# megvii-research/basedet

Hardware: AMD Instinct MI355X
Metric: images/sec training RetinaNet-R50-FPN 1333x800 (higher is better)
Workload: dtype bf16; 1 GPU; retinanet_r50_800x1344 train step (fwd+bwd+allreduce+SGD), DummyLoader boxes, random-init weights, inputs resident in HBM; per_gpu_batch=16, global_batch=16, parallelism=dp1

## Files before the change

### basedet_amd/_lib.py

```python
import ctypes as C
import os

import torch

_HERE = os.path.dirname(os.path.abspath(__file__))
LIB_PATH = os.environ.get("BASEDET_HIP_LIB") or os.path.join(_HERE, "lib", "libbasedet_hip.so")

BD_MAX_SEGS = 8
EPI_RELU, EPI_ADD_BEFORE, EPI_ADD_AFTER, EPI_MASK, EPI_SPARSE = 1, 2, 4, 8, 16


class BasedetHipError(RuntimeError):
    pass


class ConvDesc(C.Structure):
    _fields_ = [
        ("N", C.c_int32), ("Cin", C.c_int32), ("Cout", C.c_int32), ("R", C.c_int32), ("S", C.c_int32),
        ("stride", C.c_int32), ("pad", C.c_int32), ("nseg", C.c_int32),
        ("Hi", C.c_int32 * BD_MAX_SEGS), ("Wi", C.c_int32 * BD_MAX_SEGS),
        ("Ho", C.c_int32 * BD_MAX_SEGS), ("Wo", C.c_int32 * BD_MAX_SEGS),
        ("in_off", C.c_int32 * BD_MAX_SEGS), ("out_off", C.c_int32 * BD_MAX_SEGS),
        ("in_pix_per_img", C.c_int32), ("out_pix_per_img", C.c_int32),
        ("route", C.c_int32 * 4), ("sr_seed", C.c_uint32),
    ]


class PackDesc(C.Structure):
    _fields_ = [("w", C.c_void_p), ("row_scale", C.c_void_p), ("w_fwd", C.c_void_p), ("w_dgrad", C.c_void_p),
                ("Cout", C.c_int32), ("RS", C.c_int32), ("Cin", C.c_int32), ("block_start", C.c_int32)]


_P, _I, _L, _F, _Z = C.c_void_p, C.c_int, C.c_int64, C.c_float, C.c_size_t
_D = C.POINTER(ConvDesc)

SIGNATURES = {
    "bd_last_error_string": (C.c_char_p, []),
    "bd_version": (_I, []),
    "bd_conv_last_kernel": (C.c_char_p, []),
    "bd_probe_mfma_rate": (_I, [C.c_double, C.POINTER(C.c_double), C.POINTER(C.c_double), _P]),
    "bd_probe_kernel_clock": (_I, [C.c_char_p, _I, C.POINTER(C.c_double), C.POINTER(C.c_double)]),
    "bd_conv2d_fwd": (_I, [_D, _P, _P, _P, _P, _P, _I, _P]),
    "bd_conv2d_dgrad": (_I, [_D, _P, _P, _P, _P, _P, _I, _P]),
    "bd_conv2d_fwd_bits": (_I, [_D, _P, _P, _P, _P, _P, _P, _I, _P]),
    "bd_conv2d_fwd_ex": (_I, [_D, _P, _P, _P, _P, _P, _P, _P, _F, _I, _P]),
    "bd_conv2d_dgrad_ex": (_I, [_D, _P, _P, _P, _P, _P, _P, _P, _F, _I, _P]),
    "bd_conv2d_dgrad_bits": (_I, [_D, _P, _P, _P, _P, _P, _I, _P]),
    "bd_conv2d_wgrad_workspace_bytes": (_Z, [_D]),
    "bd_conv2d_wgrad": (_I, [_D, _P, _P, _P, _P, _I, _P, _Z, _P]),
    "bd_conv2d_wgrad_bias_workspace_bytes": (_Z, [_D]),
    "bd_conv2d_wgrad_bias": (_I, [_D, _P, _P, _P, _P, _P, _I, _P, _Z, _P]),
    "bd_fpn_deconv_pack": (_I, [_P, _I, _P, _P, _P]),
    "bd_fpn_deconv_fwd": (_I, [_P, _P, _P, _P, _I, _I, _I, _I, _I, _I, _P]),
    "bd_fpn_deconv_dgrad": (_I, [_P, _P, _P, _P, _I, _I, _I, _I, _I, _I, _P]),
    "bd_fpn_deconv_wgrad_workspace_bytes": (_Z, [_I, _I, _I, _I]),
    "bd_fpn_deconv_wgrad": (_I, [_P, _P, _P, _I, _P, _Z, _I, _I, _I, _I, _I, _I, _P]),
    "bd_wgrad_queue_create": (_I, [_P]),
    "bd_wgrad_queue_destroy": (_I, [_P]),
    "bd_wgrad_queue_pending": (_I, [_P]),
    "bd_conv2d_wgrad_queued": (_I, [_P, _D, _P, _P, _P, _P, _P, _I, _P, _Z, _P]),
    "bd_wgrad_queue_flush": (_I, [_P, _P]),
    "bd_stem_conv7x7_fwd": (_I, [_I, _I, _I, _P, _P, _P, _P, _P]),
    "bd_stem_pool_fwd": (_I, [_I, _I, _I, _P, _P, _P, _P, _P]),
    "bd_stem_weight_pack": (_I, [_P, _P, _P, _P]),
    "bd_weight_pack": (_I, [_P, _P, _P, _P, _I, _I, _I, _P]),
    "bd_weight_pack_blocks": (_I, [_I, _I, _I]),
    "bd_weight_pack_multi": (_I, [_P, _I, _I, _P]),
    "bd_colsum_workspace_bytes": (_Z, [_I]),
    "bd_colsum_bf16": (_I, [_P, _I, _L, _L, _L, _I, _P, _I, _P, _Z, _P]),
    "bd_pad_normalize": (_I, [_P, _I, _I, _I, _I, _I, _P, _P, _P, _P]),
    "bd_bottleneck_fwd_supported": (_I, [_I, _I, _I, _I, _I, _I, _I]),
    "bd_bottleneck_fwd": (_I, [_I, _I, _I, _I, _I, _I, _P, _P, _P, _P, _P, _P, _P, _P, _P, _P, _P]),
    "bd_h2d_create": (_I, [C.POINTER(C.c_void_p), _I, _I]),
    "bd_h2d_threads": (_I, [_P]),
    "bd_h2d_submit": (_I, [_P, _P, _I, _L, _P, _L, _P]),
    "bd_h2d_destroy": (_I, [_P]),
    "bd_pad_normalize_nchw": (_I, [_P, _I, _I, _I, _I, _I, _P, _P, _P, _P]),
    "bd_maxpool3x3s2_fwd": (_I, [_P, _I, _I, _I, _I, _P, _P]),
    "bd_upsample2x_add_fwd": (_I, [_P, _L, _L, _P, _L, _L, _I, _I, _I, _I, _P]),
    "bd_upsample2x_add_bwd": (_I, [_P, _L, _L, _P, _L, _L, _I, _I, _I, _I, _I, _P]),
    "bd_relu_bf16": (_I, [_P, _P, _L, _P]),
    "bd_relu_bwd_bf16": (_I, [_P, _P, _P, _P, _L, _P]),
    "bd_add_bf16": (_I, [_P, _P, _P, _L, _P]),
    "bd_anchors_generate": (_I, [_I, _I, _I, _F, _P, _I, _P, _P]),
    "bd_points_generate": (_I, [_I, _I, _I, _F, _I, _P, _P]),
    "bd_box_pairwise": (_I, [_P, _I, _P, _I, _I, _P, _P]),
    "bd_box_encode": (_I, [_P, _P, _L, _P, _P, _P, _P]),
    "bd_box_decode": (_I, [_P, _P, _L, _P, _P, _P, _P]),
    "bd_retina_assign_encode": (_I, [_P, _I, _P, _P, _I, _I, _F, _F, _I, _P, _P, _P, _P, _P, _P, _P, _Z, _P]),
    "bd_fcos_assign": (_I, [_P, _I, _P, _P, _P, _I, _F, _P, _P, _I, _I, _P, _P, _P, _P, _P]),
    "bd_ota_assign_workspace_bytes": (_Z, [_I, _I]),
    "bd_ota_assign": (_I, [_P, _I, _P, _P, _I, _P, _I, _P, _P, _P, _I, _I, _F, _F, _F, _F, _I, _P, _P, _P, _P, _P, _Z, _P]),
    "bd_ota_sinkhorn_workspace_bytes": (_Z, [_I, _I, _I]),
    "bd_ota_assign_sinkhorn": (_I, [_P, _I, _P, _P, _I, _P, _I, _P, _P, _P, _I, _I, _F, _F, _F, _F, _I, _F, _I, _P, _P, _P, _P, _P, _Z, _P]),
    "bd_freeanchor_workspace_bytes": (_Z, [_I, _I, _I, _I]),
    "bd_freeanchor_loss_fwd_bwd": (_I, [_P, _P, _I, _I, _P, _I, _I, _P, _P, _I, _I, _P, _P, _F, _I, _F, _F, _F, _F, _P, _P, _P, _P, _Z, _P]),
    "bd_atss_assign_workspace_bytes": (_Z, [_I, _I]),
    "bd_atss_assign": (_I, [_P, _I, _P, _P, _I, _I, _F, _P, _P, _I, _I, _P, _P, _P, _P, _P, _Z, _P]),
    "bd_nms_workspace_bytes": (_Z, [_I]),
    "bd_batched_nms": (_I, [_P, _P, _P, _I, _F, _I, _P, _P, _P, _Z, _P]),
    "bd_focal_loss_fwd_bwd": (_I, [_P, _P, _L, _I, _F, _F, _P, _I, _F, _P, _P, _P]),
    "bd_focal_loss_fwd_bwd_general": (_I, [_P, _P, _L, _I, _F, _F, _P, _I, _F, _P, _P, _P]),
    "bd_smooth_l1_fwd_bwd": (_I, [_P, _P, _P, _L, _I, _I, _F, _P, _I, _F, _P, _P, _P]),
    "bd_giou_ltrb_fwd_bwd": (_I, [_P, _P, _P, _P, _L, _P, _F, _P, _P, _P]),
    "bd_bce_logits_fwd_bwd": (_I, [_P, _I, _I, _P, _P, _L, _P, _P, _P, _P]),
    "bd_groupnorm_workspace_bytes": (_Z, [_I, _I, _I, _L]),
    "bd_groupnorm_fwd": (_I, [_P, _P, _P, _I, _I, _P, _P, _L, _I, _F, _I, _P, _P, _P, _Z, _P]),
    "bd_conv2d_fwd_gnstats_bytes": (_Z, [_D]),
    "bd_conv2d_fwd_gnstats": (_I, [_D, _P, _P, _P, _P, _P, _Z, _P]),
    "bd_groupnorm_fwd_parts": (_I, [_D, _P, _P, _P, _P, _F, _I, _P, _P, _P]),
    "bd_groupnorm_bwd": (_I, [_P, _P, _P, _P, _P, _I, _I, _P, _P, _L, _I, _I, _P, _P, _P, _I, _P, _Z, _P]),
    "bd_fcos_offsets_fwd": (_I, [_P, _I, _P, _I, _I, _P, _P, _P, _L, _P, _P]),
    "bd_fcos_offsets_workspace_bytes": (_Z, []),
    "bd_fcos_offsets_bwd": (_I, [_P, _I, _P, _I, _I, _P, _P, _P, _L, _P, _P, _P, _P, _P, _Z, _P]),
    "bd_rpn_assign_encode": (_I, [_P, _I, _P, _P, _I, _I, _F, _F, _I, _P, _P, _P, _P, _P, _P, _P, _Z, _P]),
    "bd_sample_labels": (_I, [_P, _P, _P, _I, _I, _I, _I, _P, _P]),
    "bd_segment_topk": (_I, [_P, _I, _I, _L, _I, _I, _I, _I, _P, _P, _I, _F, _I, _P, _P, _P, _P]),
    "bd_nms_batched_workspace_bytes": (_Z, [_I, _I]),
    "bd_nms_batched": (_I, [_P, _P, _P, _I, _I, _F, _I, _I, _P, _P, _P, _Z, _P]),
    "bd_rpn_proposals_workspace_bytes": (_Z, [_I, _I, _P, _I, _I, _I]),
    "bd_rpn_proposals": (_I, [_P, _I, _I, _I, _I, _I, _L, _I, _P, _P, _P, _P, _I, _P, _P, _I, _F, _I, _P, _P, _P, _Z, _P]),
    "bd_rpn_proposals_joint": (_I, [_P, _I, _I, _I, _I, _I, _L, _I, _P, _P, _P, _P, _I, _P, _P, _I, _F, _I, _P, _P, _P, _Z, _P]),
    "bd_rcnn_sample_targets": (_I, [_P, _P, _I, _P, _P, _I, _I, _P, _P, _I, _I, _I, _F, _F, _F, _P, _P, _P, _P, _P, _P, _P, _P]),
    "bd_roi_align_fwd": (_I, [_P, _L, _I, _I, _P, _P, _P, _P, _P, _P, _I, _I, _I, _I, _I, _P, _P]),
    "bd_conv1x1_thin_bwd_workspace_bytes": (_Z, []),
    "bd_conv1x1_thin_fwd": (_I, [_P, _P, _P, _L, _I, _I, _P, _P]),
    "bd_conv1x1_thin_bwd": (_I, [_P, _P, _P, _L, _I, _I, _P, _P, _P, _I, _P, _Z, _P]),
    "bd_roi_align_bwd": (_I, [_P, _L, _I, _I, _P, _P, _P, _P, _P, _P, _I, _I, _I, _I, _I, _P, _P]),
    "bd_roi_align_bwd_bf16_workspace_bytes": (_Z, [_I, _I, _P, _P, _I]),
    "bd_roi_align_bwd_bf16": (_I, [_P, _L, _I, _I, _I, _P, _P, _P, _P, _P, _P, _I, _I, _I, _I, _I, _P, _I, _P, _Z, _P]),
    "bd_subsample2x_fwd": (_I, [_P, _L, _L, _I, _I, _P, _L, _L, _I, _I, _P]),
    "bd_subsample2x_bwd_add": (_I, [_P, _L, _L, _P, _L, _L, _I, _I, _I, _I, _P]),
    "bd_f32_to_bf16": (_I, [_P, _P, _L, _P]),
    "bd_f32_to_bf16_add": (_I, [_P, _P, _L, _P]),
    "bd_rpn_loss_fwd_bwd": (_I, [_P, _I, _I, _I, _I, _P, _P, _L, _F, _P, _P, _P, _P]),
    "bd_rcnn_loss_fwd_bwd": (_I, [_P, _I, _I, _I, _P, _P, _I, _F, _P, _P, _P, _P]),
    "bd_det_scores": (_I, [_P, _P, _I, _I, _L, _I, _P, _P]),
    "bd_rcnn_predict": (_I, [_P, _I, _I, _I, _P, _P, _I, _I, _P, _P, _P, _P, _P]),
    "bd_det_candidates": (_I, [_I, _P, _P, _P, _I, _I, _P, _I, _P, _P, _I, _I, _P, _P, _P, _P, _P, _P, _P]),
    "bd_det_finalize": (_I, [_P, _P, _P, _P, _P, _I, _P, _P, _P, _P, _P]),
    "bd_sgd_momentum_step": (_I, [_P, _P, _P, _L, _F, _F, _F, _F, _P]),
    "bd_clip_grad_value": (_I, [_P, _L, _F, _F, _F, _P]),
    "bd_clip_grad_norm_workspace_bytes": (_Z, []),
    "bd_clip_grad_norm": (_I, [_P, _L, _F, _F, _F, _P, _P, _Z, _P]),
    "bd_quantize_fp8": (_I, [_P, _L, _F, _P, _P]),
    "bd_weight_pack_fp8": (_I, [_P, _P, _I, _I, _I, _F, _P, _P, _P]),
    "bd_conv2d_fwd_fp8": (_I, [_D, _P, _P, _P, _P, _P, _P, _I, _P]),
    "bd_conv2d_fwd_fp8_ex": (_I, [_D, _P, _P, _P, _P, _P, _P, _P, _F, _I, _P]),
    "bd_quantize_bf8": (_I, [_P, _L, _F, _P, C.c_uint32, _P]),
    "bd_absmax_bf16": (_I, [_P, _L, _P, _P]),
    "bd_weight_pack_fp8_t": (_I, [_P, _P, _I, _I, _I, _F, _P, _P, _P]),
    "bd_conv2d_dgrad_fp8": (_I, [_D, _P, _P, _P, _P, _P, _P, _P, _F, _I, _P]),
    "bd_conv2d_wgrad_fp8_workspace_bytes": (_Z, [_D]),
    "bd_conv2d_wgrad_fp8": (_I, [_D, _P, _P, _F, _P, _P, _I, _P, _Z, _P]),
    "bd_conv1x1_fp8": (_I, [_D, _I, _P, _P, _P, _P, _P, _P, _P, _P, _P, _P, _F, _I, _P]),
    "bd_sigmoid_focal_loss_elem": (_I, [_P, _P, _L, _F, _F, _P, _P, _P, _P]),
    "bd_bce_elem": (_I, [_P, _P, _L, _I, _P, _P, _P, _P]),
    "bd_smooth_l1_elem": (_I, [_P, _P, _L, _F, _P, _P, _P, _P]),
    "bd_iou_loss_ltrb": (_I, [_P, _P, _L, _I, _F, _P, _P, _P, _P, _P]),
    "bd_iou_to_loss": (_I, [_P, _L, _I, _F, _P, _P]),
    "bd_matcher_matrix": (_I, [_P, _I, _L, _P, _P, _I, _I, _P, _P, _P, _P]),
    "bd_assign_roi_levels": (_I, [_P, _I, _I, _I, _I, _P, _P]),
    "bd_roi_pool_max_fwd": (_I, [_P, _I, _I, _I, _I, _P, _I, _F, _I, _I, _P, _P]),
    "bd_comm_unique_id": (_I, [_P]),
    "bd_comm_init": (_I, [C.POINTER(C.c_void_p), _P, _I, _I, _I]),
    "bd_comm_rank": (_I, [_P]),
    "bd_comm_world": (_I, [_P]),
    "bd_comm_stream": (_P, [_P]),
    "bd_comm_bcast": (_I, [_P, _P, _Z, _I, _I, _P]),
    "bd_comm_allreduce": (_I, [_P, _P, _Z, _I, _I, _P]),
    "bd_comm_allreduce_async": (_I, [_P, _P, _Z, _I, _I, C.POINTER(C.c_void_p), _I]),
    "bd_comm_allreduce_async_bf16": (_I, [_P, _P, _P, _Z, _I, C.POINTER(C.c_void_p), _I]),
    "bd_comm_wait": (_I, [_P, _P]),
    "bd_comm_destroy": (_I, [_P]),
}

_lib = None


def load():
    global _lib
    if _lib is not None:
        return _lib
    if not os.path.exists(LIB_PATH):
        raise BasedetHipError(
            f"{LIB_PATH} is missing: build it with `python -m basedet_amd.build` (hipcc, gfx950). "
            "There is no CPU fallback for the basedet_amd operator path.")
    lib = C.CDLL(LIB_PATH)
    for name, (res, args) in SIGNATURES.items():
        fn = getattr(lib, name)
        fn.restype = res
        fn.argtypes = args
    _lib = lib
    return lib


# ... 27 lines not shown
```

### basedet_amd/build.py

```python
import hashlib
import os
import subprocess
import sys

HERE = os.path.dirname(os.path.abspath(__file__))
CSRC = os.path.join(HERE, "csrc")
OUT_DIR = os.path.join(HERE, "lib")
LIB = os.path.join(OUT_DIR, os.environ.get("BD_LIB_NAME", "libbasedet_hip.so"))
HIPCC = os.environ.get("HIPCC", "/opt/rocm/bin/hipcc")
ARCH = "gfx950"

SOURCES = {
    "image_ops.hip": [],
    "h2d.hip": [],
    "conv_igemm.hip": [],
    "conv3x3.hip": [],
    "conv3x3_pp.hip": [],
    "conv3x3_pp128.hip": [],
    "conv1x1.hip": [],
    "conv1x1_ring.hip": [],
    "conv1x1_thin.hip": [],
    "bottleneck_fused.hip": [],
    "conv_fp8.hip": [],
    "conv3x3_pp8.hip": [],
    "conv_wgrad.hip": [],
    "conv_wgrad3x3.hip": [],
    "conv_wgrad3x3_ring.hip": [],
    "conv_wgrad3x3_fp8.hip": [],
    "conv_wgrad1x1.hip": [],
    "conv_wgrad1x1_ring.hip": [],
    "fpn_deconv.hip": [],
    "stem.hip": [],
    "boxops.hip": ["-ffp-contract=off"],
    "rcnn_ops.hip": ["-ffp-contract=off"],
    "postprocess.hip": ["-ffp-contract=off"],
    "freeanchor.hip": ["-ffp-contract=off"],
    "ota.hip": ["-ffp-contract=off"],
    "losses.hip": [],
    "norm.hip": [],
    "comm.hip": [],
    "layer_ops.hip": ["-ffp-contract=off"],
    "probe.hip": [],
}
COMMON = ["-O3", "-std=c++17", "-fPIC", f"--offload-arch={ARCH}", "-Wno-unused-result", "-I", os.path.join(HERE, "..", "include")]
COMMON += os.environ.get("BD_EXTRA_FLAGS", "").split()


def _digest():
    h = hashlib.sha256()
    for name in sorted(os.listdir(CSRC)) + ["../../include/basedet_hip.h"]:
        with open(os.path.join(CSRC, name), "rb") as f:
            h.update(name.encode())
            h.update(f.read())
    flags = [f for f in COMMON if not os.path.isabs(f)]
    h.update(repr(sorted(SOURCES.items())).encode() + repr(flags).encode())
    return h.hexdigest()


def build(force=False, verbose=True):
    os.makedirs(OUT_DIR, exist_ok=True)
    stamp = os.path.join(OUT_DIR, "build.stamp" if "BD_LIB_NAME" not in os.environ else os.environ["BD_LIB_NAME"] + ".stamp")
    dig = _digest()
    if not force and os.path.exists(LIB) and os.path.exists(stamp) and open(stamp).read().strip() == dig:
        return LIB
    objs = []
    procs = []
    for src, extra in SOURCES.items():
        obj = os.path.join(OUT_DIR, os.environ.get("BD_LIB_NAME", "") + src.replace(".hip", ".o"))
        cmd = [HIPCC, *COMMON, *extra, "-c", os.path.join(CSRC, src), "-o", obj]
        if verbose:
            print(" ".join(cmd), flush=True)
        procs.append((src, subprocess.Popen(cmd, stdout=subprocess.PIPE, stderr=subprocess.STDOUT, text=True)))
        objs.append(obj)
    failed = False
    for src, p in procs:
        out, _ = p.communicate()
        if p.returncode != 0:
            failed = True
            sys.stderr.write(f"--- {src} failed ---\n{out}\n")
        elif verbose and out.strip():
            print(out)
    if failed:
        raise RuntimeError("hipcc failed")
    cmd = [HIPCC, "-shared", "-fPIC", f"--offload-arch={ARCH}", "-o", LIB, *objs]
    if verbose:
        print(" ".join(cmd), flush=True)
    subprocess.check_call(cmd)
    with open(stamp, "w") as f:
        f.write(dig)
    return LIB


def build_driver(verbose=False):
    src = os.path.join(HERE, "..", "tools", "abi_driver.cpp")
    name = os.path.basename(LIB)
    out = os.path.join(OUT_DIR, "abi_driver" if name == "libbasedet_hip.so" else "abi_driver." + name)
    lib = build(force=False, verbose=verbose)
    if os.path.exists(out) and os.path.getmtime(out) >= max(os.path.getmtime(src), os.path.getmtime(lib)):
        return out
    cmd = [HIPCC, "-O2", "-std=c++17", "-x", "hip", f"--offload-arch={ARCH}", "-I", os.path.join(HERE, "..", "include"), src,
           "-o", out, "-L", OUT_DIR, "-l:" + os.path.basename(LIB), "-Wl,-rpath,$ORIGIN", "-Wno-unused-result", "-Wno-unused-value"]
    if verbose:
        print(" ".join(cmd), flush=True)
    subprocess.check_call(cmd)
    return out


if __name__ == "__main__":
    print(build(force="--force" in sys.argv))
    print(build_driver(verbose=True))
```

### basedet_amd/csrc/conv3x3_pp.hip

```cpp
#include "conv3x3_pp128_body.h"

namespace {

constexpr int PH = 4, PW = 16, IH = PH + 2, IW = PW + 2;
constexpr int NPATCH = 4;
constexpr int XROWS = NPATCH * IH * IW;
constexpr int X_PITCH = 144;
constexpr int X_BYTES = XROWS * X_PITCH;
constexpr int XPASSES = 7;
constexpr int TILE_CO = 256;
constexpr int W_SLOT = TILE_CO * 128;
constexpr int NSLOT = 3;
constexpr int W_BYTES = NSLOT * W_SLOT;
constexpr int GTAB_TILES = 16;
constexpr int GTAB_BYTES = GTAB_TILES * NPATCH * 32;
constexpr int LDS_BYTES = W_BYTES + X_BYTES + TILE_CO * 4 + GTAB_BYTES;
constexpr int MAX_SEG = BD_MAX_SEGS;
constexpr int TAIL_CO = 64;

struct PSeg { int patch_start, H, W, pw, src_off, dst_off; float inv_pw; };

struct PParams {
    const bf16_raw* src;
    const bf16_raw* w;
    const float* bias;
    const bf16_raw* add;
    const bf16_raw* mask;
    bf16_raw* dst;
    int CK, CO, flags, nseg;
    int src_ppi, dst_ppi;
    unsigned src_bytes;
    int patches_per_img, total_patches, n_tiles;
    int main_grid;
    int px_tiles;
    int tail_end;
    float inv_ppi;
    PSeg seg[MAX_SEG];
    float* gn_part;
};

typedef __attribute__((address_space(3))) void lds_void_t;
typedef __attribute__((address_space(1))) const void glb_void_t;

__device__ __forceinline__ int pp_div(int n, int d, float inv) {
    int q = (int)((float)n * inv);
    const int r = n - q * d;
    q += (r >= d) - (r < 0);
    return q;
}

__device__ __forceinline__ int swz(int row, int chunk) { return row * 128 + ((chunk ^ (row & 7)) << 4); }
__device__ __forceinline__ int colperm(int f) { return f < 4 ? 2 * f : (f < 12 ? 2 * (f - 4) + 1 : 2 * (f - 8)); }
__device__ __forceinline__ int xpos(int chunk) { return (chunk >> 2) * 64 + ((((chunk & 1) << 1) | ((chunk >> 1) & 1)) << 4); }

#ifdef BD_PP_STAMP
__device__ unsigned long long g_pp_stamp[64];
__device__ unsigned long long g_pp_span[2048];
#endif
#ifndef BD_PP_ABLATE
#define BD_PP_ABLATE 0
#endif
__device__ unsigned long long g_pp_clk[2];
#define PP_FENCE() __builtin_amdgcn_sched_barrier(0)
#define PP_BARRIER() do { asm volatile("" ::: "memory"); __builtin_amdgcn_s_barrier(); asm volatile("" ::: "memory"); } while (0)

template <int MODE, bool GNS = false>
__global__ __launch_bounds__(512, 1) void conv3x3_pp_kernel(const PParams p) {
    extern __shared__ __attribute__((aligned(16))) unsigned char smem[];
    if ((int)blockIdx.x >= p.main_grid) {
        pp128::body<MODE, TAIL_CO>(p, smem, (int)blockIdx.x - p.main_grid, (int)gridDim.x - p.main_grid, p.total_patches, p.tail_end,
                                   (p.CO + TAIL_CO - 1) / TAIL_CO);
        return;
    }
    if (blockIdx.x == 0 && threadIdx.x == 0) bd_clk_mark(g_pp_clk, false);
    unsigned char* wbuf = smem;
    unsigned char* xbuf = smem + W_BYTES;
    float* sbias = reinterpret_cast<float*>(smem + W_BYTES + X_BYTES);

#ifdef BD_PP_STAMP
    int st_n = 0;
    const bool st_on = blockIdx.x == 100 % gridDim.x && threadIdx.x == 0;
#define PP_STAMP() do { if (st_on && st_n < 62) g_pp_stamp[st_n] = __builtin_amdgcn_s_memtime(); ++st_n; } while (0)
    PP_STAMP();
    if (st_on) g_pp_stamp[62] = __builtin_amdgcn_s_memrealtime();
    if (threadIdx.x == 0 && blockIdx.x < 1024) g_pp_span[2 * blockIdx.x] = __builtin_amdgcn_s_memrealtime();
#else
#define PP_STAMP() do { } while (0)
#endif
    const int tid = threadIdx.x, lane = tid & 63, wave = __builtin_amdgcn_readfirstlane(tid >> 6);
    const int wm = wave >> 2, wp = wave & 3;
    int bid = blockIdx.x;
    {
        const int nwg = p.main_grid;
        const int q = nwg >> 3, r = nwg & 7, xcd = bid & 7;
        bid = (xcd < r ? xcd * (q + 1) : r * (q + 1) + (xcd - r) * q) + (bid >> 3);
    }
    const int ct = bid % p.n_tiles;
    int pt = bid / p.n_tiles;
    const int pt_step = p.main_grid / p.n_tiles;
    const int co0 = ct * TILE_CO;

    constexpr unsigned X_NONE = 0x80000000u;
    const int x_lds0 = (tid >> 3) * X_PITCH + xpos(tid & 7);
    unsigned x_off[XPASSES];

    int* gtab = reinterpret_cast<int*>(smem + W_BYTES + X_BYTES + TILE_CO * 4);
    const int pt_first = pt;
    auto build_table = [&](int k0) {
        const int k = k0 + (lane >> 2);
        const int ptile = pt_first + k * pt_step;
        const int pid = ptile * NPATCH + (lane & (NPATCH - 1));
        int vH = 0, vW = 0, vy = 0, vx = 0, vs = 0, vd = 0;
        if (ptile < p.px_tiles && pid < p.total_patches) {
            const int n = pp_div(pid, p.patches_per_img, p.inv_ppi);
            const int rem = pid - n * p.patches_per_img;
            int g_start = p.seg[0].patch_start, g_H = p.seg[0].H, g_W = p.seg[0].W, g_pw = p.seg[0].pw;
            int g_src = p.seg[0].src_off, g_dst = p.seg[0].dst_off;
            float g_inv = p.seg[0].inv_pw;
#pragma unroll
            for (int q = 1; q < MAX_SEG; ++q) {
                const bool in = q < p.nseg && rem >= p.seg[q].patch_start;
                g_start = in ? p.seg[q].patch_start : g_start; g_H = in ? p.seg[q].H : g_H; g_W = in ? p.seg[q].W : g_W;
                g_pw = in ? p.seg[q].pw : g_pw; g_src = in ? p.seg[q].src_off : g_src; g_dst = in ? p.seg[q].dst_off : g_dst;
                g_inv = in ? p.seg[q].inv_pw : g_inv;
            }
            const int local = rem - g_start;
            const int by = pp_div(local, g_pw, g_inv), bx = local - by * g_pw;
            vy = by * PH; vx = bx * PW; vH = g_H; vW = g_W;
            vs = n * p.src_ppi + g_src;
            vd = n * p.dst_ppi + g_dst;
        }
        typedef __attribute__((ext_vector_type(4))) int i32x4_t;
        i32x4_t* e = reinterpret_cast<i32x4_t*>(gtab + ((k & (GTAB_TILES - 1)) * NPATCH + (lane & (NPATCH - 1))) * 8);
        e[0] = (i32x4_t){vy, vx, vH, vW};
        e[1] = (i32x4_t){vs, vd, 0, 0};
    };
    auto decode = [&](int k, int& e_oy0, int& e_px0, int& e_H, int& e_W, int& e_dst) {
        int py0[NPATCH], px0[NPATCH], pH[NPATCH], pWd[NPATCH];
        int psrc[NPATCH], pdst[NPATCH];
        int tq = tid;
        asm volatile("" : "+v"(tq));
        {
            typedef __attribute__((ext_vector_type(4))) int i32x4_t;
            const i32x4_t* e = reinterpret_cast<const i32x4_t*>(gtab + ((k & (GTAB_TILES - 1)) * NPATCH + (tq & (NPATCH - 1))) * 8);
            const i32x4_t e0 = e[0], e1 = e[1];
#pragma unroll
            for (int q = 0; q < NPATCH; ++q) {
                py0[q] = __builtin_amdgcn_readlane(e0[0], q); px0[q] = __builtin_amdgcn_readlane(e0[1], q);
                pH[q] = __builtin_amdgcn_readlane(e0[2], q); pWd[q] = __builtin_amdgcn_readlane(e0[3], q);
                psrc[q] = __builtin_amdgcn_readlane(e1[0], q); pdst[q] = __builtin_amdgcn_readlane(e1[1], q);
            }
        }
#pragma unroll
        for (int k = 0; k < XPASSES; ++k) {
            const int row = (tq >> 3) + 64 * k;
            unsigned off = X_NONE;
            if (row < XROWS) {
                const int lo = (64 * k) / (IH * IW), hi = (64 * k + 63) / (IH * IW) < NPATCH ? (64 * k + 63) / (IH * IW) : NPATCH - 1;
                const bool up = row >= hi * (IH * IW);
                const int pk = up ? hi : lo;
                const int rr = row - pk * (IH * IW);
                const int iy = rr / IW, ix = rr - iy * IW;
                const int qy = up ? py0[hi] : py0[lo], qx = up ? px0[hi] : px0[lo], H = up ? pH[hi] : pH[lo];
                const int W = up ? pWd[hi] : pWd[lo], qs = up ? psrc[hi] : psrc[lo];
                const int y = qy - 1 + iy, x = qx - 1 + ix;
                if (y >= 0 && x >= 0 && y < H && x < W) off = (unsigned)((qs + y * W + x) * p.CK + (tq & 7) * 8) * 2u;
            }
            x_off[k] = off;
        }
        e_oy0 = py0[0]; e_px0 = px0[0]; e_H = pH[0]; e_W = pWd[0]; e_dst = pdst[0];
#pragma unroll
        for (int q = 1; q < NPATCH; ++q)
            if (wp == q) { e_oy0 = py0[q]; e_px0 = px0[q]; e_H = pH[q]; e_W = pWd[q]; e_dst = pdst[q]; }
    };
    int c_oy0, c_px0, c_H, c_W, c_dst;
    int kt = 0;
    if (wave == 0) build_table(0);
    asm volatile("s_waitcnt lgkmcnt(0)" ::: "memory");
    PP_BARRIER();
    decode(0, c_oy0, c_px0, c_H, c_W, c_dst);
    const __amdgpu_buffer_rsrc_t x_rsrc =
        __builtin_amdgcn_make_buffer_rsrc(const_cast<bf16_raw*>(p.src), 0, p.src_bytes, 0x00020000);
    u32x4_t rx[XPASSES];
    auto load_x = [&](int cb) {
        int so = cb * 128;
        asm volatile("" : "+s"(so));
        const bool dead = cb * 64 + (tid & 7) * 8 >= p.CK;
#pragma unroll
        for (int k = 0; k < XPASSES; ++k) rx[k] = __builtin_amdgcn_raw_buffer_load_b128(x_rsrc, dead ? X_NONE : x_off[k], so, 0);
    };
    auto write_x = [&]() {
#pragma unroll
        for (int k = 0; k < XPASSES; ++k)
            if (k < XPASSES - 1 || (tid >> 3) + 64 * k < XROWS)
                *reinterpret_cast<u32x4_t*>(xbuf + x_lds0 + k * (64 * X_PITCH)) = rx[k];
    };

    unsigned dma_src[4];
#pragma unroll
    for (int k = 0; k < 4; ++k) {
        const int pc = wave + 8 * k;
        const int lrow = 8 * pc + (lane >> 3);
        const int chunk = (lane & 7) ^ (lane >> 3);
        const int rho = lrow & 15;
        int co = co0 + (lrow & 192) + 32 * ((lrow >> 5) & 1) + 8 * (rho >> 2) + 4 * ((lrow >> 4) & 1) + (rho & 3);
        if (co >= p.CO) co = p.CO - 1;
        dma_src[k] = (unsigned)(co * 9 * p.CK + chunk * 8) * 2u;
    }
    const __amdgpu_buffer_rsrc_t w_rsrc =
        __builtin_amdgcn_make_buffer_rsrc(const_cast<bf16_raw*>(p.w), 0, (unsigned)(p.CO * 9 * p.CK) * 2u, 0x00020000);
    bool dma_on = true;
    auto dma_piece = [&](int tap, int cb, int slot, int k) {
        if ((BD_PP_ABLATE & 2) && !dma_on) return;
        unsigned char* l = wbuf + slot * W_SLOT + (wave + 8 * k) * 1024;
        int so = (tap * p.CK + cb * 64) * 2;
        asm volatile("" : "+s"(so));
        __builtin_amdgcn_raw_ptr_buffer_load_lds(w_rsrc, (lds_void_t*)l, 16, dma_src[k], so, 0, 0);
    };

    f32x4_t acc[8][4];

    const int frow = lane & 15, fchunk = lane >> 4;
    const unsigned char* a_base[2];
#pragma unroll
    for (int kk = 0; kk < 2; ++kk) a_base[kk] = wbuf + swz(wm * 128 + frow, kk * 4 + fchunk);
    typedef __attribute__((address_space(3))) const unsigned char lds_u8_t;
    typedef __attribute__((address_space(3))) const bf16x8_t lds_bf16x8_t;
    unsigned a_hi[2];
#pragma unroll
    for (int kk = 0; kk < 2; ++kk) {
        a_hi[kk] = (unsigned)(size_t)(lds_u8_t*)(a_base[kk]) + 2 * W_SLOT;
        asm volatile("" : "+v"(a_hi[kk]));
    }
    const unsigned char* b_base = xbuf + (wp * (IH * IW) + colperm(frow)) * X_PITCH + xpos(fchunk);

    bf16x8_t fa[8], fb[4];
    auto load_a = [&](int kk, int slot) {
#pragma unroll
        for (int i = 0; i < 8; ++i) {
            if (slot == 2) fa[i] = *(lds_bf16x8_t*)(size_t)(a_hi[kk] + i * 2048);
            else fa[i] = *reinterpret_cast<const bf16x8_t*>(a_base[kk] + slot * W_SLOT + i * 2048);
        }
    };
    auto load_b = [&](int kk, int t) {
        int dy = t / 3, dx = t - 3 * (t / 3);
        if (MODE == 1) { dy = 2 - dy; dx = 2 - dx; }
#pragma unroll
        for (int j = 0; j < 4; ++j)
            fb[j] = *reinterpret_cast<const bf16x8_t*>(b_base + ((j + dy) * IW + dx) * X_PITCH + kk * 64);
    };
    auto mfma_rows = [&](int i0, int i1) {
#pragma unroll
        for (int i = i0; i < i1; ++i)
#pragma unroll
            for (int j = 0; j < 4; ++j)
                asm volatile("v_mfma_f32_16x16x32_bf16 %0, %1, %2, %0" : "+v"(acc[i][j]) : "v"(fa[i]), "v"(fb[j]));
    };

    const int kblocks = (p.CK + 63) >> 6;

    PP_STAMP();
    if (tid < TILE_CO) sbias[tid] = (p.bias && co0 + tid < p.CO) ? p.bias[co0 + tid] : 0.f;
    load_x(0);
#pragma unroll
    for (int k = 0; k < 4; ++k) dma_piece(0, 0, 0, k);
#pragma unroll
    for (int k = 0; k < 4; ++k) dma_piece(1, 0, 1, k);
#pragma unroll
    for (int k = 0; k < 4; ++k) dma_piece(2, 0, 2, k);
    write_x();
    asm volatile("s_waitcnt vmcnt(0) lgkmcnt(0)" ::: "memory");
    PP_BARRIER();
    PP_FENCE();
    if (BD_PP_ABLATE & 2) dma_on = false;

    PP_STAMP();
#if defined(BD_PP_PRIO) && BD_PP_PRIO == 1
    if (wm == 1) __builtin_amdgcn_s_setprio(1);
#endif
    for (;;) {
    const int pt_next = pt + pt_step;
    const bool more = pt_next < p.px_tiles;
    int n_oy0 = 0, n_px0 = 0, n_H = 0, n_W = 0, n_dst = 0;
#pragma unroll
    for (int i = 0; i < 8; ++i)
#pragma unroll
        for (int j = 0; j < 4; ++j) acc[i][j] = (f32x4_t){0.f, 0.f, 0.f, 0.f};
    for (int cb = 0; cb < kblocks; ++cb) {
        const bool last_kb = cb + 1 == kblocks;
        const bool cont = !last_kb || more;
        const int nb = last_kb ? 0 : cb + 1;
        if (last_kb) PP_STAMP();
        if (last_kb && more) decode(kt + 1, n_oy0, n_px0, n_H, n_W, n_dst);
        if (wm == 1) PP_BARRIER();
        PP_FENCE();
#pragma unroll
        for (int t = 0; t < 9; ++t) {
#pragma unroll
            for (int kk = 0; kk < 2; ++kk) {
                const int slot = t % 3;
                if (!((BD_PP_ABLATE & 1) && kk == 1)) {
                load_b(kk, t);
                PP_FENCE();
                load_a(kk, slot);
                PP_FENCE();
                }
                if (kk == 1) {
                    if (BD_PP_ABLATE & 2) { }
                    else if (!cont && t >= 7) asm volatile("s_waitcnt vmcnt(0)" ::: "memory");
                    else if (t >= 1 || cb > 0) asm volatile("s_waitcnt vmcnt(1)" ::: "memory");
                    if (t == 6) {
                        if (cont) load_x(nb);
                        else {
#pragma unroll
                            for (int k = 0; k < XPASSES; ++k) asm volatile("" : "=v"(rx[k]));
                        }
                    }
                    PP_FENCE();
                }
                if (kk == 0) {
                    if (t + 1 < 9) { if (t > 1 || cb > 0) dma_piece(t + 1, cb, (t + 1) % 3, 3); }
                    else if (cont) dma_piece(0, nb, 0, 3);
                    if (t + 2 < 9) { if (t > 0 || cb > 0) dma_piece(t + 2, cb, (t + 2) % 3, 0); }
                    else if (cont) dma_piece(t - 7, nb, (t + 2) % 3, 0);
                } else {
#pragma unroll
                    for (int pc = 1; pc < 3; ++pc) {
                        if (t + 2 < 9) { if (t > 0 || cb > 0) dma_piece(t + 2, cb, (t + 2) % 3, pc); }
                        else if (cont) dma_piece(t - 7, nb, (t + 2) % 3, pc);
                    }
                    if (t == 8 && last_kb && more) dma_piece(1, 0, 1, 3);
                }
                PP_FENCE();
                PP_BARRIER();
                asm volatile("s_waitcnt lgkmcnt(0)" ::: "memory");
                PP_FENCE();
#if defined(BD_PP_PRIO) && BD_PP_PRIO == 0
                __builtin_amdgcn_s_setprio(1);
#endif
                mfma_rows(0, 8);
#if defined(BD_PP_PRIO) && BD_PP_PRIO == 0
                __builtin_amdgcn_s_setprio(0);
#endif
                PP_FENCE();
                PP_BARRIER();
                PP_FENCE();
            }
        }
        if (wm == 0) PP_BARRIER();
        PP_FENCE();
        if (cont) {
            write_x();
            asm volatile("s_waitcnt lgkmcnt(0)" ::: "memory");
            PP_BARRIER();
            PP_FENCE();
        }
    }

    PP_STAMP();
    asm volatile("s_nop 15\n\ts_nop 15" ::: "memory");
    int lq = lane;
    asm volatile("" : "+v"(lq));
    const int cg = lq >> 4, erow = lq & 15;
    const bool do_relu = !GNS && (p.flags & BD_EPI_RELU);
    const bool add_before = !GNS && (p.flags & BD_EPI_ADD_BEFORE) && p.add;
    const bool add_after = !GNS && (p.flags & BD_EPI_ADD_AFTER) && p.add;
    const bool do_mask = !GNS && (p.flags & BD_EPI_MASK) && p.mask;
    const int cbase = co0 + wm * 128 + 8 * cg;
    const int oy0 = c_oy0, ox = c_px0 + colperm(erow), H = c_H, W = c_W, dbase = c_dst;
    if (!add_before && !add_after) {
        typedef __attribute__((ext_vector_type(2))) float f32x2_e;
        typedef __attribute__((ext_vector_type(2))) __bf16 bf16x2_e;
        typedef __attribute__((ext_vector_type(2))) short i16x2_e;
        const i16x2_e relu_floor = do_relu ? (i16x2_e){0, 0} : (i16x2_e){-32768, -32768};
        bf16_raw* drow[4];
        const bf16_raw* mrow[4];
        bool okj[4];
#pragma unroll
        for (int j = 0; j < 4; ++j) {
            const int oy = oy0 + j;
            okj[j] = oy < H && ox < W;
            const long long e = (long long)(dbase + oy * W + ox) * p.CO + cbase;
            drow[j] = p.dst + e;
            mrow[j] = p.mask + e;
        }
        u32x4_t mv[4][4];
#pragma unroll
        for (int h = 0; h < 4; ++h) {
            const bool okh = cbase + 32 * h < p.CO;
#pragma unroll
            for (int j = 0; j < 4; ++j) {
                mv[h][j] = (u32x4_t){0u, 0u, 0u, 0u};
                if (do_mask && okh && okj[j]) mv[h][j] = *reinterpret_cast<const u32x4_t*>(mrow[j] + 32 * h);
            }
        }
        PP_FENCE();
        if (more) {
#pragma unroll
            for (int k = 0; k < 4; ++k) dma_piece(2, 0, 2, k);
        }
        PP_FENCE();
        float gsum[4] = {0.f, 0.f, 0.f, 0.f}, gsq[4] = {0.f, 0.f, 0.f, 0.f};
        auto unit = [&](int h, int j, const f32x4_t b0, const f32x4_t b1) {
            u32x4_t o;
#pragma unroll
            for (int k = 0; k < 4; ++k) {
                const f32x4_t a = acc[2 * h + (k >> 1)][j];
                const f32x4_t bb = (k >> 1) ? b1 : b0;
                f32x2_e v = {a[2 * (k & 1)], a[2 * (k & 1) + 1]};
                v += (f32x2_e){bb[2 * (k & 1)], bb[2 * (k & 1) + 1]};
                if constexpr (GNS) {
                    if (okj[j]) { gsum[h] += v[0] + v[1]; gsq[h] += v[0] * v[0] + v[1] * v[1]; }
                }
                i16x2_e w = __builtin_bit_cast(i16x2_e, __builtin_convertvector(v, bf16x2_e));
                if (do_mask) {
                    unsigned gate;
                    asm("v_pk_sub_i16 %0, 0, %1 clamp\n\tv_pk_ashrrev_i16 %0, 15, %0 op_sel_hi:[0,1]" : "=v"(gate) : "v"(mv[h][j][k]));
                    w &= __builtin_bit_cast(i16x2_e, gate);
                }
                w = __builtin_elementwise_max(w, relu_floor);
                o[k] = __builtin_bit_cast(unsigned, w);
            }
            return o;
        };
#pragma unroll
        for (int h = 0; h < 4; ++h) {
            const bool okh = cbase + 32 * h < p.CO;
            const f32x4_t b0 = *reinterpret_cast<const f32x4_t*>(sbias + wm * 128 + 8 * cg + 32 * h);
            const f32x4_t b1 = *reinterpret_cast<const f32x4_t*>(sbias + wm * 128 + 8 * cg + 32 * h + 4);
            if (h == 0) {
                u32x4_t o0[4];
#pragma unroll
                for (int j = 0; j < 4; ++j) o0[j] = unit(0, j, b0, b1);
                PP_FENCE();
                PP_STAMP();
                if (more) asm volatile("s_waitcnt vmcnt(4)" ::: "memory");
                else asm volatile("s_waitcnt vmcnt(0)" ::: "memory");
                PP_STAMP();
                PP_FENCE();
#pragma unroll
                for (int j = 0; j < 4; ++j) {
                    if (BD_PP_ABLATE & 4) asm volatile("" :: "v"(o0[j]));
                    else if (okh && okj[j]) *reinterpret_cast<u32x4_t*>(drow[j]) = o0[j];
                }
            } else {
#pragma unroll
                for (int j = 0; j < 4; ++j) {
                    const u32x4_t o = unit(h, j, b0, b1);
                    if (BD_PP_ABLATE & 4) asm volatile("" :: "v"(o));
                    else if (okh && okj[j]) *reinterpret_cast<u32x4_t*>(drow[j] + 32 * h) = o;
                }
            }
        }
        if constexpr (GNS) {
            const int pid = pt * NPATCH + wp;
#pragma unroll
            for (int h = 0; h < 4; ++h) {
                float a = gsum[h], b = gsq[h];
#pragma unroll
                for (int m = 8; m >= 1; m >>= 1) { a += __shfl_xor(a, m, 64); b += __shfl_xor(b, m, 64); }
                if (erow == 0 && pid < p.total_patches && cbase + 32 * h < p.CO) {
                    float* o = p.gn_part + ((long long)pid * 32 + ((cbase + 32 * h) >> 3)) * 2;
                    *reinterpret_cast<f32x2_t*>(o) = (f32x2_t){a, b};
                }
            }
        }
    } else {
    if (more) {
#pragma unroll
        for (int k = 0; k < 4; ++k) dma_piece(2, 0, 2, k);
    }
    long long erow_off[4];
#pragma unroll
    for (int j = 0; j < 4; ++j) erow_off[j] = (long long)(dbase + (oy0 + j) * W + ox) * p.CO + cbase;
#pragma unroll
    for (int hp = 0; hp < 2; ++hp) {
        u32x4_t av[2][4], mv[2][4];
#pragma unroll
        for (int hh = 0; hh < 2; ++hh) {
            const int h = 2 * hp + hh;
#pragma unroll
            for (int j = 0; j < 4; ++j) {
                const int oy = oy0 + j;
                const bool ok = cbase + 32 * h < p.CO && oy < H && ox < W;
                const long long idx = erow_off[j] + 32 * h;
                av[hh][j] = (u32x4_t){0u, 0u, 0u, 0u}; mv[hh][j] = (u32x4_t){0u, 0u, 0u, 0u};
                if (ok && (add_before || add_after)) av[hh][j] = *reinterpret_cast<const u32x4_t*>(p.add + idx);
                if (ok && do_mask) mv[hh][j] = *reinterpret_cast<const u32x4_t*>(p.mask + idx);
            }
        }
        if (hp == 0) asm volatile("s_waitcnt vmcnt(0)" ::: "memory");
#pragma unroll
        for (int hh = 0; hh < 2; ++hh) {
            const int h = 2 * hp + hh;
            if (cbase + 32 * h >= p.CO) continue;
            float bias[8];
            {
                const f32x4_t b0 = *reinterpret_cast<const f32x4_t*>(sbias + wm * 128 + 8 * cg + 32 * h);
                const f32x4_t b1 = *reinterpret_cast<const f32x4_t*>(sbias + wm * 128 + 8 * cg + 32 * h + 4);
#pragma unroll
                for (int k = 0; k < 4; ++k) { bias[k] = b0[k]; bias[4 + k] = b1[k]; }
            }
#pragma unroll
            for (int j = 0; j < 4; ++j) {
                const int oy = oy0 + j;
                if (oy >= H || ox >= W) continue;
                const long long idx = erow_off[j] + 32 * h;
                float v[8];
#pragma unroll
                for (int k = 0; k < 8; ++k) v[k] = acc[2 * h + (k >> 2)][j][k & 3] + bias[k];
                const u32x4_t a4 = av[hh][j], m4 = mv[hh][j];
                if (add_before) {
#pragma unroll
                    for (int k = 0; k < 4; ++k) { v[2 * k] += bf_lo(a4[k]); v[2 * k + 1] += bf_hi(a4[k]); }
                }
                if (do_relu) {
#pragma unroll
                    for (int k = 0; k < 8; ++k) v[k] = fmaxf(v[k], 0.f);
                }
                if (do_mask) {
#pragma unroll
                    for (int k = 0; k < 4; ++k) {
                        if (!(bf_lo(m4[k]) > 0.f)) v[2 * k] = 0.f;
                        if (!(bf_hi(m4[k]) > 0.f)) v[2 * k + 1] = 0.f;
                    }
                }
                if (add_after) {
#pragma unroll
                    for (int k = 0; k < 4; ++k) { v[2 * k] += bf_lo(a4[k]); v[2 * k + 1] += bf_hi(a4[k]); }
                }
                u32x4_t o;
#pragma unroll
                for (int k = 0; k < 4; ++k) o[k] = pack_bf2(v[2 * k], v[2 * k + 1]);
                *reinterpret_cast<u32x4_t*>(p.dst + idx) = o;
            }
        }
    }
    }
    PP_STAMP();
    if (!more) break;
    ++kt;
    pt = pt_next;
    c_oy0 = n_oy0; c_px0 = n_px0; c_H = n_H; c_W = n_W; c_dst = n_dst;
    PP_FENCE();
    PP_STAMP();
    }
    if (blockIdx.x == 0 && threadIdx.x == 0) bd_clk_mark(g_pp_clk, true);
#ifdef BD_PP_STAMP
    if (st_on) { g_pp_stamp[63] = __builtin_amdgcn_s_memrealtime(); g_pp_stamp[61] = __builtin_amdgcn_s_memtime(); }
    if (threadIdx.x == 0 && blockIdx.x < 1024) { asm volatile("s_waitcnt vmcnt(0)" ::: "memory"); g_pp_span[2 * blockIdx.x + 1] = __builtin_amdgcn_s_memrealtime(); }
#endif
}

}

BD_KNOB int g_pp_tail_split = 1;
BD_KNOB int g_pp_persistent = 1;
extern BD_KNOB int g_patch_pp;
static int pp_launch(const bd_conv_desc* d, int mode, const void* src, const void* w, const float* bias, const void* add,
                     const void* mask, void* dst, int flags, float* gn_part, hipStream_t stream) {
    PParams p{};
    p.gn_part = gn_part;
    p.CK = mode == 0 ? d->Cin : d->Cout;
    p.CO = mode == 0 ? d->Cout : d->Cin;
    p.src_ppi = mode == 0 ? d->in_pix_per_img : d->out_pix_per_img;
    p.dst_ppi = mode == 0 ? d->out_pix_per_img : d->in_pix_per_img;
    if (p.CK % 8 != 0 || p.CO <= 128 || p.CO % 8 != 0) return 1;
    if ((long long)d->N * p.src_ppi * p.CK * 2 >= 0x7fffffffll || (long long)d->N * p.dst_ppi >= 0x7fffffffll ||
        (long long)p.CO * 9 * p.CK >= 0x7fffffffll) return 1;
    p.src = (const bf16_raw*)src; p.w = (const bf16_raw*)w; p.bias = bias;
    p.add = (const bf16_raw*)add; p.mask = (const bf16_raw*)mask; p.dst = (bf16_raw*)dst;
    p.flags = flags; p.nseg = d->nseg;
    p.src_bytes = (unsigned)((long long)d->N * p.src_ppi * p.CK * 2);
    int ps = 0;
    for (int s = 0; s < d->nseg; ++s) {
        PSeg& sg = p.seg[s];
        sg.patch_start = ps; sg.H = d->Ho[s]; sg.W = d->Wo[s]; sg.pw = cdiv(d->Wo[s], PW); sg.inv_pw = 1.0f / (float)sg.pw;
        sg.src_off = mode == 0 ? d->in_off[s] : d->out_off[s];
        sg.dst_off = mode == 0 ? d->out_off[s] : d->in_off[s];
        ps += cdiv(d->Ho[s], PH) * sg.pw;
    }
    p.patches_per_img = ps;
    p.inv_ppi = 1.0f / (float)ps;
    p.total_patches = ps * d->N;
    if (p.total_patches >= (1 << 24)) return 1;
    p.n_tiles = cdiv(p.CO, TILE_CO);
    int grid = cdiv(p.total_patches, NPATCH) * p.n_tiles;
    int tail_wgs = 0;
    int px_tiles = cdiv(p.total_patches, NPATCH);
    p.tail_end = p.total_patches;
    const int num_cus = bd_num_cus();
    if (g_pp_tail_split && !gn_part && p.n_tiles == 1 && px_tiles > num_cus) {
        const int r = px_tiles % num_cus;
        if (r > 0 && r * (TILE_CO / TAIL_CO) <= num_cus) {
            px_tiles -= r;
            p.total_patches = px_tiles * NPATCH;
            tail_wgs = cdiv(p.tail_end - p.total_patches, NPATCH) * cdiv(p.CO, TAIL_CO);
        }
    }
    p.px_tiles = px_tiles;
    p.main_grid = px_tiles * p.n_tiles;
    if (g_pp_persistent) {
        const int g1 = (num_cus / p.n_tiles) * p.n_tiles;
        const int rounds = cdiv(px_tiles * p.n_tiles, g1 * GTAB_TILES);
        if (g1 * rounds < p.main_grid) p.main_grid = g1 * rounds;
    }
    {
        const int grid128 = cdiv(p.total_patches, NPATCH) * cdiv(p.CO, 128);
        if (!gn_part && g_patch_pp < 2 && 3 * cdiv(grid, 256) >= 2 * cdiv(grid128, 256)) return 1;
    }
    BD_ONCE_PER_DEVICE(
        (void)hipFuncSetAttribute(reinterpret_cast<const void*>(&conv3x3_pp_kernel<0>), hipFuncAttributeMaxDynamicSharedMemorySize, LDS_BYTES);
        (void)hipFuncSetAttribute(reinterpret_cast<const void*>(&conv3x3_pp_kernel<1>), hipFuncAttributeMaxDynamicSharedMemorySize, LDS_BYTES));
    bd_note_kernel("conv3x3_pp_kernel");
    if (gn_part) {
        BD_ONCE_PER_DEVICE((void)hipFuncSetAttribute(reinterpret_cast<const void*>(&conv3x3_pp_kernel<0, true>), hipFuncAttributeMaxDynamicSharedMemorySize, LDS_BYTES));
        hipLaunchKernelGGL((conv3x3_pp_kernel<0, true>), dim3(p.main_grid), dim3(512), LDS_BYTES, stream, p);
    } else if (mode == 0) hipLaunchKernelGGL((conv3x3_pp_kernel<0>), dim3(p.main_grid + tail_wgs), dim3(512), LDS_BYTES, stream, p);
    else hipLaunchKernelGGL((conv3x3_pp_kernel<1>), dim3(p.main_grid + tail_wgs), dim3(512), LDS_BYTES, stream, p);
    return 0;
}

int bd_pp_clk_read(unsigned long long* out2, int reset) {
    if (hipMemcpyFromSymbol(out2, HIP_SYMBOL(g_pp_clk), 16) != hipSuccess) return 1;
    if (reset) { const unsigned long long z[2] = {0, 0}; if (hipMemcpyToSymbol(HIP_SYMBOL(g_pp_clk), z, 16) != hipSuccess) return 1; }
    return 0;
}

#ifdef BD_PP_STAMP
extern "C" int bd_debug_pp_stamp(unsigned long long* out2) {
    return hipMemcpyFromSymbol(out2, HIP_SYMBOL(g_pp_stamp), 512) == hipSuccess ? 0 : 1;
}
extern "C" int bd_debug_pp_span(unsigned long long* out2048) {
    return hipMemcpyFromSymbol(out2048, HIP_SYMBOL(g_pp_span), 2048 * 8) == hipSuccess ? 0 : 1;
}
#endif

int bd_conv3x3_pp_launch(const bd_conv_desc* d, int mode, const void* src, const void* w, const float* bias, const void* add,
                         const void* mask, void* dst, int flags, hipStream_t stream) {
    return pp_launch(d, mode, src, w, bias, add, mask, dst, flags, nullptr, stream);
}

int bd_conv3x3_pp_patch_starts(const bd_conv_desc* d, int* starts) {
    int ps = 0;
    for (int s = 0; s < d->nseg; ++s) { starts[s] = ps; ps += cdiv(d->Ho[s], PH) * cdiv(d->Wo[s], PW); }
    starts[d->nseg] = ps;
    return ps;
}

extern "C" size_t bd_conv2d_fwd_gnstats_bytes(const bd_conv_desc* d) {
    if (!d || d->nseg < 1 || d->nseg > BD_MAX_SEGS) return 0;
    int starts[BD_MAX_SEGS + 1];
    return (size_t)d->N * bd_conv3x3_pp_patch_starts(d, starts) * 32 * 2 * sizeof(float);
}

extern "C" int bd_conv2d_fwd_gnstats(const bd_conv_desc* d, const void* x, const void* w_packed, const float* bias, void* y, float* part,
                                     size_t part_bytes, bd_stream_t stream) {
    BD_ROUTE(d);
    BD_REQUIRE(d && x && w_packed && y && part, "conv2d_fwd_gnstats: null pointer");
    BD_REQUIRE(d->R == 3 && d->S == 3 && d->stride == 1 && d->pad == 1 && d->Cout == 256 && d->Cin % 64 == 0,
               "conv2d_fwd_gnstats: 3x3 / stride 1 / pad 1 into 256 channels (GroupNorm(32, 256)) only; got %dx%d s%d p%d %d -> %d", d->R, d->S,
               d->stride, d->pad, d->Cin, d->Cout);
    for (int s = 0; s < d->nseg; ++s)
        BD_REQUIRE(d->Hi[s] == d->Ho[s] && d->Wi[s] == d->Wo[s], "conv2d_fwd_gnstats: level %d changes size", s);
    if (part_bytes < bd_conv2d_fwd_gnstats_bytes(d)) { bd_set_error("conv2d_fwd_gnstats: statistics buffer too small"); return BD_EWORKSPACE; }
    if (pp_launch(d, 0, x, w_packed, bias, nullptr, nullptr, y, 0, part, (hipStream_t)stream) != 0) {
        bd_set_error("conv2d_fwd_gnstats: shape not taken by conv3x3_pp_kernel (tensor too large for 32-bit offsets?)");
        return BD_EINVAL;
    }
    BD_CHECK_LAUNCH("bd_conv2d_fwd_gnstats");
    return BD_OK;
}
```

### basedet_amd/csrc/conv_igemm.hip

```cpp
#include "igemm_params.h"

using namespace igemm;

namespace {

template <int BK>
struct Cfg {
    static constexpr int CHUNKS = BK / 8;
    static constexpr int ROWS_PER_PASS = 256 / CHUNKS;
    static constexpr int PASSES = 128 / ROWS_PER_PASS;
    static constexpr int LDS_STRIDE = BK == 64 ? 160 : 64;
    static constexpr int TILE_BYTES = 128 * LDS_STRIDE;
    __device__ static __forceinline__ int off(int row, int chunk) {
        if constexpr (BK == 64) return row * LDS_STRIDE + chunk * 16;
        else return row * 64 + ((chunk ^ ((row >> 1) & 3)) << 4);
    }
};

template <int BK, bool PRE, bool BUF>
__global__ __launch_bounds__(256) void conv_igemm_kernel(const IgemmParams p) {
    using C = Cfg<BK>;
    extern __shared__ __attribute__((aligned(16))) unsigned char smem[];
    unsigned char* tiles = smem;
    unsigned int* s_tapmask = reinterpret_cast<unsigned int*>(smem);
// ... 380 lines not shown

}


int bd_conv3x3_patch_launch(const bd_conv_desc* d, int mode, const void* src, const void* w, const float* bias,
                            const void* add, const void* mask, void* dst, int flags, hipStream_t stream);

extern BD_KNOB int g_patch_dma;
extern BD_KNOB int g_patch_pp;
extern BD_KNOB int g_patch_pp128;
extern BD_KNOB int g_conv1x1_s2;
extern BD_KNOB int g_pp_tail_split;
extern BD_KNOB int g_pp_persistent;
static int bd_route_patch3x3(int enable) {
#ifdef BD_AB_SKIP
    g_skip_s2_3x3 = (enable >> 4) & 1;
#else
    if ((enable >> 4) & 1) {
        bd_set_error("bd_conv_desc.route[1]: bit 4 (skip the 3x3 / stride-2 launches: a timing A/B that leaves stale outputs) exists in "
                     "-DBD_AB_SKIP diagnostic builds only");
        return BD_EINVAL;
    }
#endif
    g_use_patch3x3 = enable & 1; g_bk32_for_1x1 = (enable >> 1) & 1;
    g_patch_dma = ((enable >> 3) & 1) ^ 1;
    g_patch_pp = ((enable >> 6) & 1) ? 0 : (((enable >> 7) & 1) ? 1 : 2);
    g_patch_pp128 = ((enable >> 9) & 1) ? -1 : ((enable >> 8) & 1);
    g_bk32_s2 = ((enable >> 10) & 1) ^ 1;
    g_igemm_prefetch_epi = ((enable >> 5) & 1) ^ 1;
    g_igemm_buf = ((enable >> 11) & 1) ^ 1;
    g_conv1x1_s2 = ((enable >> 12) & 1) ^ 1;
    g_pp_tail_split = ((enable >> 13) & 1) ^ 1;
    g_pp_persistent = ((enable >> 14) & 1) ^ 1;
    if ((enable >> 16) & 1) {
        bd_set_error("bd_conv_desc.route[1]: bit 16 (conv_igemm_wide.hip) is gone since round 6");
        return BD_EINVAL;
    }
    return BD_OK;
}

int bd_route_dense1x1(int depth);
int bd_route_wgrad(int use_tr);
extern BD_KNOB int g_fp8_patch;

BdRouteScope::BdRouteScope(const bd_conv_desc* d) : rc(BD_OK) {
    const int r0 = d ? d->route[0] : 0, r1 = d ? d->route[1] : 0, r2 = d ? d->route[2] : 0, r3 = d ? d->route[3] : 0;
    if (r0 < 0 || r1 < 0 || r2 < 0 || r3 < 0) {
        bd_set_error("bd_conv_desc.route: negative word (0 = the library's choice, otherwise the route + 1)");
        rc = BD_EINVAL;
        return;
    }
    if ((rc = bd_route_dense1x1(r0 ? r0 - 1 : 1)) != BD_OK) return;
    if ((rc = bd_route_patch3x3(r1 ? r1 - 1 : 3)) != BD_OK) return;
    if ((rc = bd_route_wgrad(r2 ? r2 - 1 : 1)) != BD_OK) return;
    g_fp8_patch = r3 ? (r3 - 1 != 0) : 1;
    g_fp8_sr_seed = d ? d->sr_seed : 0u;
}

int bd_conv1x1_dense_launch(const void* x, const void* w, const float* bias, const void* add, const void* mask, const unsigned* maskbits,
                            void* y, unsigned* ybits, void* y8, float q_scale, int y8_bf8, long long M, int CK, int CO, int flags,
                            hipStream_t stream);

int bd_conv1x1_s2_launch(const bd_conv_desc* d, int mode, const void* src, const void* w, const float* bias, const void* add, const void* mask,
                         const unsigned* maskbits, void* dst, int flags, hipStream_t stream);
namespace {
bool is_dense_1x1(const bd_conv_desc* d) {
    return d->R == 1 && d->S == 1 && d->stride == 1 && d->pad == 0 && d->nseg == 1 && d->in_off[0] == 0 && d->out_off[0] == 0 &&
           d->in_pix_per_img == d->Hi[0] * d->Wi[0] && d->out_pix_per_img == d->Ho[0] * d->Wo[0];
}
}

static int conv2d_fwd_impl(const bd_conv_desc* d, const void* x, const void* w_packed, const float* bias, const void* add, void* y,
                           unsigned* ybits, void* y8, float q_scale, int flags, bd_stream_t stream) {
    if (int e = check_desc(d)) return e;
    BD_REQUIRE(x && w_packed && y, "conv2d_fwd: null pointer");
    BD_REQUIRE(d->Cin % 8 == 0, "conv2d_fwd: Cin=%d must be a multiple of 8", d->Cin);
    BD_REQUIRE(d->Cout % 8 == 0, "conv2d_fwd: Cout=%d must be a multiple of 8", d->Cout);
    BD_REQUIRE(!(flags & BD_EPI_MASK), "conv2d_fwd: BD_EPI_MASK is a dgrad-only flag");
    if (is_dense_1x1(d) &&
        bd_conv1x1_dense_launch(x, w_packed, bias, add, nullptr, nullptr, y, ybits, y8, q_scale, 0, (long long)d->N * d->out_pix_per_img,
                                d->Cin, d->Cout, flags, (hipStream_t)stream) == 0) {
        BD_CHECK_LAUNCH("bd_conv2d_fwd(dense 1x1)");
        return BD_OK;
    }
    if (!ybits && !y8 && d->stride == 2 && d->R == 1 &&
        bd_conv1x1_s2_launch(d, 0, x, w_packed, bias, add, nullptr, nullptr, y, flags, (hipStream_t)stream) == 0) {
        BD_CHECK_LAUNCH("bd_conv2d_fwd(1x1 stride 2)");
        return BD_OK;
    }
    BD_REQUIRE(ybits == nullptr && y8 == nullptr, "conv2d_fwd_bits / _ex: the bit-packed ReLU mask and the e4m3 twin are written by the dense "
               "1x1 kernel only (1x1 / stride 1 over one dense level, Cout %% 32 == 0, tensors < 2 GB)");
#ifdef BD_AB_SKIP
    if (g_skip_s2_3x3 && d->R == 3 && d->S == 3 && d->stride == 2) return BD_OK;
#endif
    if (g_use_patch3x3 && is_3x3s1(d)) {
        bd_conv3x3_patch_launch(d, 0, x, w_packed, bias, add, nullptr, y, flags, (hipStream_t)stream);
        BD_CHECK_LAUNCH("bd_conv2d_fwd(3x3 patch)");
        return BD_OK;
    }
    IgemmParams p{};
    p.src = (const bf16_raw*)x; p.w = (const bf16_raw*)w_packed; p.bias = bias;
    p.add = (const bf16_raw*)add; p.mask = nullptr; p.dst = (bf16_raw*)y;
    p.CK = d->Cin; p.CO = d->Cout; p.R = d->R; p.S = d->S; p.stride = d->stride; p.pad = d->pad;
    p.mode = 0; p.flags = flags;
    p.nsub = d->nseg;
    long long m = 0;
    for (int s = 0; s < d->nseg; ++s) {
        SubSeg& ss = p.sub[s];
        ss.m_start = (int)m;
        ss.Hs = d->Ho[s]; ss.Ws = d->Wo[s]; ss.y0 = 0; ss.x0 = 0; ss.step = 1;
        ss.Wd = d->Wo[s]; ss.dst_off = d->out_off[s];
        ss.Hsrc = d->Hi[s]; ss.Wsrc = d->Wi[s]; ss.src_off = d->in_off[s];
        ss.inv_per_img = 1.0f / (float)(ss.Hs * ss.Ws); ss.inv_ws = 1.0f / (float)ss.Ws;
        m += (long long)d->N * d->Ho[s] * d->Wo[s];
    }
    BD_REQUIRE(m < (1ll << 24), "conv2d_fwd: too many pixels (2^24 limit of the fast index decode)");
    p.linear_dst = (d->nseg == 1 && d->out_off[0] == 0 && d->out_pix_per_img == d->Ho[0] * d->Wo[0]) ? 1 : 0;
    p.linear_src = (p.linear_dst && d->R == 1 && d->S == 1 && d->stride == 1 && d->pad == 0 && d->in_off[0] == 0 &&
                    d->in_pix_per_img == d->Hi[0] * d->Wi[0]) ? 1 : 0;
    p.M = (int)m;
    p.src_pix_per_img = d->in_pix_per_img; p.dst_pix_per_img = d->out_pix_per_img;
    set_buffer_sizes(p, d->N);
    p.m_tiles = cdiv(p.M, TILE_P); p.n_tiles = cdiv(p.CO, TILE_C);
    if (p.CK > 32 && !(g_bk32_for_1x1 && p.R * p.S == 1) && !(g_bk32_s2 && p.stride == 2 && p.m_tiles * p.n_tiles >= 512))
        launch_igemm<64>(p, (hipStream_t)stream);
    else launch_igemm<32>(p, (hipStream_t)stream);
    BD_CHECK_LAUNCH("bd_conv2d_fwd");
    return BD_OK;
}

extern "C" int bd_conv2d_fwd(const bd_conv_desc* d, const void* x, const void* w_packed, const float* bias,
                             const void* add, void* y, int flags, bd_stream_t stream) {
    BD_ROUTE(d);
    return conv2d_fwd_impl(d, x, w_packed, bias, add, y, nullptr, nullptr, 1.f, flags, stream);
}

extern "C" int bd_conv2d_fwd_ex(const bd_conv_desc* d, const void* x, const void* w_packed, const float* bias, const void* add, void* y,
                                uint32_t* ybits, void* y8, float q_scale, int flags, bd_stream_t stream) {
    BD_ROUTE(d);
    return conv2d_fwd_impl(d, x, w_packed, bias, add, y, ybits, y8, q_scale, flags, stream);
}

extern "C" int bd_conv2d_fwd_bits(const bd_conv_desc* d, const void* x, const void* w_packed, const float* bias, const void* add, void* y,
                                  uint32_t* ybits, int flags, bd_stream_t stream) {
    BD_ROUTE(d);
    BD_REQUIRE(ybits != nullptr, "conv2d_fwd_bits: null ybits");
    return conv2d_fwd_impl(d, x, w_packed, bias, add, y, ybits, nullptr, 1.f, flags, stream);
}

static int conv2d_dgrad_impl(const bd_conv_desc* d, const void* g, const void* w_packed_t, const void* add, const void* mask,
                             const unsigned* maskbits, void* dx, void* dx8, float q_scale, int flags, bd_stream_t stream) {
    if (int e = check_desc(d)) return e;
    BD_REQUIRE(g && w_packed_t && dx, "conv2d_dgrad: null pointer");
    if (d->stride == 1) flags &= ~BD_EPI_SPARSE;
    BD_REQUIRE(d->Cout % 8 == 0, "conv2d_dgrad: Cout=%d must be a multiple of 8 (pad the gradient)", d->Cout);
    BD_REQUIRE(d->Cin % 8 == 0, "conv2d_dgrad: Cin=%d must be a multiple of 8", d->Cin);
    BD_REQUIRE(!(flags & BD_EPI_RELU), "conv2d_dgrad: BD_EPI_RELU is a forward-only flag");
    if (is_dense_1x1(d) &&
        bd_conv1x1_dense_launch(g, w_packed_t, nullptr, add, mask, maskbits, dx, nullptr, dx8, q_scale, 1, (long long)d->N * d->in_pix_per_img,
                                d->Cout, d->Cin, flags, (hipStream_t)stream) == 0) {
        BD_CHECK_LAUNCH("bd_conv2d_dgrad(dense 1x1)");
        return BD_OK;
    }
    if (!dx8 && d->stride == 2 && d->R == 1 &&
        bd_conv1x1_s2_launch(d, 1, g, w_packed_t, nullptr, add, mask, maskbits, dx, flags, (hipStream_t)stream) == 0) {
        BD_CHECK_LAUNCH("bd_conv2d_dgrad(1x1 stride 2)");
        return BD_OK;
    }
    BD_REQUIRE(maskbits == nullptr && dx8 == nullptr, "conv2d_dgrad_bits / _ex: the bit-packed ReLU mask is read, and the e5m2 twin written, by "
               "the dense 1x1 kernel only (1x1 / stride 1 over one dense level, Cin %% 32 == 0, tensors < 2 GB)");
#ifdef BD_AB_SKIP
    if (g_skip_s2_3x3 && d->R == 3 && d->S == 3 && d->stride == 2) return BD_OK;
#endif
    if (g_use_patch3x3 && is_3x3s1(d)) {
        bd_conv3x3_patch_launch(d, 1, g, w_packed_t, nullptr, add, mask, dx, flags, (hipStream_t)stream);
        BD_CHECK_LAUNCH("bd_conv2d_dgrad(3x3 patch)");
        return BD_OK;
    }
    IgemmParams p{};
    p.src = (const bf16_raw*)g; p.w = (const bf16_raw*)w_packed_t; p.bias = nullptr;
    p.add = (const bf16_raw*)add; p.mask = (const bf16_raw*)mask; p.dst = (bf16_raw*)dx;
    p.CK = d->Cout; p.CO = d->Cin; p.R = d->R; p.S = d->S; p.stride = d->stride; p.pad = d->pad;
    p.mode = 1; p.flags = flags;
    long long m = 0;
    int ns = 0;
    const int st = d->stride;
    const bool sparse = (flags & BD_EPI_SPARSE) && st > 1;
    BD_REQUIRE(!(flags & BD_EPI_SPARSE) || ((flags & BD_EPI_ADD_BEFORE) && add == dx),
               "conv2d_dgrad: BD_EPI_SPARSE needs an in-place accumulate (BD_EPI_ADD_BEFORE with add == dx)");
    p.flags = flags & ~BD_EPI_SPARSE;
    for (int s = 0; s < d->nseg; ++s) {
        for (int qy = 0; qy < st; ++qy)
            for (int qx = 0; qx < st; ++qx) {
                const int Hs = (d->Hi[s] - qy + st - 1) / st, Ws = (d->Wi[s] - qx + st - 1) / st;
                if (Hs <= 0 || Ws <= 0) continue;
                if (sparse) {
                    bool ry = false, rx = false;
                    for (int r = 0; r < d->R; ++r) ry = ry || ((qy + d->pad - r) % st + st) % st == 0;
                    for (int c = 0; c < d->S; ++c) rx = rx || ((qx + d->pad - c) % st + st) % st == 0;
                    if (!(ry && rx)) continue;
                }
                BD_REQUIRE(ns < MAX_SUB, "conv2d_dgrad: too many sub-segments (levels x stride^2 > %d)", MAX_SUB);
                SubSeg& ss = p.sub[ns++];
                ss.m_start = (int)m;
                ss.Hs = Hs; ss.Ws = Ws; ss.y0 = qy; ss.x0 = qx; ss.step = st;
                ss.Wd = d->Wi[s]; ss.dst_off = d->in_off[s];
                ss.Hsrc = d->Ho[s]; ss.Wsrc = d->Wo[s]; ss.src_off = d->out_off[s];
                ss.inv_per_img = 1.0f / (float)(Hs * Ws); ss.inv_ws = 1.0f / (float)Ws;
                m += (long long)d->N * Hs * Ws;
            }
    }
    p.nsub = ns;
    BD_REQUIRE(m < (1ll << 24), "conv2d_dgrad: too many pixels (2^24 limit of the fast index decode)");
    p.linear_dst = (d->nseg == 1 && st == 1 && d->in_off[0] == 0 && d->in_pix_per_img == d->Hi[0] * d->Wi[0]) ? 1 : 0;
    p.linear_src = (p.linear_dst && d->R == 1 && d->S == 1 && d->pad == 0 && d->out_off[0] == 0 &&
                    d->out_pix_per_img == d->Ho[0] * d->Wo[0]) ? 1 : 0;
    p.M = (int)m;
    p.src_pix_per_img = d->out_pix_per_img; p.dst_pix_per_img = d->in_pix_per_img;
    set_buffer_sizes(p, d->N);
    p.m_tiles = cdiv(p.M, TILE_P); p.n_tiles = cdiv(p.CO, TILE_C);
    if (p.CK > 32 && !(g_bk32_for_1x1 && p.R * p.S == 1) && !(g_bk32_s2 && p.stride == 2 && p.m_tiles * p.n_tiles >= 512))
        launch_igemm<64>(p, (hipStream_t)stream);
    else launch_igemm<32>(p, (hipStream_t)stream);
    BD_CHECK_LAUNCH("bd_conv2d_dgrad");
    return BD_OK;
}

extern "C" int bd_conv2d_dgrad(const bd_conv_desc* d, const void* g, const void* w_packed_t, const void* add,
                               const void* mask, void* dx, int flags, bd_stream_t stream) {
    BD_ROUTE(d);
    return conv2d_dgrad_impl(d, g, w_packed_t, add, mask, nullptr, dx, nullptr, 1.f, flags, stream);
}

extern "C" int bd_conv2d_dgrad_ex(const bd_conv_desc* d, const void* g, const void* w_packed_t, const void* add, const void* mask,
                                  const uint32_t* maskbits, void* dx, void* dx8, float q_scale, int flags, bd_stream_t stream) {
    BD_ROUTE(d);
    return conv2d_dgrad_impl(d, g, w_packed_t, add, maskbits ? nullptr : mask, maskbits, dx, dx8, q_scale,
                             maskbits ? (flags | BD_EPI_MASK) : flags, stream);
}

extern "C" int bd_conv2d_dgrad_bits(const bd_conv_desc* d, const void* g, const void* w_packed_t, const void* add, const uint32_t* maskbits,
                                    void* dx, int flags, bd_stream_t stream) {
    BD_ROUTE(d);
    BD_REQUIRE(maskbits != nullptr, "conv2d_dgrad_bits: null maskbits");
    return conv2d_dgrad_impl(d, g, w_packed_t, add, nullptr, maskbits, dx, nullptr, 1.f, flags | BD_EPI_MASK, stream);
}
```

### basedet_amd/csrc/conv_wgrad.hip

```cpp
#include <vector>
#include "common.h"

namespace {

constexpr int TILE = 128;
constexpr int ROW_PITCH = 288;
constexpr int MAX_SEG = BD_MAX_SEGS;

struct WSeg {
    int m_start;
    int Ho, Wo, per_img;
    float inv_per_img, inv_wo;
    int Hi, Wi, in_off, out_off;
};

struct WgradParams {
    const bf16_raw* x;
    const bf16_raw* g;
    float* slab;
    int Cin, Cout, R, S, stride, pad;
    int M, nseg;
    int in_pix_per_img, out_pix_per_img;
    int ci_tiles, co_tiles, splits, steps_per_split, total_steps;
    WSeg seg[MAX_SEG];
// ... 147 lines not shown
        if (more) stage_write(cur ^ 1);
        __syncthreads();
        cur ^= 1;
    }

    float* slab = p.slab + (long long)split * p.Cout * RS * p.Cin;
#pragma unroll
    for (int j = 0; j < 4; ++j) {
        const int co = co0 + wco * 64 + j * 16 + idx;
        if (co >= p.Cout) continue;
#pragma unroll
        for (int i = 0; i < 4; ++i) {
            const int ci = ci0 + wci * 64 + i * 16 + g4 * 4;
            if (ci >= p.Cin) continue;
            *reinterpret_cast<f32x4_t*>(slab + ((long long)co * RS + tap) * p.Cin + ci) = acc[i][j];
        }
    }
}

}
#include "wgrad_reduce.h"
namespace {

__global__ __launch_bounds__(256) void wgrad_batch_reduce_kernel(const BdRedBatch b) {
    __shared__ f32x4_t red[4][64];
    int ei = 0;
#pragma unroll 1
    for (int k = 1; k < b.count; ++k)
        if ((int)blockIdx.x >= b.e[k].block_begin) ei = k;
    const BdRedEntry& en = b.e[ei];
    const int tx = threadIdx.x & 63, ty = threadIdx.x >> 6;
    const long long e = (long long)((int)blockIdx.x - en.block_begin) * 64 + tx;
    const long long n4 = en.n4;
    f32x4_t s = {0.f, 0.f, 0.f, 0.f};
    if (e < n4) {
        const long long stride = n4 * 4;
        const float* src = en.slab + e * 4;
        const int splits = en.splits;
        int k = ty;
        for (; k + 12 < splits; k += 16) {
            const f32x4_t v0 = *reinterpret_cast<const f32x4_t*>(src + (long long)k * stride);
            const f32x4_t v1 = *reinterpret_cast<const f32x4_t*>(src + (long long)(k + 4) * stride);
            const f32x4_t v2 = *reinterpret_cast<const f32x4_t*>(src + (long long)(k + 8) * stride);
            const f32x4_t v3 = *reinterpret_cast<const f32x4_t*>(src + (long long)(k + 12) * stride);
            s += v0; s += v1; s += v2; s += v3;
        }
        for (; k < splits; k += 4) s += *reinterpret_cast<const f32x4_t*>(src + (long long)k * stride);
    }
    red[ty][tx] = s;
    __syncthreads();
    if (ty != 0 || e >= n4) return;
    f32x4_t t = red[0][tx];
    t += red[1][tx]; t += red[2][tx]; t += red[3][tx];
    long long idx;
    int row;
    if (en.kind == 0) {
        idx = e * 4;
        row = (int)(idx / en.row_len);
    } else {
        const int regs = en.regs;
        const long long per_tile = 8ll * regs * 64;
        const int tile = (int)(e / per_tile);
        int r = (int)(e - tile * per_tile);
        const int wave = r / (regs * 64);
        r -= wave * (regs * 64);
        const int reg = r >> 6, lane = r & 63;
        const int ci_tile = tile / en.co_tiles, co_tile = tile - ci_tile * en.co_tiles;
        int co, ci, tap = 0, taps = 1;
        if (en.kind == 1) {
            tap = reg >> 2; taps = 9;
            co = co_tile * en.tco + (wave >> 2) * 64 + (reg & 3) * 16 + (lane & 15);
            ci = ci_tile * en.tci + (wave & 3) * 16 + (lane >> 4) * 4;
        } else {
            const int i = reg / en.fj, j = reg - i * en.fj;
            const int wco_n = en.tco / (16 * en.fj);
            const int wci = wave / wco_n, wco = wave - wci * wco_n;
            co = co_tile * en.tco + (wco * en.fj + j) * 16 + (lane & 15);
            ci = ci_tile * en.tci + (wci * en.fi + i) * 16 + (lane >> 4) * 4;
        }
        if (co >= en.Cout || ci >= en.Cin) return;
        idx = ((long long)co * taps + tap) * en.Cin + ci;
        row = co;
    }
    float* d = en.dw + idx;
    if (en.row_scale) t *= en.row_scale[row];
    if (en.accumulate) t += *reinterpret_cast<const f32x4_t*>(d);
    *reinterpret_cast<f32x4_t*>(d) = t;
}

int launch_batch(const BdRedEntry* entries, int count, hipStream_t stream) {
    for (int base = 0; base < count; base += BD_RED_MAX) {
        BdRedBatch b{};
        b.count = count - base < BD_RED_MAX ? count - base : BD_RED_MAX;
        int blocks = 0;
        for (int k = 0; k < b.count; ++k) {
            b.e[k] = entries[base + k];
            b.e[k].block_begin = blocks;
            blocks += (int)cdiv64(b.e[k].n4, 64);
        }
        if (blocks > 0) hipLaunchKernelGGL(wgrad_batch_reduce_kernel, dim3(blocks), dim3(256), 0, stream, b);
    }
    return 0;
}

BdRedEntry plain_entry(const float* slab, int splits, long long n, int row_len, const float* row_scale, float* dw, int accumulate) {
    BdRedEntry e{};
    e.slab = slab; e.dw = dw; e.row_scale = row_scale; e.kind = 0; e.splits = splits; e.accumulate = accumulate;
    e.n4 = (int)(n / 4); e.row_len = row_len;
    return e;
}

struct Plan { int ci_tiles, co_tiles, splits, steps_per_split, total_steps; long long M; };

constexpr int BKP_DEFAULT = 64;
BD_KNOB int g_wgrad_use_tr = 1;
BD_KNOB int g_wgrad_use_3x3 = 1;
BD_KNOB int g_wgrad_use_ring = 1;

bool is_3x3s1(const bd_conv_desc* d) {
    if (!(d->R == 3 && d->S == 3 && (d->stride == 1 || d->stride == 2) && d->pad == 1)) return false;
    if ((long long)d->N * d->in_pix_per_img * d->Cin * 2 >= 0x7fffffffll || (long long)d->N * d->out_pix_per_img * d->Cout * 2 >= 0x7fffffffll)
        return false;
    for (int s = 0; s < d->nseg; ++s)
        if ((d->Hi[s] - 1) / d->stride + 1 != d->Ho[s] || (d->Wi[s] - 1) / d->stride + 1 != d->Wo[s]) return false;
    return true;
}

Plan make_plan(const bd_conv_desc* d) {
    Plan pl;
    long long M = 0;
    for (int s = 0; s < d->nseg; ++s) M += (long long)d->N * d->Ho[s] * d->Wo[s];
    pl.M = M;
    pl.ci_tiles = cdiv(d->Cin, TILE);
    pl.co_tiles = cdiv(d->Cout, TILE);
    pl.total_steps = (int)cdiv64(M, BKP_DEFAULT);
    const int tiles = d->R * d->S * pl.ci_tiles * pl.co_tiles;
    int splits = 1024 / tiles;
    if (splits < 1) splits = 1;
    const int max_splits = pl.total_steps / 4 > 0 ? pl.total_steps / 4 : 1;
    if (splits > max_splits) splits = max_splits;
    pl.steps_per_split = cdiv(pl.total_steps, splits);
    pl.splits = cdiv(pl.total_steps, pl.steps_per_split);
    return pl;
}

}

int bd_wgrad1x1_splits(const bd_conv_desc* d);
int bd_wgrad1x1_launch(const bd_conv_desc* d, const void* x, const void* g, float* slab, int* splits_out, hipStream_t stream);
int bd_wgrad3x3_splits(const bd_conv_desc* d, int* total_patches_out, int* patches_per_img_out);
int bd_wgrad3x3_launch(const bd_conv_desc* d, const void* x, const void* g, float* slab, float* csum, int* splits_out, hipStream_t stream);
bool bd_wgrad3x3r_eligible(const bd_conv_desc* d);
size_t bd_wgrad3x3r_slab_bytes(const bd_conv_desc* d, int* splits_out);
int bd_wgrad3x3r_launch(const bd_conv_desc* d, const void* x, const void* g, float* slab, float* csum, int* splits_out, hipStream_t stream);
void bd_wgrad3x3r_entry(const bd_conv_desc* d, BdRedEntry* e);
bool bd_wgrad1x1r_eligible(const bd_conv_desc* d);
size_t bd_wgrad1x1r_slab_bytes(const bd_conv_desc* d, int* splits_out);
int bd_wgrad1x1r_launch(const bd_conv_desc* d, const void* x, const void* g, float* slab, int* splits_out, hipStream_t stream);
void bd_wgrad1x1r_entry(const bd_conv_desc* d, BdRedEntry* e);

int bd_route_wgrad(int use_tr) {
    g_wgrad_use_tr = use_tr & 1;
    g_wgrad_use_3x3 = (use_tr & 2) ? 0 : 1;
    g_wgrad_use_ring = (use_tr & 4) ? 0 : 1;
    if (!(use_tr & 1)) g_wgrad_use_3x3 = 0;
    return BD_OK;
}

void bd_wgrad_reduce_launch(const float* slab, int splits, long long n, int row_len, const float* row_scale, float* dw, int accumulate,
                            hipStream_t stream) {
    const BdRedEntry e = plain_entry(slab, splits, n, row_len, row_scale, dw, accumulate);
    launch_batch(&e, 1, stream);
}

extern "C" size_t bd_conv2d_wgrad_workspace_bytes(const bd_conv_desc* d) {
    BdRouteScope rs__(d);
    if (rs__.rc != BD_OK) return 0;
    if (!d || d->nseg < 1 || d->nseg > BD_MAX_SEGS) return 0;
    const Plan pl = make_plan(d);
    size_t splits = (size_t)pl.splits;
    if (is_3x3s1(d)) {
        const size_t s3 = (size_t)bd_wgrad3x3_splits(d, nullptr, nullptr);
        if (s3 > splits) splits = s3;
    }
    if (d->R == 1 && d->S == 1 && d->pad == 0) {
        const size_t s1 = (size_t)bd_wgrad1x1_splits(d);
        if (s1 > splits) splits = s1;
    }
    size_t bytes = splits * d->Cout * d->R * d->S * d->Cin * sizeof(float);
    if (bd_wgrad3x3r_eligible(d)) {
        const size_t r = bd_wgrad3x3r_slab_bytes(d, nullptr);
        if (r > bytes) bytes = r;
    }
    if (bd_wgrad1x1r_eligible(d)) {
        const size_t r = bd_wgrad1x1r_slab_bytes(d, nullptr);
        if (r > bytes) bytes = r;
    }
    return bytes;
}

namespace {
size_t align256(size_t v) { return (v + 255) & ~size_t(255); }
}

extern "C" size_t bd_colsum_workspace_bytes(int C);
extern "C" int bd_colsum_bf16(const void* g, int N, int64_t pix_per_img, int64_t off, int64_t cnt, int C, float* out, int accumulate,
                              void* ws, size_t ws_bytes, bd_stream_t stream);
struct bd_wgrad_queue { std::vector<BdRedEntry> entries; };
static int wgrad_impl(const bd_conv_desc* d, const void* x, const void* g, const float* row_scale, float* dw, float* dbias,
                      int accumulate, void* ws, size_t ws_bytes, bd_stream_t stream, bd_wgrad_queue* q);

extern "C" size_t bd_conv2d_wgrad_bias_workspace_bytes(const bd_conv_desc* d) {
    BdRouteScope rs__(d);
    if (rs__.rc != BD_OK) return 0;
    const size_t w = bd_conv2d_wgrad_workspace_bytes(d);
    if (!w) return 0;
    size_t extra = bd_colsum_workspace_bytes(d->Cout);
    if (is_3x3s1(d)) {
        const size_t s3 = (size_t)bd_wgrad3x3_splits(d, nullptr, nullptr) * d->Cout * sizeof(float);
        if (s3 > extra) extra = s3;
    }
    if (bd_wgrad3x3r_eligible(d)) {
        int sr = 1;
        (void)bd_wgrad3x3r_slab_bytes(d, &sr);
        const size_t s3 = (size_t)sr * d->Cout * sizeof(float);
        if (s3 > extra) extra = s3;
    }
    return align256(w) + extra;
}

extern "C" int bd_conv2d_wgrad_bias(const bd_conv_desc* d, const void* x, const void* g, const float* row_scale, float* dw,
                                    float* dbias, int accumulate, void* ws, size_t ws_bytes, bd_stream_t stream) {
    BD_ROUTE(d);
    BD_REQUIRE(dbias, "conv2d_wgrad_bias: null bias gradient");
    BD_REQUIRE(d && d->Cout <= 2048, "conv2d_wgrad_bias: Cout must be <= 2048");
    const size_t need = bd_conv2d_wgrad_bias_workspace_bytes(d);
    if (ws_bytes < need) {
        bd_set_error("conv2d_wgrad_bias: workspace %zu < required %zu bytes", ws_bytes, need);
        return BD_EWORKSPACE;
    }
    return wgrad_impl(d, x, g, row_scale, dw, dbias, accumulate, ws, ws_bytes, stream, nullptr);
}

extern "C" int bd_conv2d_wgrad(const bd_conv_desc* d, const void* x, const void* g, const float* row_scale,
                               float* dw, int accumulate, void* ws, size_t ws_bytes, bd_stream_t stream) {
    BD_ROUTE(d);
    return wgrad_impl(d, x, g, row_scale, dw, nullptr, accumulate, ws, ws_bytes, stream, nullptr);
}

extern "C" int bd_wgrad_queue_create(bd_wgrad_queue_t* out) {
    BD_REQUIRE(out != nullptr, "bd_wgrad_queue_create: null argument");
    *out = new bd_wgrad_queue();
    return BD_OK;
}
extern "C" int bd_wgrad_queue_destroy(bd_wgrad_queue_t q) {
    delete q;
    return BD_OK;
}
extern "C" int bd_wgrad_queue_pending(bd_wgrad_queue_t q) { return q ? (int)q->entries.size() : 0; }
extern "C" int bd_conv2d_wgrad_queued(bd_wgrad_queue_t q, const bd_conv_desc* d, const void* x, const void* g, const float* row_scale, float* dw,
                                      float* dbias, int accumulate, void* ws, size_t ws_bytes, bd_stream_t stream) {
    BD_ROUTE(d);
    BD_REQUIRE(q != nullptr, "bd_conv2d_wgrad_queued: null queue");
    if (dbias) {
        BD_REQUIRE(d && d->Cout <= 2048, "conv2d_wgrad_queued: Cout must be <= 2048");
        const size_t need = bd_conv2d_wgrad_bias_workspace_bytes(d);
        if (ws_bytes < need) {
            bd_set_error("conv2d_wgrad_queued: workspace %zu < required %zu bytes", ws_bytes, need);
            return BD_EWORKSPACE;
        }
    }
    return wgrad_impl(d, x, g, row_scale, dw, dbias, accumulate, ws, ws_bytes, stream, q);
}
extern "C" int bd_wgrad_queue_flush(bd_wgrad_queue_t q, bd_stream_t stream) {
    BD_REQUIRE(q != nullptr, "bd_wgrad_queue_flush: null queue");
    if (q->entries.empty()) return BD_OK;
    launch_batch(q->entries.data(), (int)q->entries.size(), (hipStream_t)stream);
    q->entries.clear();
    BD_CHECK_LAUNCH("bd_wgrad_queue_flush");
    return BD_OK;
}

static int wgrad_impl(const bd_conv_desc* d, const void* x, const void* g, const float* row_scale, float* dw, float* dbias,
                      int accumulate, void* ws, size_t ws_bytes, bd_stream_t stream, bd_wgrad_queue* q) {
    BD_REQUIRE(d && x && g && dw && ws, "conv2d_wgrad: null pointer");
    BD_REQUIRE(d->nseg >= 1 && d->nseg <= BD_MAX_SEGS, "conv2d_wgrad: nseg out of range");
    BD_REQUIRE(d->Cin % 8 == 0 && d->Cout % 8 == 0, "conv2d_wgrad: Cin=%d / Cout=%d must be multiples of 8", d->Cin, d->Cout);
    const Plan pl = make_plan(d);
    BD_REQUIRE(pl.M < (1ll << 24), "conv2d_wgrad: %lld pixels exceed the 2^24 fast-division range", pl.M);
    const size_t need = bd_conv2d_wgrad_workspace_bytes(d);
    if (ws_bytes < need) {
        bd_set_error("conv2d_wgrad: workspace %zu < required %zu bytes", ws_bytes, need);
        return BD_EWORKSPACE;
    }
    unsigned char* extra = (unsigned char*)ws + align256(need);
    auto bias_fallback = [&]() -> int {
        long long dense = 0;
        bool packed = true;
        for (int s = 0; s < d->nseg; ++s) { packed = packed && d->out_off[s] == dense; dense += (long long)d->Ho[s] * d->Wo[s]; }
        if (packed && dense == d->out_pix_per_img)
            return bd_colsum_bf16(g, 1, 0, 0, (int64_t)d->N * dense, d->Cout, dbias, accumulate, extra, bd_colsum_workspace_bytes(d->Cout), stream);
        for (int s = 0; s < d->nseg; ++s) {
            const int e = bd_colsum_bf16(g, d->N, d->out_pix_per_img, d->out_off[s], (int64_t)d->Ho[s] * d->Wo[s], d->Cout, dbias,
                                         (s > 0 || accumulate) ? 1 : 0, extra, bd_colsum_workspace_bytes(d->Cout), stream);
            if (e != BD_OK) return e;
        }
        return BD_OK;
    };
    auto finish = [&](const BdRedEntry& we, int splits, bool fused_csum) -> int {
        BdRedEntry es[2] = {we, {}};
        int n = 1;
        if (dbias && fused_csum) es[n++] = plain_entry((const float*)extra, splits, d->Cout, 1, nullptr, dbias, accumulate);
        if (q) {
            for (int k = 0; k < n; ++k) q->entries.push_back(es[k]);
        } else {
            launch_batch(es, n, (hipStream_t)stream);
            BD_CHECK_LAUNCH("bd_conv2d_wgrad(reduce)");
        }
        return (dbias && !fused_csum) ? bias_fallback() : BD_OK;
    };
    if (g_wgrad_use_3x3 && g_wgrad_use_ring && bd_wgrad3x3r_eligible(d)) {
        int splitsr = 1;
        bd_note_kernel("conv_wgrad3x3_ring_kernel");
        bd_wgrad3x3r_launch(d, x, g, (float*)ws, dbias ? (float*)extra : nullptr, &splitsr, (hipStream_t)stream);
        BD_CHECK_LAUNCH("bd_conv2d_wgrad(3x3 ring)");
        BdRedEntry e{};
        bd_wgrad3x3r_entry(d, &e);
        e.slab = (const float*)ws; e.splits = splitsr; e.row_scale = row_scale; e.dw = dw; e.accumulate = accumulate;
        return finish(e, splitsr, true);
    }
    if (g_wgrad_use_3x3 && is_3x3s1(d)) {
        int splits3 = 1;
        bd_note_kernel("conv_wgrad3x3_kernel");
        bd_wgrad3x3_launch(d, x, g, (float*)ws, dbias ? (float*)extra : nullptr, &splits3, (hipStream_t)stream);
        BD_CHECK_LAUNCH("bd_conv2d_wgrad(3x3)");
        return finish(plain_entry((const float*)ws, splits3, (long long)d->Cout * 9 * d->Cin, 9 * d->Cin, row_scale, dw, accumulate), splits3, true);
    }
    if (g_wgrad_use_3x3 && g_wgrad_use_ring && bd_wgrad1x1r_eligible(d)) {
        int splitsr = 1;
        bd_note_kernel("conv_wgrad1x1_ring_kernel");
        bd_wgrad1x1r_launch(d, x, g, (float*)ws, &splitsr, (hipStream_t)stream);
        BD_CHECK_LAUNCH("bd_conv2d_wgrad(1x1 ring)");
        BdRedEntry e{};
        bd_wgrad1x1r_entry(d, &e);
        e.slab = (const float*)ws; e.splits = splitsr; e.row_scale = row_scale; e.dw = dw; e.accumulate = accumulate;
        return finish(e, splitsr, false);
    }
    if (g_wgrad_use_3x3 && d->R == 1 && d->S == 1 && d->pad == 0) {
        int splits1 = 1;
        bd_note_kernel("conv_wgrad1x1_kernel");
        bd_wgrad1x1_launch(d, x, g, (float*)ws, &splits1, (hipStream_t)stream);
        BD_CHECK_LAUNCH("bd_conv2d_wgrad(1x1)");
        return finish(plain_entry((const float*)ws, splits1, (long long)d->Cout * d->Cin, d->Cin, row_scale, dw, accumulate), splits1, false);
    }
    WgradParams p{};
    p.x = (const bf16_raw*)x; p.g = (const bf16_raw*)g; p.slab = (float*)ws;
    p.Cin = d->Cin; p.Cout = d->Cout; p.R = d->R; p.S = d->S; p.stride = d->stride; p.pad = d->pad;
    p.M = (int)pl.M; p.nseg = d->nseg;
    p.in_pix_per_img = d->in_pix_per_img; p.out_pix_per_img = d->out_pix_per_img;
    p.ci_tiles = pl.ci_tiles; p.co_tiles = pl.co_tiles; p.splits = pl.splits;
    p.steps_per_split = pl.steps_per_split; p.total_steps = pl.total_steps;
    long long m = 0;
    for (int s = 0; s < d->nseg; ++s) {
        WSeg& sg = p.seg[s];
        sg.m_start = (int)m;
        sg.Ho = d->Ho[s]; sg.Wo = d->Wo[s]; sg.per_img = d->Ho[s] * d->Wo[s];
        sg.inv_per_img = 1.0f / (float)sg.per_img; sg.inv_wo = 1.0f / (float)sg.Wo;
        sg.Hi = d->Hi[s]; sg.Wi = d->Wi[s]; sg.in_off = d->in_off[s]; sg.out_off = d->out_off[s];
        m += (long long)d->N * sg.per_img;
    }
    const int grid = pl.splits * d->R * d->S * pl.ci_tiles * pl.co_tiles;
    const size_t lds = 4 * BKP_DEFAULT * ROW_PITCH;
    BD_ONCE_PER_DEVICE(
        (void)hipFuncSetAttribute(reinterpret_cast<const void*>(&conv_wgrad_kernel<BKP_DEFAULT, true>),
                            hipFuncAttributeMaxDynamicSharedMemorySize, (int)lds);
        (void)hipFuncSetAttribute(reinterpret_cast<const void*>(&conv_wgrad_kernel<BKP_DEFAULT, false>),
                            hipFuncAttributeMaxDynamicSharedMemorySize, (int)lds));
    bd_note_kernel("conv_wgrad_kernel");
    if (g_wgrad_use_tr)
        hipLaunchKernelGGL((conv_wgrad_kernel<BKP_DEFAULT, true>), dim3(grid), dim3(256), lds, (hipStream_t)stream, p);
    else
        hipLaunchKernelGGL((conv_wgrad_kernel<BKP_DEFAULT, false>), dim3(grid), dim3(256), lds, (hipStream_t)stream, p);
    BD_CHECK_LAUNCH("bd_conv2d_wgrad");
    const long long n = (long long)d->Cout * d->R * d->S * d->Cin;
    return finish(plain_entry((const float*)ws, pl.splits, n, d->R * d->S * d->Cin, row_scale, dw, accumulate), pl.splits, false);
}
```

### basedet_amd/csrc/conv_wgrad3x3_ring.hip

```cpp
#include <stdlib.h>
#include "common.h"
#include "wgrad_reduce.h"

namespace {

constexpr int RK_CI = 64, RK_CO = 128;
constexpr int XW = 10;
constexpr int X_PIECES = 13;
constexpr int X_BYTES = X_PIECES * 1024;
constexpr int G_PIECES = 16;
constexpr int G_BYTES = G_PIECES * 1024;
constexpr int STAGE = X_BYTES + G_BYTES;
constexpr int DEPTH = 3;
constexpr int NSTAGE = 5;
constexpr int LDS_BYTES = NSTAGE * STAGE;
constexpr int REGS = 36;
constexpr unsigned X_NONE = 0x80000000u;

typedef __attribute__((address_space(3))) void lds_void_rk_t;

struct RSeg { int patch_start, H, W, pw, in_off, out_off, Hi, Wi; };

struct RParams {
    const bf16_raw* x;
    const bf16_raw* g;
    float* slab;
    float* csum;
    int Cin, Cout, N, nseg;
    int in_ppi, out_ppi;
    unsigned x_bytes, g_bytes;
    int patches_per_img, total_patches, patches_per_split;
    int ci_tiles, co_tiles;
    RSeg seg[BD_MAX_SEGS];
};

#ifdef BD_RK_STAMP
__device__ unsigned long long g_rk_stamp[8][8];
#endif

#ifndef BD_RK_ABLATE
#define BD_RK_ABLATE 0
#endif
__device__ unsigned long long g_rk_clk[2];

__device__ __forceinline__ void rk_dma16(__amdgpu_buffer_rsrc_t rsrc, unsigned lds_addr, unsigned voff, int soff = 0) {
    asm volatile("s_mov_b32 m0, %1\n\ts_nop 0\n\tbuffer_load_dwordx4 %0, %2, %3 offen lds" : : "v"(voff), "s"(lds_addr), "s"(rsrc), "s"(soff) : "memory");
}

__global__ __launch_bounds__(512) void conv_wgrad3x3_ring_kernel(const RParams p) {
    extern __shared__ __attribute__((aligned(16))) unsigned char smem[];
    const int tid = threadIdx.x, lane = tid & 63, wave = __builtin_amdgcn_readfirstlane(tid >> 6);
    const int wi = wave & 3, wo = wave >> 2;
    if (blockIdx.x == 0 && threadIdx.x == 0) bd_clk_mark(g_rk_clk, false);
    int bid = blockIdx.x;
    {
        const int nwg = gridDim.x;
        const int q = nwg >> 3, r = nwg & 7, xcd = bid & 7;
        bid = (xcd < r ? xcd * (q + 1) : r * (q + 1) + (xcd - r) * q) + (bid >> 3);
    }
    const int wg = bid;
    const int tiles = p.ci_tiles * p.co_tiles;
    const int split = bid / tiles;
    bid -= split * tiles;
    const int ci_tile = bid / p.co_tiles, co_tile = bid - ci_tile * p.co_tiles;
    const int ci0 = ci_tile * RK_CI, co0 = co_tile * RK_CO;
    const int pbeg = split * p.patches_per_split;
    int pend = pbeg + p.patches_per_split;
    if (pend > p.total_patches) pend = p.total_patches;
    const int nsteps = pend > pbeg ? pend - pbeg : 0;

    const bool two_x = wave + 8 < X_PIECES;
    int x_iy[2], x_ix[2], x_cb[2];
    bool x_ok[2], g_ok[2];
#pragma unroll
    for (int k = 0; k < 2; ++k) {
        const int R = 8 * (wave + 8 * k) + (lane >> 3);
        const int iy = R / XW, ix = R - iy * XW;
        const int c = (lane & 7) ^ (2 * ((ix >> 1) & 3));
        x_ok[k] = R < XW * XW && ci0 + c * 8 < p.Cin;
        x_iy[k] = x_ok[k] ? iy : 0;
        x_ix[k] = ix;
        x_cb[k] = c * 16;
    }
    int g_ry[2], g_rx[2], g_cb[2];
#pragma unroll
    for (int k = 0; k < 2; ++k) {
        const int R = 4 * (wave + 8 * k) + (lane >> 4);
        const int pos = lane & 15;
        const int c = 2 * ((pos >> 1) ^ (R & 7)) + (pos & 1);
        g_ok[k] = co0 + c * 8 < p.Cout;
        g_ry[k] = R >> 3;
        g_rx[k] = R & 7;
        g_cb[k] = c * 16;
    }
    const unsigned lds0 = __builtin_amdgcn_readfirstlane((unsigned)reinterpret_cast<uintptr_t>((lds_void_rk_t*)smem));
    const __amdgpu_buffer_rsrc_t x_rsrc = __builtin_amdgcn_make_buffer_rsrc(const_cast<bf16_raw*>(p.x), 0, p.x_bytes, 0x00020000);
    const __amdgpu_buffer_rsrc_t g_rsrc = __builtin_amdgcn_make_buffer_rsrc(const_cast<bf16_raw*>(p.g), 0, p.g_bytes, 0x00020000);

    int c_n = 0, c_s = 0, c_by = 0, c_bx = 0, c_rows = 1;
    RSeg sg = p.seg[0];
    int x_vec[2], g_vec[2];
    unsigned x_in[2], g_in[2];
    auto level_vectors = [&]() {
#pragma unroll
        for (int k = 0; k < 2; ++k) {
            x_vec[k] = ((x_iy[k] * sg.Wi + x_ix[k]) * p.Cin) * 2 + x_cb[k];
            g_vec[k] = ((g_ry[k] * sg.W + g_rx[k]) * p.Cout) * 2 + g_cb[k];
            x_in[k] = x_ok[k] ? (unsigned)x_vec[k] : X_NONE;
            g_in[k] = g_ok[k] ? (unsigned)g_vec[k] : X_NONE;
        }
    };
    auto seek = [&](int pid) {
        c_n = pid / p.patches_per_img;
        const int rem = pid - c_n * p.patches_per_img;
        c_s = 0;
#pragma unroll
        for (int k = 1; k < BD_MAX_SEGS; ++k)
            if (k < p.nseg && rem >= p.seg[k].patch_start) c_s = k;
        sg = p.seg[c_s];
        const int local = rem - sg.patch_start;
        c_by = local / sg.pw; c_bx = local - c_by * sg.pw;
        c_rows = (sg.H + 7) >> 3;
        level_vectors();
    };
    auto advance = [&]() {
        if (++c_bx < sg.pw) return;
        c_bx = 0;
        if (++c_by < c_rows) return;
        c_by = 0;
        if (p.nseg == 1) { ++c_n; return; }
        if (++c_s == p.nseg) { c_s = 0; ++c_n; }
        sg = p.seg[c_s];
        c_rows = (sg.H + 7) >> 3;
        level_vectors();
    };
    bool in_loop = false;
    auto issue_x = [&](int stage, bool dead) {
        if ((BD_RK_ABLATE & 2) && in_loop) return;
        const unsigned Xs = lds0 + stage * STAGE + wave * 1024;
        const int ys = c_by * 8 - 1, xs = c_bx * 8 - 1;
        const int xorg = ((c_n * p.in_ppi + sg.in_off + ys * sg.Wi + xs) * p.Cin + ci0) * 2;
        if (!dead && ys >= 0 && xs >= 0 && ys + XW <= sg.Hi && xs + XW <= sg.Wi) {
#pragma unroll
            for (int k = 0; k < 2; ++k) {
                if (k == 1 && (!two_x || (BD_RK_ABLATE & 4))) break;
                rk_dma16(x_rsrc, Xs + k * 8192, x_in[k], xorg);
            }
            return;
        }
#pragma unroll
        for (int k = 0; k < 2; ++k) {
            if (k == 1 && (!two_x || (BD_RK_ABLATE & 4))) break;
            const bool ok = !dead & x_ok[k] & ((unsigned)(ys + x_iy[k]) < (unsigned)sg.Hi) & ((unsigned)(xs + x_ix[k]) < (unsigned)sg.Wi);
            rk_dma16(x_rsrc, Xs + k * 8192, ok ? (unsigned)(xorg + x_vec[k]) : X_NONE);
        }
    };
    auto issue_g = [&](int stage, bool dead) {
        if ((BD_RK_ABLATE & 2) && in_loop) return;
        const unsigned Gs = lds0 + stage * STAGE + X_BYTES + wave * 1024;
        const int y0 = c_by * 8, x0 = c_bx * 8;
        const int gorg = ((c_n * p.out_ppi + sg.out_off + y0 * sg.W + x0) * p.Cout + co0) * 2;
        if (!dead && y0 + 8 <= sg.H && x0 + 8 <= sg.W) {
#pragma unroll
            for (int k = 0; k < 2; ++k) rk_dma16(g_rsrc, Gs + k * 8192, g_in[k], gorg);
            return;
        }
#pragma unroll
        for (int k = 0; k < 2; ++k) {
            const bool ok = !dead & g_ok[k] & (y0 + g_ry[k] < sg.H) & (x0 + g_rx[k] < sg.W);
            rk_dma16(g_rsrc, Gs + k * 8192, ok ? (unsigned)(gorg + g_vec[k]) : X_NONE);
        }
    };

    const int g4 = lane >> 4, idx = lane & 15;
    const int tr_q = idx >> 2, tr_p = idx & 3;
    const int prow_hi = 2 * (g4 >> 1);
    const int pcol = 4 * (g4 & 1) + tr_q;
    int xa[3], ga[4];
#pragma unroll
    for (int s = 0; s < 3; ++s)
        xa[s] = (prow_hi * XW + pcol + s) * 128 + ((wi ^ (((pcol + s) >> 1) & 3)) * 32) + tr_p * 8;
#pragma unroll
    for (int j = 0; j < 4; ++j)
        ga[j] = X_BYTES + (prow_hi * 8 + pcol) * 256 + (((4 * wo + j) ^ pcol) * 32) + tr_p * 8;

    typedef __attribute__((ext_vector_type(8))) short s16x8_t;
    auto tr_frag = [&](const unsigned char* a0, int hi_bytes) -> bf16x8_t {
        const s16x4_t lo = __builtin_amdgcn_ds_read_tr16_b64_v4i16((__attribute__((address_space(3))) s16x4_t*)(a0));
        const s16x4_t hi = __builtin_amdgcn_ds_read_tr16_b64_v4i16((__attribute__((address_space(3))) s16x4_t*)(a0 + hi_bytes));
        const s16x8_t v = {lo[0], lo[1], lo[2], lo[3], hi[0], hi[1], hi[2], hi[3]};
        return __builtin_bit_cast(bf16x8_t, v);
    };

    f32x4_t acc[9][4];
#pragma unroll
    for (int t = 0; t < 9; ++t)
#pragma unroll
        for (int j = 0; j < 4; ++j) acc[t][j] = (f32x4_t){0.f, 0.f, 0.f, 0.f};
    f32x4_t cacc = {0.f, 0.f, 0.f, 0.f};
    const bool do_cs = p.csum != nullptr && ci_tile == 0;
    bf16x8_t ones;
    {
        const s16x8_t o = {0x3f80, 0x3f80, 0x3f80, 0x3f80, 0x3f80, 0x3f80, 0x3f80, 0x3f80};
        ones = __builtin_bit_cast(bf16x8_t, o);
    }

    typedef __attribute__((ext_vector_type(8))) int i32x8_t;
    typedef __attribute__((ext_vector_type(4))) int i32x4_t;
    typedef __attribute__((ext_vector_type(2))) int i32x2_t;
    i32x8_t xr[3];
    bf16x8_t fb[4];
    auto tr64 = [&](const unsigned char* a0) -> i32x2_t {
        const s16x4_t v = __builtin_amdgcn_ds_read_tr16_b64_v4i16((__attribute__((address_space(3))) s16x4_t*)(a0));
        return __builtin_bit_cast(i32x2_t, v);
    };
    auto load_half = [&](int stage, int kk) {
        const unsigned char* base = smem + stage * STAGE;
#pragma unroll
        for (int j = 0; j < 4; ++j) fb[j] = tr_frag(base + ga[j] + (4 * kk * 8) * 256, 8 * 256);
#pragma unroll
        for (int sx = 0; sx < 3; ++sx) {
            const unsigned char* b0 = base + xa[sx] + (4 * kk * XW) * 128;
            const i32x2_t r0 = tr64(b0), r1 = tr64(b0 + XW * 128), r2 = tr64(b0 + 2 * XW * 128), r3 = tr64(b0 + 3 * XW * 128);
            xr[sx] = (i32x8_t){r0[0], r0[1], r1[0], r1[1], r2[0], r2[1], r3[0], r3[1]};
        }
    };
    auto mfma_taps = [&](int t0, int t1, bool with_bias) {
#pragma unroll
        for (int t = t0; t < t1; ++t) {
            const int r = t / 3, sx = t - 3 * (t / 3);
            const i32x4_t w = r == 0 ? __builtin_shufflevector(xr[sx], xr[sx], 0, 1, 2, 3)
                                     : (r == 1 ? __builtin_shufflevector(xr[sx], xr[sx], 2, 3, 4, 5) : __builtin_shufflevector(xr[sx], xr[sx], 4, 5, 6, 7));
            const bf16x8_t a = __builtin_bit_cast(bf16x8_t, w);
#pragma unroll
            for (int j = 0; j < 4; ++j)
                acc[t][j] = __builtin_amdgcn_mfma_f32_16x16x32_bf16(a, fb[j], acc[t][j], 0, 0, 0);
        }
        if (with_bias && do_cs) {
            if (wi == 0) cacc = __builtin_amdgcn_mfma_f32_16x16x32_bf16(ones, fb[0], cacc, 0, 0, 0);
            else if (wi == 1) cacc = __builtin_amdgcn_mfma_f32_16x16x32_bf16(ones, fb[1], cacc, 0, 0, 0);
            else if (wi == 2) cacc = __builtin_amdgcn_mfma_f32_16x16x32_bf16(ones, fb[2], cacc, 0, 0, 0);
            else cacc = __builtin_amdgcn_mfma_f32_16x16x32_bf16(ones, fb[3], cacc, 0, 0, 0);
        }
    };
#define RK_BARRIER() do { asm volatile("" ::: "memory"); __builtin_amdgcn_s_barrier(); asm volatile("" ::: "memory"); } while (0)
#define RK_FENCE() __builtin_amdgcn_sched_barrier(0)

#if defined(BD_PP_PRIO) && BD_PP_PRIO == 1
    if (wave >= 4) __builtin_amdgcn_s_setprio(1);
#endif
    if (nsteps > 0) {
        seek(pbeg);
#pragma unroll 1
        for (int d = 0; d < DEPTH; ++d) {
            issue_x(d, d >= nsteps);
            issue_g(d, d >= nsteps);
            advance();
        }
        if (two_x) asm volatile("s_waitcnt vmcnt(8)" ::: "memory");
        else asm volatile("s_waitcnt vmcnt(6)" ::: "memory");
        RK_BARRIER();
        if (wo == 1) RK_BARRIER();
        RK_FENCE();
        in_loop = true;
        int stage = 0, fill = DEPTH;
#ifdef BD_RK_STAMP
        unsigned long long st[4] = {0, 0, 0, 0};
        const unsigned long long st_begin = __builtin_amdgcn_s_memtime(), st_rbegin = __builtin_amdgcn_s_memrealtime();
        unsigned long long last__ = st_begin;
#define RK_T(i) do { const unsigned long long now__ = __builtin_amdgcn_s_memtime(); st[i] += now__ - last__; last__ = now__; } while (0)
#else
#define RK_T(i) do { } while (0)
#endif
#pragma unroll 1
        for (int t = 0; t < nsteps; ++t) {
            const bool dead = t + DEPTH >= nsteps;
#pragma unroll
            for (int kk = 0; kk < 2; ++kk) {
                if (!((BD_RK_ABLATE & 1) && kk == 1)) load_half(stage, kk);
                RK_FENCE();
                if (kk == 0) {
                    issue_x(fill, dead);
                } else {
                    if (BD_RK_ABLATE & 6) { }
                    else if (two_x) asm volatile("s_waitcnt vmcnt(6)" ::: "memory");
                    else asm volatile("s_waitcnt vmcnt(4)" ::: "memory");
                    issue_g(fill, dead);
                    advance();
                }
                RK_FENCE();
                RK_T(0);
                RK_BARRIER();
                RK_T(1);
                asm volatile("s_waitcnt lgkmcnt(0)" ::: "memory");
                RK_FENCE();
#if defined(BD_PP_PRIO) && BD_PP_PRIO == 0
                __builtin_amdgcn_s_setprio(1);
#endif
                mfma_taps(0, 9, true);
#if defined(BD_PP_PRIO) && BD_PP_PRIO == 0
                __builtin_amdgcn_s_setprio(0);
#endif
                RK_FENCE();
                RK_T(2);
                RK_BARRIER();
                RK_FENCE();
                RK_T(3);
            }
            stage = stage + 1 == NSTAGE ? 0 : stage + 1;
            fill = fill + 1 == NSTAGE ? 0 : fill + 1;
        }
        if (wo == 0) RK_BARRIER();
#ifdef BD_RK_STAMP
        if (blockIdx.x == 100 % gridDim.x && lane == 0) {
            for (int k = 0; k < 4; ++k) g_rk_stamp[wave][k] = st[k];
            g_rk_stamp[wave][4] = (unsigned long long)nsteps;
            g_rk_stamp[wave][5] = __builtin_amdgcn_s_memtime() - st_begin;
            g_rk_stamp[wave][6] = __builtin_amdgcn_s_memrealtime() - st_rbegin;
        }
#endif
    }

    float* out = p.slab + ((size_t)(wg * 8 + wave) * REGS) * 256 + lane * 4;
#pragma unroll
    for (int t = 0; t < 9; ++t)
#pragma unroll
        for (int j = 0; j < 4; ++j) *reinterpret_cast<f32x4_t*>(out + (t * 4 + j) * 256) = acc[t][j];
    if (do_cs && g4 == 0) {
        const int co = co0 + wo * 64 + wi * 16 + idx;
        if (co < p.Cout) p.csum[(size_t)split * p.Cout + co] = cacc[0];
    }
    if (blockIdx.x == 0 && threadIdx.x == 0) bd_clk_mark(g_rk_clk, true);
}

struct RPlan { int ci_tiles, co_tiles, tiles, splits, total, ppi, per; };

RPlan ring_plan(const bd_conv_desc* d) {
    RPlan pl;
    pl.ppi = 0;
    for (int s = 0; s < d->nseg; ++s) pl.ppi += cdiv(d->Ho[s], 8) * cdiv(d->Wo[s], 8);
    pl.total = pl.ppi * d->N;
    pl.ci_tiles = cdiv(d->Cin, RK_CI);
    pl.co_tiles = cdiv(d->Cout, RK_CO);
    pl.tiles = pl.ci_tiles * pl.co_tiles;
    static const int target_env = bd_tune_env("BD_WGRAD3R_TARGET", 0);
    const int target = target_env > 0 ? target_env : bd_num_cus();
    int splits = target / pl.tiles;
    if (splits < 1) splits = 1;
    const int max_splits = pl.total / 8 > 0 ? pl.total / 8 : 1;
    if (splits > max_splits) splits = max_splits;
    pl.per = cdiv(pl.total, splits);
    pl.splits = cdiv(pl.total, pl.per);
    return pl;
}

}

int bd_rk_clk_read(unsigned long long* out2, int reset) {
    if (hipMemcpyFromSymbol(out2, HIP_SYMBOL(g_rk_clk), 16) != hipSuccess) return 1;
    if (reset) { const unsigned long long z[2] = {0, 0}; if (hipMemcpyToSymbol(HIP_SYMBOL(g_rk_clk), z, 16) != hipSuccess) return 1; }
    return 0;
}

#ifdef BD_RK_STAMP
extern "C" int bd_debug_rk_stamp(unsigned long long* out64) {
    return hipMemcpyFromSymbol(out64, HIP_SYMBOL(g_rk_stamp), sizeof(g_rk_stamp)) == hipSuccess ? 0 : 1;
}
#endif

bool bd_wgrad3x3r_eligible(const bd_conv_desc* d) {
    if (!(d->R == 3 && d->S == 3 && d->stride == 1 && d->pad == 1)) return false;
    if (d->Cin < 64 || d->Cout < 96 || d->Cin % 8 || d->Cout % 8) return false;
    if ((long long)d->N * d->in_pix_per_img * d->Cin * 2 >= 0x7fffffffll || (long long)d->N * d->out_pix_per_img * d->Cout * 2 >= 0x7fffffffll)
        return false;
    for (int s = 0; s < d->nseg; ++s)
        if (d->Hi[s] != d->Ho[s] || d->Wi[s] != d->Wo[s]) return false;
    return true;
}

size_t bd_wgrad3x3r_slab_bytes(const bd_conv_desc* d, int* splits_out) {
    const RPlan pl = ring_plan(d);
    if (splits_out) *splits_out = pl.splits;
    return (size_t)pl.splits * pl.tiles * 8 * REGS * 1024;
}

int bd_wgrad3x3r_launch(const bd_conv_desc* d, const void* x, const void* g, float* slab, float* csum, int* splits_out, hipStream_t stream) {
    RParams p{};
    const RPlan pl = ring_plan(d);
    p.x = (const bf16_raw*)x; p.g = (const bf16_raw*)g; p.slab = slab; p.csum = csum;
    p.Cin = d->Cin; p.Cout = d->Cout; p.N = d->N; p.nseg = d->nseg;
    p.in_ppi = d->in_pix_per_img; p.out_ppi = d->out_pix_per_img;
    p.x_bytes = (unsigned)((long long)d->N * d->in_pix_per_img * d->Cin * 2);
    p.g_bytes = (unsigned)((long long)d->N * d->out_pix_per_img * d->Cout * 2);
    p.total_patches = pl.total; p.patches_per_img = pl.ppi; p.patches_per_split = pl.per;
    p.ci_tiles = pl.ci_tiles; p.co_tiles = pl.co_tiles;
    int ps = 0;
    for (int s = 0; s < d->nseg; ++s) {
        RSeg& sg = p.seg[s];
        sg.patch_start = ps; sg.H = d->Ho[s]; sg.W = d->Wo[s]; sg.pw = cdiv(d->Wo[s], 8);
        sg.in_off = d->in_off[s]; sg.out_off = d->out_off[s]; sg.Hi = d->Hi[s]; sg.Wi = d->Wi[s];
        ps += cdiv(d->Ho[s], 8) * sg.pw;
    }
    BD_ONCE_PER_DEVICE(
        (void)hipFuncSetAttribute(reinterpret_cast<const void*>(&conv_wgrad3x3_ring_kernel), hipFuncAttributeMaxDynamicSharedMemorySize, LDS_BYTES));
    hipLaunchKernelGGL(conv_wgrad3x3_ring_kernel, dim3(pl.splits * pl.tiles), dim3(512), LDS_BYTES, stream, p);
    *splits_out = pl.splits;
    return 0;
}

void bd_wgrad3x3r_entry(const bd_conv_desc* d, BdRedEntry* e) {
    const RPlan pl = ring_plan(d);
    e->kind = 1; e->regs = REGS; e->co_tiles = pl.co_tiles; e->tci = RK_CI; e->tco = RK_CO; e->fi = 0; e->fj = 0;
    e->Cin = d->Cin; e->Cout = d->Cout; e->n4 = 8 * REGS * 64 * pl.tiles; e->row_len = 0;
}
```

### basedet_amd/models/engine.py

```python
import numpy as np
import torch

from .. import ops
from ..ops import Geom

BN_EPS = 1e-5


class ParamArena:

    def __init__(self, device):
        self.device = device
        self.entries = []
        self.total = 0
        self.w = self.g = self.v = None

    def reserve(self, name, shape):
        n = int(np.prod(shape))
        off = self.total
        self.entries.append((name, tuple(shape), off, n))
        self.total += (n + 63) // 64 * 64
        return len(self.entries) - 1

    def allocate(self):
        self.w = torch.zeros(self.total, dtype=torch.float32, device=self.device)
        self.g = torch.zeros(self.total, dtype=torch.float32, device=self.device)
        self.v = torch.zeros(self.total, dtype=torch.float32, device=self.device)

    def view(self, which, idx):
        _, shape, off, n = self.entries[idx]
        return getattr(self, which)[off:off + n].view(shape)


class ConvLayer:

    def __init__(self, name, cin, cout, k, stride, pad, device, bn_prefix=None, has_bias=False, trainable=True,
                 cout_pad=None):
        self.name, self.cin, self.cout_real, self.k, self.stride, self.pad = name, cin, cout, k, stride, pad
        self.cout = cout_pad or cout
        self.bn_prefix, self.has_bias, self.trainable = bn_prefix, has_bias, trainable
        self.device = device
        self.w = self.b = self.gw = self.gb = None
        self.row_scale = None
        self.w_fwd = torch.empty((self.cout, k * k, cin), dtype=torch.bfloat16, device=device)
        self.w_dgrad = torch.empty((cin, k * k, self.cout), dtype=torch.bfloat16, device=device) if trainable else None
        self._desc_cache = {}
        self.fp8 = False
        self.fp8_dgrad = False
        self.fp8_wgrad = False
        self.fp8_1x1 = False
        self.fp8_1x1_dgrad = False
        self.w_q8 = self.w_scale8 = self.w_q8t = self.w_scale8t = None
        self.act_scale = 1.0
        self.grad_scale = 4096.0
        self.amax_slot = None
        self.probe_ctl = None
        self.q8_scratch = None

    def bind(self, arena, params):
        w = torch.from_numpy(params[self.name + ".weight"]).permute(0, 2, 3, 1).contiguous()
        if self.cout != self.cout_real:
            pad = torch.zeros((self.cout - self.cout_real,) + tuple(w.shape[1:]))
            w = torch.cat([w, pad], 0)
        if self.trainable:
            self.w = arena.view("w", self._wi); self.gw = arena.view("g", self._wi)
            self.w.copy_(w)
        else:
            self.w = w.to(self.device)
        if self.bn_prefix:
            g, b = params[self.bn_prefix + ".weight"], params[self.bn_prefix + ".bias"]
            m, v = params[self.bn_prefix + ".running_mean"], params[self.bn_prefix + ".running_var"]
            scale = g / np.sqrt(v + BN_EPS)
            self.row_scale = torch.from_numpy(scale.astype(np.float32)).to(self.device)
            self.b = torch.from_numpy((b - m * scale).astype(np.float32)).to(self.device)
        elif self.has_bias:
            b = torch.from_numpy(params[self.name + ".bias"])
            if self.cout != self.cout_real:
                b = torch.cat([b, torch.zeros(self.cout - self.cout_real)])
            if self.trainable:
                self.b = arena.view("w", self._bi); self.gb = arena.view("g", self._bi)
                self.b.copy_(b)
            else:
                self.b = b.to(self.device)

    def reserve(self, arena):
        if not self.trainable:
            return
        self._wi = arena.reserve(self.name + ".weight", (self.cout, self.k, self.k, self.cin))
        if self.has_bias:
            self._bi = arena.reserve(self.name + ".bias", (self.cout,))

    def export(self, out):
        out[self.name + ".weight"] = self.w[: self.cout_real].permute(0, 3, 1, 2).contiguous().cpu().numpy()
        if self.has_bias and not self.bn_prefix:
            out[self.name + ".bias"] = self.b[: self.cout_real].cpu().numpy().copy()

    def export_grad(self, out):
        out[self.name + ".weight"] = self.gw[: self.cout_real].permute(0, 3, 1, 2).contiguous().cpu()
        if self.gb is not None:
            out[self.name + ".bias"] = self.gb[: self.cout_real].cpu().clone()

    def enable_fp8(self, q8_scratch, act_scale=1.0, dgrad=False, grad_scale=4096.0, wgrad=False):
        assert self.cin % 16 == 0 and self.cout % 8 == 0
        self.fp8, self.q8_scratch, self.act_scale = True, q8_scratch, float(act_scale)
        self.w_q8 = torch.empty((self.cout, self.k * self.k, self.cin), dtype=torch.uint8, device=self.device)
        self.w_scale8 = torch.empty((self.cout,), dtype=torch.float32, device=self.device)
        if wgrad and self.trainable and self.k == 3 and self.stride == 1 and self.cin % 16 == 0 and self.cout % 16 == 0:
            self.fp8_wgrad, self.grad_scale = True, float(grad_scale)
        if dgrad and self.trainable and self.k == 3 and self.stride == 1 and self.cin > 128 and self.cout % 16 == 0:
            self.fp8_dgrad, self.grad_scale = True, float(grad_scale)
            self.w_q8t = torch.empty((self.cin, self.k * self.k, self.cout), dtype=torch.uint8, device=self.device)
            self.w_scale8t = torch.empty((self.cin,), dtype=torch.float32, device=self.device)

    def enable_fp8_1x1(self, act_scale=1.0, dgrad=False, grad_scale=4096.0, expanding=True):
        assert self.k == 1 and self.stride == 1 and self.cin % 32 == 0 and self.cout % 32 == 0
        self.act_scale, self.grad_scale = float(act_scale), float(grad_scale)
        if self.cin % 128 == 0 and (self.cin >= 2 * self.cout or expanding):
            self.fp8_1x1 = True
            self.w_q8 = torch.empty((self.cout, 1, self.cin), dtype=torch.uint8, device=self.device)
            self.w_scale8 = torch.empty((self.cout,), dtype=torch.float32, device=self.device)
        if dgrad and self.trainable and self.cout % 128 == 0 and (self.cout >= 2 * self.cin or expanding):
            self.fp8_1x1_dgrad = True
            self.w_q8t = torch.empty((self.cin, 1, self.cout), dtype=torch.uint8, device=self.device)
            self.w_scale8t = torch.empty((self.cin,), dtype=torch.float32, device=self.device)

    def pack_fp8(self):
        if self.k == 1 and (self.fp8_1x1 or self.fp8_1x1_dgrad):
            if self.fp8_1x1:
                ops.weight_pack_fp8(self.w, self.row_scale, self.cout, 1, self.cin, self.act_scale, self.w_q8, self.w_scale8)
            if self.fp8_1x1_dgrad:
                ops.weight_pack_fp8_t(self.w, self.row_scale, self.cout, 1, self.cin, self.grad_scale, self.w_q8t, self.w_scale8t)
            return
        ops.weight_pack_fp8(self.w, self.row_scale, self.cout, self.k * self.k, self.cin, self.act_scale, self.w_q8, self.w_scale8)
        if self.fp8_dgrad:
            ops.weight_pack_fp8_t(self.w, self.row_scale, self.cout, self.k * self.k, self.cin, self.grad_scale, self.w_q8t, self.w_scale8t)

    def pack(self):
        ops.weight_pack(self.w, self.row_scale, self.w_fwd, self.w_dgrad, self.cout, self.k * self.k, self.cin)
        if self.fp8 or self.fp8_1x1 or self.fp8_1x1_dgrad:
            self.pack_fp8()

    def desc(self, gin: Geom, gout: Geom):
        key = (gin.N, tuple(gin.H), tuple(gin.W), tuple(gin.off), gin.pix_per_img,
               tuple(gout.H), tuple(gout.W), tuple(gout.off), gout.pix_per_img)
        d = self._desc_cache.get(key)
        if d is None:
            d = ops.conv_desc(gin, gout, self.cin, self.cout, self.k, self.k, self.stride, self.pad)
            self._desc_cache[key] = d
        return d

    def forward(self, x, gin, gout, y, add=None, relu=False, bits=None, x8=None, y8=None, q_scale=1.0):
        flags = (ops.EPI_RELU if relu else 0) | (ops.EPI_ADD_BEFORE if add is not None else 0)
        if self.fp8_1x1 and x8 is not None and ops.conv1x1_fp8_ok(self.desc(gin, gout), 0):
            return ops.conv1x1_fp8(self.desc(gin, gout), 0, x8, self.w_q8, self.w_scale8, self.b, y, add=add, bits=bits, y8=y8,
                                   q_scale=q_scale, flags=flags)
        if self.fp8 and bits is None:
            xq = x8 if x8 is not None else ops.quantize_fp8(x, self.act_scale, self.q8_scratch(x.numel())[: x.numel()])
            return ops.conv2d_fwd_fp8(self.desc(gin, gout), xq, self.w_q8, self.w_scale8, self.b, y, add=add, flags=flags, y8=y8,
                                      q_scale=self.act_scale)
        return ops.conv2d_fwd(self.desc(gin, gout), x, self.w_fwd, self.b, y, add=add, flags=flags, bits=bits,
                              y8=y8 if (y8 is not None and ops.dense_1x1_bits_ok(self.desc(gin, gout))) else None, q_scale=q_scale)

    def gnstats_ok(self):
        return (not self.fp8) and self.k == 3 and self.stride == 1 and self.pad == 1 and self.cout == 256 and self.cin % 64 == 0

    def forward_gnstats(self, x, gin, gout, y, part):
        return ops.conv2d_fwd_gnstats(self.desc(gin, gout), x, self.w_fwd, self.b, y, part)

    def dgrad(self, g, gin, gout, dx, first=True, mask=None, add_after=None, maskbits=None, g8=None, dx8=None, q_scale=1.0,
              add_before=None, sparse=False):
        flags, add = 0, None
        if add_after is not None:
            flags |= ops.EPI_ADD_AFTER
            add = add_after
        elif add_before is not None:
            flags |= ops.EPI_ADD_BEFORE
            add = add_before
        elif not first:
            flags |= ops.EPI_ADD_BEFORE
            add = dx
            if sparse and self.stride > 1:
                flags |= ops.EPI_SPARSE
        if mask is not None or maskbits is not None:
            flags |= ops.EPI_MASK
        if maskbits is not None:
            mask = None
        d = self.desc(gin, gout)
        if self.amax_slot is not None and self.probe_ctl[0] and (self.fp8_1x1_dgrad or self.fp8_dgrad):
            ops.absmax_bf16(g, self.amax_slot)
        if self.fp8_1x1_dgrad and g8 is not None and ops.conv1x1_fp8_ok(d, 1):
            ops.conv1x1_fp8(d, 1, g8, self.w_q8t, self.w_scale8t, None, dx, add=add, mask=mask, maskbits=maskbits, y8=dx8,
                            q_scale=q_scale, flags=flags)
            return dx8 is not None
        if self.fp8_dgrad and maskbits is None:
            gq = g8 if g8 is not None else ops.quantize_bf8(g, self.grad_scale, self.q8_scratch(g.numel())[: g.numel()])
            ops.conv2d_dgrad_fp8(d, gq, self.w_q8t, self.w_scale8t, dx, add=add, mask=mask, flags=flags, dx8=dx8, q_scale=q_scale)
            return dx8 is not None
        if dx8 is not None and not ops.dense_1x1_bits_ok(d):
            dx8 = None
        ops.conv2d_dgrad(d, g, self.w_dgrad, dx, add=add, mask=mask, flags=flags, maskbits=maskbits, dx8=dx8, q_scale=q_scale)
        return dx8 is not None

    def dgrad_writes_twin(self, gin, gout):
        return self.fp8_dgrad or ops.dense_1x1_bits_ok(self.desc(gin, gout))

    def wgrad(self, x, g, gin, gout, ws, colsum_ws=None, x8=None, g8=None, queue=None):
        d = self.desc(gin, gout)
        if self.fp8_wgrad and x8 is not None and g8 is not None:
            ops.conv2d_wgrad_fp8(d, x8, g8, 1.0 / (self.act_scale * self.grad_scale), self.gw, ws, row_scale=self.row_scale)
            if self.gb is not None:
                ops.colsum_bf16(g, g.shape[0], self.cout, self.gb, colsum_ws)
            return
        if queue is not None:
            queue.wgrad(d, x, g, self.gw, self.gb, ws, row_scale=self.row_scale)
        elif self.gb is not None:
            ops.conv2d_wgrad_bias(d, x, g, self.gw, self.gb, ws, row_scale=self.row_scale)
        else:
            ops.conv2d_wgrad(d, x, g, self.gw, ws, row_scale=self.row_scale)

    def thin_backward_ok(self, gin: Geom):
        return (self.k == 1 and self.stride == 1 and self.pad == 0 and self.cin == 256 and self.cout == 16 and self.trainable
                and self.row_scale is None and self.gb is not None and not (self.fp8 or self.fp8_1x1)
                and sum(h * w for h, w in zip(gin.H, gin.W)) == gin.pix_per_img)

    def thin_forward(self, x, gin: Geom, y):
        ops.conv1x1_thin_fwd(x, self.w, self.b, gin.pixels, self.cin, self.cout, y)

    def thin_backward(self, x, g, gin: Geom, dx, ws):
        ops.conv1x1_thin_bwd(x, g, self.w, gin.pixels, self.cin, self.cout, dx, self.gw, self.gb, self.cout_real, ws)

    def wgrad_ws_bytes(self, gin, gout):
        d = self.desc(gin, gout)
        n = ops.conv2d_wgrad_bias_workspace_bytes(d) if self.gb is not None else ops.conv2d_wgrad_workspace_bytes(d)
        return max(n, ops.conv2d_wgrad_fp8_workspace_bytes(d)) if self.fp8_wgrad else n


class FusedPredConv(ConvLayer):

    def __init__(self, name, parts, cin, k, stride, pad, device, cout_pad):
        self.parts = parts
        super().__init__(name, cin, sum(c for _, c in parts), k, stride, pad, device, has_bias=True, trainable=True, cout_pad=cout_pad)

    def bind(self, arena, params):
        merged = dict(params)
        merged[self.name + ".weight"] = np.concatenate([params[n + ".weight"] for n, _ in self.parts], 0)
        merged[self.name + ".bias"] = np.concatenate([params[n + ".bias"] for n, _ in self.parts], 0)
        super().bind(arena, merged)

    def export(self, out):
        o = 0
        for n, c in self.parts:
            out[n + ".weight"] = self.w[o:o + c].permute(0, 3, 1, 2).contiguous().cpu().numpy()
            out[n + ".bias"] = self.b[o:o + c].cpu().numpy().copy()
            o += c

    def export_grad(self, out):
        o = 0
        for n, c in self.parts:
            out[n + ".weight"] = self.gw[o:o + c].permute(0, 3, 1, 2).contiguous().cpu()
            out[n + ".bias"] = self.gb[o:o + c].cpu().clone()
            o += c


class FCLayer(ConvLayer):

    def __init__(self, name, cin, cout, device, in_chw=None, parts=None, cout_pad=None):
        self.in_chw = in_chw
        self.parts = parts
        super().__init__(name, cin, cout, 1, 1, 0, device, has_bias=True, trainable=True, cout_pad=cout_pad)

    def _names(self):
        return [n for n, _ in self.parts] if self.parts else [self.name]

    def _to_ours(self, w):
        if self.in_chw:
            c, h, wd = self.in_chw
            w = w.reshape(-1, c, h, wd).permute(0, 2, 3, 1).reshape(-1, c * h * wd)
        return w.contiguous()

    def _to_ref(self, w):
        if self.in_chw:
            c, h, wd = self.in_chw
            w = w.reshape(-1, h, wd, c).permute(0, 3, 1, 2).reshape(-1, c * h * wd)
        return w.contiguous()

    def bind(self, arena, params):
        w = np.concatenate([np.asarray(params[n + ".weight"], np.float32) for n in self._names()], 0)
        b = np.concatenate([np.asarray(params[n + ".bias"], np.float32) for n in self._names()], 0)
        w = self._to_ours(torch.from_numpy(w)).numpy().reshape(self.cout_real, self.cin, 1, 1)
        super().bind(arena, {self.name + ".weight": w, self.name + ".bias": b})

    def _split(self, w, b, out, to_numpy):
        w = self._to_ref(w[: self.cout_real].reshape(self.cout_real, self.cin))
        b = b[: self.cout_real]
        o = 0
        for n, c in (self.parts or [(self.name, self.cout_real)]):
            wn, bn = w[o:o + c].cpu(), b[o:o + c].cpu()
            out[n + ".weight"] = wn.numpy().copy() if to_numpy else wn.clone()
            out[n + ".bias"] = bn.numpy().copy() if to_numpy else bn.clone()
            o += c

    def export(self, out):
        self._split(self.w, self.b, out, True)

    def export_grad(self, out):
        self._split(self.gw, self.gb, out, False)


class DeconvLayer(ConvLayer):

    def __init__(self, name, ch, device):
        super().__init__(name, ch, ch, 4, 2, 1, device)
        self.ch = ch
        self.w_fwd = torch.empty((4, ch, 4, ch), dtype=torch.bfloat16, device=device)
        self.w_dgrad = torch.empty((ch, 16, ch), dtype=torch.bfloat16, device=device)

    def pack(self):
        ops.fpn_deconv_pack(self.w, self.ch, self.w_fwd, self.w_dgrad)

    def forward(self, x, gc: Geom, y, add=None):
        return ops.fpn_deconv_fwd(x, self.w_fwd, y, gc.N, gc.H[0], gc.W[0], self.ch, add=add)

    def dgrad(self, dy, gc: Geom, dx, add=None):
        return ops.fpn_deconv_dgrad(dy, self.w_dgrad, dx, gc.N, gc.H[0], gc.W[0], self.ch, add=add)

    def wgrad(self, x, g, gin, gout, ws, colsum_ws=None, x8=None, g8=None, queue=None):
        ops.fpn_deconv_wgrad(x, g, self.gw, ws, gout.N, gout.H[0], gout.W[0], self.ch)

    def wgrad_ws_bytes(self, gin, gout):
        return ops.fpn_deconv_wgrad_workspace_bytes(gout.N, gout.H[0], gout.W[0], self.ch)
```

### basedet_amd/models/retinanet.py

```python
import math

import numpy as np
import torch
from contextlib import nullcontext as _nullcontext

from .. import ops
from ..utils.registry import registers
from . import params as P
from .fpn_base import FPNDetector, _round_up


@registers.models.register()
class RetinaNet(FPNDetector):
    @staticmethod
    def init_params(cfg, seed=0):
        return P.init_retinanet_params(cfg, seed)

    @classmethod
    def check_config(cls, cfg):
        super().check_config(cfg)
        if not cfg.MODEL.HEAD.get("WITH_NORM", True):
            raise ValueError("MODEL.HEAD.WITH_NORM = False is not supported for the RetinaNet family: only True (the default) is implemented")

    def _build_head(self, add, params):
        m = self.cfg.MODEL
        dev = self.device
        ch = self.fpn_ch
        self.num_anchors = len(m.ANCHOR.SCALES[0]) * len(m.ANCHOR.RATIOS[0])
        nc = m.HEAD.NUM_CONVS
        self.cls_tower = [add(f"head.cls_subnet.{2 * i}", ch, ch, 3, 1, 1, bias=True) for i in range(nc)]
        self.box_tower = [add(f"head.bbox_subnet.{2 * i}", ch, ch, 3, 1, 1, bias=True) for i in range(nc)]
        A, K = self.num_anchors, self.num_classes
        self.cls_score = add("head.cls_score", ch, A * K, 3, 1, 1, bias=True)
        self.box_ld = _round_up(A * 4, 8)
        self.bbox_pred = add("head.bbox_pred", ch, A * 4, 3, 1, 1, bias=True, cout_pad=self.box_ld)
        scales = np.asarray(m.ANCHOR.SCALES, np.float32).tolist()
        ratios = np.asarray(m.ANCHOR.RATIOS, np.float32).tolist()
        if len(ratios) == 1:
            ratios = ratios * len(self.strides)
        if len(scales) == 1:
            scales = scales * len(self.strides)
        self.base_anchors = []
        for sc_, ra_ in zip(scales, ratios):
            base = []
            for s_ in sc_:
                area = float(s_) ** 2.0
                for r_ in ra_:
                    w = math.sqrt(area / float(r_)); h = float(r_) * w
                    base.append([-w / 2.0, -h / 2.0, w / 2.0, h / 2.0])
            self.base_anchors.append(torch.tensor(base, dtype=torch.float32, device=dev))

    def _head_convs(self):
        return self.cls_tower + self.box_tower + [self.cls_score, self.bbox_pred]

    def _plan_head(self, pl):
        dev = self.device
        ch = self.fpn_ch
        N = pl.N
        sizes = pl.sizes
        bf = dict(dtype=torch.bfloat16, device=dev)

        def act(g, c):
            return torch.empty((g.pixels, c), **bf)

        nc = len(self.cls_tower)
        pl.cls_act = [act(pl.pyr, ch) for _ in range(nc)]
        pl.box_act = [act(pl.pyr, ch) for _ in range(nc)]
        A, K = self.num_anchors, self.num_classes
        pl.logits = act(pl.pyr, A * K)
        pl.offsets = act(pl.pyr, self.box_ld)
        pl.d_logits = torch.empty_like(pl.logits)
        pl.d_offsets = torch.empty_like(pl.offsets)
        pl.g_tower = [[act(pl.pyr, ch) for _ in range(nc)] for _ in range(2)]
        tw = lambda: torch.empty((pl.pyr.pixels, ch), dtype=torch.uint8, device=dev)
        pl.cls_act8 = [tw() if c.fp8 else None for c in self.cls_tower]
        pl.box_act8 = [tw() if c.fp8 else None for c in self.box_tower]
        tg = self.fp8_grad_twins
        pl.g_tower8 = [[tw() if (c.fp8_dgrad and tg) else None for c in tower] for tower in (self.cls_tower, self.box_tower)]
        pl.g_P8 = tw() if (tg and all(t[0].fp8_dgrad for t in (self.cls_tower, self.box_tower))) else None
        tot = pl.pyr.pix_per_img * A
        pl.anchors = torch.empty((tot, 4), dtype=torch.float32, device=dev)
        o = 0
        for (h, w), s, base in zip(sizes, self.strides, self.base_anchors):
            n = h * w * A
            ops.anchors_generate(h, w, s, self.cfg.MODEL.ANCHOR.OFFSET, base, pl.anchors[o:o + n])
            o += n
        pl.A_total = tot
        pl.labels = torch.empty((N, tot), dtype=torch.int32, device=dev)
        pl.match_idx = torch.empty((N, tot), dtype=torch.int32, device=dev)
        pl.gt_offsets = torch.empty((N, tot, 4), dtype=torch.float32, device=dev)
        pl.num_fg = torch.zeros((1,), dtype=torch.int32, device=dev)
        pl.loss_buf = torch.zeros((2,), dtype=torch.float32, device=dev)

    def head_forward(self, pl):
        side = None
        if (bool(self.cfg.MODEL.get("HEAD_TOWERS_CONCURRENT", True)) and self.device.type == "cuda" and self.async_wgrad
                and self._tstream is not None and self.weight_dtype != "fp8_e4m3"):
            side = self._tstream
            side.wait_stream(torch.cuda.current_stream())
        with torch.cuda.stream(side) if side is not None else _nullcontext():
            t, t8 = pl.P, getattr(pl, "P8", None)
            for c, a, a8 in zip(self.box_tower, pl.box_act, pl.box_act8):
                c.forward(t, pl.pyr, pl.pyr, a, relu=True, x8=t8, y8=a8); t, t8 = a, a8
            self.bbox_pred.forward(t, pl.pyr, pl.pyr, pl.offsets, x8=t8)
        t, t8 = pl.P, getattr(pl, "P8", None)
        for c, a, a8 in zip(self.cls_tower, pl.cls_act, pl.cls_act8):
            c.forward(t, pl.pyr, pl.pyr, a, relu=True, x8=t8, y8=a8); t, t8 = a, a8
        self.cls_score.forward(t, pl.pyr, pl.pyr, pl.logits, x8=t8)
        if side is not None:
            torch.cuda.current_stream().wait_stream(side)

    def get_losses(self, inputs):
        assert self.training
        pre = self.pre_process(inputs)
        pl = pre["plan"]
        self._cur = pl
        m = self.cfg.MODEL
        gt = pre["gt_boxes"]
        num_gt = pre["img_info"][:, 4].to(torch.int32).contiguous()
        N, Gmax = gt.shape[0], gt.shape[1]
        ws = pl.wgrad_ws[: N * Gmax]
        thr = m.MATCHER.THRESHOLDS
        side = self._tstream if (self.async_wgrad and self._tstream is not None and m.get("ASSIGN_ON_SIDE_STREAM", True)) else None
        if side is not None:
            side.wait_stream(torch.cuda.current_stream())
        with torch.cuda.stream(side) if side is not None else _nullcontext():
            ops.retina_assign_encode(pl.anchors, gt, num_gt, thr[0], thr[1], m.MATCHER.ALLOW_LOW_QUALITY, m.BOX_REG.MEAN,
                                     m.BOX_REG.STD, pl.labels, pl.match_idx, pl.gt_offsets, pl.num_fg, ws)
        self.network_forward(pl)
        if side is not None:
            torch.cuda.current_stream().wait_stream(side)
        pl.loss_buf.zero_()
        rows = N * pl.A_total
        ops.focal_loss_fwd_bwd(pl.logits, pl.labels, rows, self.num_classes, m.LOSSES.FOCAL_LOSS_ALPHA,
                               m.LOSSES.FOCAL_LOSS_GAMMA, pl.num_fg, 1.0, pl.loss_buf[0:1], pl.d_logits)
        ops.smooth_l1_fwd_bwd(pl.offsets, pl.gt_offsets, pl.labels, pl.pyr.pixels, self.num_anchors, self.box_ld,
                              m.LOSSES.SMOOTH_L1_BETA, pl.num_fg, m.LOSSES.REG_LOSS_WEIGHT, pl.loss_buf[1:2], pl.d_offsets)
        cls_loss, reg_loss = pl.loss_buf[0], pl.loss_buf[1]
        return {"total_loss": cls_loss + reg_loss, "cls_loss": cls_loss, "reg_loss": reg_loss}

    def head_backward(self, pl, ws, cws):
        pyr = pl.pyr
        for ti, (tower, acts, pred, dpred) in enumerate(((self.cls_tower, pl.cls_act, self.cls_score, pl.d_logits),
                                                         (self.box_tower, pl.box_act, self.bbox_pred, pl.d_offsets))):
            gbuf, g8 = pl.g_tower[ti], pl.g_tower8[ti]
            n = len(tower)
            gs = tower[n - 1].grad_scale
            self._wgrad(pred, acts[-1], dpred, pyr, pyr, ws, cws)
            tw = g8[n - 1] if pred.dgrad_writes_twin(pyr, pyr) else None
            if not pred.dgrad(dpred, pyr, pyr, gbuf[n - 1], mask=acts[-1], dx8=tw, q_scale=gs):
                tw = None
            act8 = pl.cls_act8 if ti == 0 else pl.box_act8
            for i in range(n - 1, -1, -1):
                x = acts[i - 1] if i > 0 else pl.P
                x8 = (act8[i - 1] if i > 0 else pl.P8) if tw is not None else None
                self._wgrad(tower[i], x, gbuf[i], pyr, pyr, ws, cws, x8=x8, g8=tw)
                if i > 0:
                    nxt = g8[i - 1] if tower[i].dgrad_writes_twin(pyr, pyr) else None
                    wrote = tower[i].dgrad(gbuf[i], pyr, pyr, gbuf[i - 1], mask=acts[i - 1], g8=tw, dx8=nxt, q_scale=tower[i - 1].grad_scale)
                    tw = nxt if wrote else None
                else:
                    wrote_p = tower[i].dgrad(gbuf[i], pyr, pyr, pl.g_P, first=(ti == 0), g8=tw,
                                             dx8=pl.g_P8 if tower[i].dgrad_writes_twin(pyr, pyr) else None,
                                             q_scale=self.output[self.fpn_stages[0]].grad_scale)
        pl.g_P8_ready = pl.g_P8 is not None and bool(wrote_p)

    def _debug_head(self, pl, out, lvl):
        for i in range(pl.pyr.nlev):
            for k in range(len(self.cls_tower)):
                out[f"cls{k}_{i}"] = lvl(pl.cls_act[k], i)
                out[f"box{k}_{i}"] = lvl(pl.box_act[k], i)
            out[f"logits_{i}"] = lvl(pl.logits, i)
            out[f"offs_{i}"] = lvl(pl.offsets, i, self.num_anchors * 4)

    def inference(self, inputs):
        assert not self.training
        pre = self.pre_process(inputs)
        pl = pre["plan"]
        assert pl.N == 1, "inference supports batch size 1 (retinanet.py:174)"
        self.network_forward(pl)
        K, A = self.num_classes, self.num_anchors
        m = self.cfg.MODEL
        rows = pl.pyr.pix_per_img * A
        scores = torch.empty((rows * K,), dtype=torch.float32, device=self.device)
        ops.det_scores(pl.logits, rows, K, scores)
        return self._detect(scores, [h * w * A for h, w in pl.sizes], K, 0, pre["img_info"], anchors=pl.anchors, offsets=pl.offsets,
                            off_ld=self.box_ld, A=A, mean=m.BOX_REG.MEAN, std=m.BOX_REG.STD)
```

### basedet_amd/ops.py

```python
import ctypes as C
from dataclasses import dataclass, field
from typing import List, Optional

import torch

from . import _lib
from ._lib import ConvDesc, EPI_ADD_AFTER, EPI_ADD_BEFORE, EPI_MASK, EPI_RELU, EPI_SPARSE, check, f32arr, i32arr, ptr, stream_ptr


@dataclass
class Geom:
    N: int
    H: List[int]
    W: List[int]
    off: List[int] = field(default_factory=list)
    pix_per_img: int = 0

    def __post_init__(self):
        if not self.off:
            o = 0
            self.off = []
            for h, w in zip(self.H, self.W):
                self.off.append(o)
                o += h * w
            if not self.pix_per_img:
                self.pix_per_img = o
        if not self.pix_per_img:
            self.pix_per_img = sum(h * w for h, w in zip(self.H, self.W))

    @property
    def nlev(self):
        return len(self.H)

    @property
    def pixels(self):
        return self.N * self.pix_per_img

    def level(self, i):
        return Geom(self.N, [self.H[i]], [self.W[i]], [self.off[i]], self.pix_per_img)

    def conv_out(self, R, stride, pad):
        H = [(h + 2 * pad - R) // stride + 1 for h in self.H]
        W = [(w + 2 * pad - R) // stride + 1 for w in self.W]
        return Geom(self.N, H, W)


def single(N, H, W):
    return Geom(N, [H], [W])


def conv_desc(gin: Geom, gout: Geom, Cin, Cout, R, S, stride, pad) -> ConvDesc:
    d = ConvDesc()
    d.N, d.Cin, d.Cout, d.R, d.S, d.stride, d.pad, d.nseg = gin.N, Cin, Cout, R, S, stride, pad, gin.nlev
    assert gin.nlev == gout.nlev <= _lib.BD_MAX_SEGS
    for i in range(gin.nlev):
        d.Hi[i], d.Wi[i], d.Ho[i], d.Wo[i] = gin.H[i], gin.W[i], gout.H[i], gout.W[i]
        d.in_off[i], d.out_off[i] = gin.off[i], gout.off[i]
    d.in_pix_per_img, d.out_pix_per_img = gin.pix_per_img, gout.pix_per_img
    return d


def L():
    return _lib.load()


_ROUTE = [0, 0, 0, 0]
_SR_SEED = [0]
_ROUTE_NAMES = {"dense1x1": 0, "patch3x3": 1, "wgrad": 2, "fp8_patch": 3}


def set_route(**kw):
    for k, v in kw.items():
        _ROUTE[_ROUTE_NAMES[k]] = 0 if v is None else int(v) + 1


def reset_route():
    _ROUTE[:] = [0, 0, 0, 0]
    _SR_SEED[0] = 0


def _stamp(d):
    d.route[0], d.route[1], d.route[2], d.route[3] = _ROUTE
    d.sr_seed = _SR_SEED[0]
    return d


def conv2d_fwd(d, x, w_packed, bias, y, add=None, flags=0, bits=None, y8=None, q_scale=1.0):
    if y8 is not None:
        check(L().bd_conv2d_fwd_ex(C.byref(_stamp(d)), ptr(x), ptr(w_packed), ptr(bias), ptr(add), ptr(y), ptr(bits), ptr(y8), float(q_scale), flags,
                                   stream_ptr()), "bd_conv2d_fwd_ex")
        return y
    if bits is not None:
        check(L().bd_conv2d_fwd_bits(C.byref(_stamp(d)), ptr(x), ptr(w_packed), ptr(bias), ptr(add), ptr(y), ptr(bits), flags, stream_ptr()),
              "bd_conv2d_fwd_bits")
        return y
    check(L().bd_conv2d_fwd(C.byref(_stamp(d)), ptr(x), ptr(w_packed), ptr(bias), ptr(add), ptr(y), flags, stream_ptr()), "bd_conv2d_fwd")
    return y


def conv2d_dgrad(d, g, w_packed_t, dx, add=None, mask=None, flags=0, maskbits=None, dx8=None, q_scale=1.0):
    if dx8 is not None:
        check(L().bd_conv2d_dgrad_ex(C.byref(_stamp(d)), ptr(g), ptr(w_packed_t), ptr(add), ptr(mask), ptr(maskbits), ptr(dx), ptr(dx8),
                                     float(q_scale), flags, stream_ptr()), "bd_conv2d_dgrad_ex")
        return dx
    if maskbits is not None:
        check(L().bd_conv2d_dgrad_bits(C.byref(_stamp(d)), ptr(g), ptr(w_packed_t), ptr(add), ptr(maskbits), ptr(dx), flags, stream_ptr()),
              "bd_conv2d_dgrad_bits")
        return dx
    check(L().bd_conv2d_dgrad(C.byref(_stamp(d)), ptr(g), ptr(w_packed_t), ptr(add), ptr(mask), ptr(dx), flags, stream_ptr()), "bd_conv2d_dgrad")
    return dx


def quantize_fp8(x, scale, q):
    check(L().bd_quantize_fp8(ptr(x), x.numel(), float(scale), ptr(q), stream_ptr()), "bd_quantize_fp8")
    return q


def weight_pack_fp8(w, row_scale, Cout, RS, Cin, act_scale, wq, wscale):
    check(L().bd_weight_pack_fp8(ptr(w), ptr(row_scale), Cout, RS, Cin, float(act_scale), ptr(wq), ptr(wscale), stream_ptr()),
          "bd_weight_pack_fp8")


def conv2d_fwd_fp8(d, xq, wq, wscale, bias, y, add=None, flags=0, y8=None, q_scale=1.0):
    check(L().bd_conv2d_fwd_fp8_ex(C.byref(_stamp(d)), ptr(xq), ptr(wq), ptr(wscale), ptr(bias), ptr(add), ptr(y), ptr(y8), float(q_scale), flags,
                                   stream_ptr()), "bd_conv2d_fwd_fp8")
    return y


def quantize_bf8(x, scale, q):
    check(L().bd_quantize_bf8(ptr(x), x.numel(), float(scale), ptr(q), _SR_SEED[0], stream_ptr()), "bd_quantize_bf8")
    return q


def fp8_set_stochastic_rounding(seed):
    _SR_SEED[0] = int(seed) & 0xFFFFFFFF


def absmax_bf16(x, out):
    check(L().bd_absmax_bf16(ptr(x), x.numel(), ptr(out), stream_ptr()), "bd_absmax_bf16")


def weight_pack_fp8_t(w, row_scale, Cout, RS, Cin, grad_scale, wq_t, wscale_t):
    check(L().bd_weight_pack_fp8_t(ptr(w), ptr(row_scale), Cout, RS, Cin, float(grad_scale), ptr(wq_t), ptr(wscale_t), stream_ptr()),
          "bd_weight_pack_fp8_t")


def conv2d_dgrad_fp8(d, g8, wq_t, wscale_t, dx, add=None, mask=None, flags=0, dx8=None, q_scale=1.0):
    check(L().bd_conv2d_dgrad_fp8(C.byref(_stamp(d)), ptr(g8), ptr(wq_t), ptr(wscale_t), ptr(add), ptr(mask), ptr(dx), ptr(dx8), float(q_scale),
                                  flags, stream_ptr()), "bd_conv2d_dgrad_fp8")
    return dx


def conv1x1_fp8(d, mode, xq, wq, wscale, bias, y, add=None, mask=None, maskbits=None, bits=None, y8=None, q_scale=1.0, flags=0):
    check(L().bd_conv1x1_fp8(C.byref(_stamp(d)), mode, ptr(xq), ptr(wq), ptr(wscale), ptr(bias), ptr(add), ptr(mask), ptr(maskbits), ptr(y),
                             ptr(bits), ptr(y8), float(q_scale), flags, stream_ptr()), "bd_conv1x1_fp8")
    return y


def conv2d_wgrad_fp8_workspace_bytes(d):
    return int(L().bd_conv2d_wgrad_fp8_workspace_bytes(C.byref(_stamp(d))))


def conv2d_wgrad_fp8(d, x8, g8, inv_scale, dw, ws, row_scale=None, accumulate=False):
    check(L().bd_conv2d_wgrad_fp8(C.byref(_stamp(d)), ptr(x8), ptr(g8), float(inv_scale), ptr(row_scale), ptr(dw), int(accumulate), ptr(ws),
                                  ws.numel() * ws.element_size(), stream_ptr()), "bd_conv2d_wgrad_fp8")
    return dw


def conv1x1_fp8_ok(d, mode):
    K, CO = (d.Cin, d.Cout) if mode == 0 else (d.Cout, d.Cin)
    return dense_1x1_bits_ok(d) and K % 128 == 0 and CO % 32 == 0


def fp8_dgrad_ok(d):
    same = all(d.Hi[i] == d.Ho[i] and d.Wi[i] == d.Wo[i] for i in range(d.nseg))
    return d.R == 3 and d.S == 3 and d.stride == 1 and d.pad == 1 and same and d.Cin > 128 and d.Cin % 8 == 0 and d.Cout % 16 == 0


def dense_1x1_bits_ok(d):
    return (d.R == 1 and d.S == 1 and d.stride == 1 and d.pad == 0 and d.nseg == 1 and d.in_off[0] == 0 and d.out_off[0] == 0
            and d.in_pix_per_img == d.Hi[0] * d.Wi[0] and d.out_pix_per_img == d.Ho[0] * d.Wo[0]
            and d.Cin % 32 == 0 and d.Cout % 32 == 0 and d.N * d.in_pix_per_img * max(d.Cin, d.Cout) * 2 < 0x7fffffff)


def conv2d_wgrad_workspace_bytes(d):
    return int(L().bd_conv2d_wgrad_workspace_bytes(C.byref(_stamp(d))))


def conv2d_wgrad(d, x, g, dw, ws, row_scale=None, accumulate=False):
    check(L().bd_conv2d_wgrad(C.byref(_stamp(d)), ptr(x), ptr(g), ptr(row_scale), ptr(dw), int(accumulate), ptr(ws),
                              ws.numel() * ws.element_size(), stream_ptr()), "bd_conv2d_wgrad")
    return dw


def conv2d_wgrad_bias_workspace_bytes(d):
    return int(L().bd_conv2d_wgrad_bias_workspace_bytes(C.byref(_stamp(d))))


def conv2d_wgrad_bias(d, x, g, dw, dbias, ws, row_scale=None, accumulate=False):
    check(L().bd_conv2d_wgrad_bias(C.byref(_stamp(d)), ptr(x), ptr(g), ptr(row_scale), ptr(dw), ptr(dbias), int(accumulate), ptr(ws),
                                   ws.numel() * ws.element_size(), stream_ptr()), "bd_conv2d_wgrad_bias")
    return dw


def fpn_deconv_pack(w, C, w_fwd, w_dgrad):
    check(L().bd_fpn_deconv_pack(ptr(w), C, ptr(w_fwd), ptr(w_dgrad), stream_ptr()), "bd_fpn_deconv_pack")


def fpn_deconv_fwd(x, w_fwd, y, N, Hc, Wc, C, add=None):
    check(L().bd_fpn_deconv_fwd(ptr(x), ptr(w_fwd), ptr(add), ptr(y), N, Hc, Wc, 2 * Hc, 2 * Wc, C, stream_ptr()), "bd_fpn_deconv_fwd")
    return y


def fpn_deconv_dgrad(dy, w_dgrad, dx, N, Hc, Wc, C, add=None):
    check(L().bd_fpn_deconv_dgrad(ptr(dy), ptr(w_dgrad), ptr(add), ptr(dx), N, Hc, Wc, 2 * Hc, 2 * Wc, C, stream_ptr()), "bd_fpn_deconv_dgrad")
    return dx


def fpn_deconv_wgrad_workspace_bytes(N, Hc, Wc, C):
    return int(L().bd_fpn_deconv_wgrad_workspace_bytes(N, Hc, Wc, C))


def fpn_deconv_wgrad(x, dy, dw, ws, N, Hc, Wc, C, accumulate=False):
    check(L().bd_fpn_deconv_wgrad(ptr(x), ptr(dy), ptr(dw), int(accumulate), ptr(ws), ws.numel() * ws.element_size(), N, Hc, Wc,
                                  2 * Hc, 2 * Wc, C, stream_ptr()), "bd_fpn_deconv_wgrad")
    return dw


def stem_conv7x7_fwd(N, H, W, x_halo, w_stem, bias, y):
    check(L().bd_stem_conv7x7_fwd(N, H, W, ptr(x_halo), ptr(w_stem), ptr(bias), ptr(y), stream_ptr()), "bd_stem_conv7x7_fwd")
    return y


def stem_weight_pack(w, row_scale, w_stem):
    check(L().bd_stem_weight_pack(ptr(w), ptr(row_scale), ptr(w_stem), stream_ptr()), "bd_stem_weight_pack")


def weight_pack(w, row_scale, w_fwd, w_dgrad, Cout, RS, Cin):
    check(L().bd_weight_pack(ptr(w), ptr(row_scale), ptr(w_fwd), ptr(w_dgrad), Cout, RS, Cin, stream_ptr()), "bd_weight_pack")


def build_pack_table(entries, device):
    import ctypes as C
    import numpy as np
    from ._lib import PackDesc
    arr = (PackDesc * len(entries))()
    start = 0
    for i, (w, rs, wf, wd, co, r, ci) in enumerate(entries):
        arr[i].w = w.data_ptr()
        arr[i].row_scale = rs.data_ptr() if rs is not None else None
        arr[i].w_fwd = wf.data_ptr() if wf is not None else None
        arr[i].w_dgrad = wd.data_ptr() if wd is not None else None
        arr[i].Cout, arr[i].RS, arr[i].Cin, arr[i].block_start = co, r, ci, start
        start += int(L().bd_weight_pack_blocks(co, r, ci))
    raw = np.frombuffer(bytes(arr), dtype=np.uint8).copy()
    return torch.from_numpy(raw).to(device), len(entries), start


def weight_pack_multi(table):
    t, n, blocks = table
    check(L().bd_weight_pack_multi(ptr(t), n, blocks, stream_ptr()), "bd_weight_pack_multi")


# ... 491 lines not shown
```

### include/basedet_hip.h

```cpp
#ifndef BASEDET_HIP_H
#define BASEDET_HIP_H

#include <stddef.h>
#include <stdint.h>

#ifdef __cplusplus
extern "C" {
#endif

#define BD_OK 0
#define BD_EINVAL (-1)
#define BD_ELAUNCH (-2)
#define BD_EWORKSPACE (-3)

#define BD_MAX_SEGS 8

#define BD_EPI_RELU 1
#define BD_EPI_ADD_BEFORE 2
#define BD_EPI_ADD_AFTER 4
#define BD_EPI_MASK 8
#define BD_EPI_SPARSE 16

typedef void* bd_stream_t;

typedef struct bd_conv_desc {
    int32_t N;
    int32_t Cin, Cout;
    int32_t R, S;
    int32_t stride, pad;
    int32_t nseg;
    int32_t Hi[BD_MAX_SEGS], Wi[BD_MAX_SEGS];
    int32_t Ho[BD_MAX_SEGS], Wo[BD_MAX_SEGS];
    int32_t in_off[BD_MAX_SEGS], out_off[BD_MAX_SEGS];
    int32_t in_pix_per_img, out_pix_per_img;
    int32_t route[4];
    uint32_t sr_seed;
} bd_conv_desc;

const char* bd_last_error_string(void);
int bd_version(void);
const char* bd_conv_last_kernel(void);
int bd_probe_mfma_rate(double seconds, double* tflops_out, double* clock_mhz_out, bd_stream_t stream);

int bd_probe_kernel_clock(const char* kernel, int reset, double* clock_mhz_out, double* busy_ms_out);


int bd_conv2d_fwd(const bd_conv_desc* d, const void* x, const void* w_packed, const float* bias,
                  const void* add, void* y, int flags, bd_stream_t stream);

int bd_conv2d_dgrad(const bd_conv_desc* d, const void* g, const void* w_packed_t, const void* add,
                    const void* mask, void* dx, int flags, bd_stream_t stream);

int bd_conv2d_fwd_bits(const bd_conv_desc* d, const void* x, const void* w_packed, const float* bias, const void* add, void* y,
                       uint32_t* ybits, int flags, bd_stream_t stream);
int bd_conv2d_dgrad_bits(const bd_conv_desc* d, const void* g, const void* w_packed_t, const void* add, const uint32_t* maskbits,
                         void* dx, int flags, bd_stream_t stream);
int bd_conv2d_fwd_ex(const bd_conv_desc* d, const void* x, const void* w_packed, const float* bias, const void* add, void* y,
                     uint32_t* ybits, void* y8, float q_scale, int flags, bd_stream_t stream);
int bd_conv2d_dgrad_ex(const bd_conv_desc* d, const void* g, const void* w_packed_t, const void* add, const void* mask,
                       const uint32_t* maskbits, void* dx, void* dx8, float q_scale, int flags, bd_stream_t stream);

size_t bd_conv2d_wgrad_workspace_bytes(const bd_conv_desc* d);
int bd_conv2d_wgrad(const bd_conv_desc* d, const void* x, const void* g, const float* row_scale, float* dw,
                    int accumulate, void* ws, size_t ws_bytes, bd_stream_t stream);

size_t bd_conv2d_wgrad_bias_workspace_bytes(const bd_conv_desc* d);
int bd_conv2d_wgrad_bias(const bd_conv_desc* d, const void* x, const void* g, const float* row_scale, float* dw, float* dbias,
                         int accumulate, void* ws, size_t ws_bytes, bd_stream_t stream);

typedef struct bd_wgrad_queue* bd_wgrad_queue_t;
int bd_wgrad_queue_create(bd_wgrad_queue_t* out);
int bd_wgrad_queue_destroy(bd_wgrad_queue_t q);
int bd_wgrad_queue_pending(bd_wgrad_queue_t q);
int bd_conv2d_wgrad_queued(bd_wgrad_queue_t q, const bd_conv_desc* d, const void* x, const void* g, const float* row_scale, float* dw,
                           float* dbias, int accumulate, void* ws, size_t ws_bytes, bd_stream_t stream);
int bd_wgrad_queue_flush(bd_wgrad_queue_t q, bd_stream_t stream);



int bd_stem_conv7x7_fwd(int N, int H, int W, const void* x_halo, const void* w_stem, const float* bias,
                        void* y, bd_stream_t stream);
int bd_stem_pool_fwd(int N, int H, int W, const void* x_halo, const void* w_stem, const float* bias, void* y_pool,
                     bd_stream_t stream);
int bd_stem_weight_pack(const float* w , const float* row_scale, void* w_stem,
                        bd_stream_t stream);

int bd_weight_pack(const float* w, const float* row_scale, void* w_fwd, void* w_dgrad, int Cout, int RS,
                   int Cin, bd_stream_t stream);

typedef struct bd_pack_desc {
    const float* w;
    const float* row_scale;
    void* w_fwd;
    void* w_dgrad;
    int32_t Cout, RS, Cin, block_start;
} bd_pack_desc;
int bd_weight_pack_blocks(int Cout, int RS, int Cin);
int bd_weight_pack_multi(const bd_pack_desc* descs_dev, int n, int total_blocks, bd_stream_t stream);

size_t bd_colsum_workspace_bytes(int C);
int bd_colsum_bf16(const void* g, int N, int64_t pix_per_img, int64_t off, int64_t cnt, int C, float* out,
                   int accumulate, void* ws, size_t ws_bytes, bd_stream_t stream);

int bd_bottleneck_fwd_supported(int N, int H, int W, int Cin, int Cmid, int Cout, int has_downsample);
int bd_bottleneck_fwd(int N, int H, int W, int Cin, int Cmid, int Cout, const void* x, const void* w1, const float* b1, const void* w2,
                      const float* b2, const void* w3, const float* b3, const void* wd, const float* bd, void* y, bd_stream_t stream);


int bd_pad_normalize(const float* in, int N, int H, int W, int Hp, int Wp, const float* mean3,
                     const float* std3, void* out, bd_stream_t stream);
typedef struct bd_h2d* bd_h2d_t;
#define BD_HOST_F64 0
#define BD_HOST_F32 1
#define BD_HOST_U8 2
int bd_h2d_create(bd_h2d_t* out, int device, int threads);
int bd_h2d_threads(bd_h2d_t h);
int bd_h2d_submit(bd_h2d_t h, const void* src_host, int src_dtype, int64_t n, float* dst_dev, int64_t chunk_elems, bd_stream_t stream);
int bd_h2d_destroy(bd_h2d_t h);

int bd_pad_normalize_nchw(const float* in, int N, int H, int W, int Hp, int Wp, const float* mean3,
                          const float* std3, float* out, bd_stream_t stream);

int bd_maxpool3x3s2_fwd(const void* x, int N, int H, int W, int C, void* y, bd_stream_t stream);

int bd_upsample2x_add_fwd(const void* top, int64_t top_pix_per_img, int64_t top_off, void* lateral,
                          int64_t lat_pix_per_img, int64_t lat_off, int N, int H, int W, int C,
                          bd_stream_t stream);
int bd_upsample2x_add_bwd(const void* dlat, int64_t lat_pix_per_img, int64_t lat_off, void* dtop,
                          int64_t top_pix_per_img, int64_t top_off, int N, int H, int W, int C,
                          int accumulate, bd_stream_t stream);

int bd_fpn_deconv_pack(const float* w, int C, void* w_fwd, void* w_dgrad, bd_stream_t stream);
int bd_fpn_deconv_fwd(const void* x, const void* w_fwd, const void* add, void* y, int N, int Hc, int Wc, int Hf, int Wf, int C,
                      bd_stream_t stream);
int bd_fpn_deconv_dgrad(const void* dy, const void* w_dgrad, const void* add, void* dx, int N, int Hc, int Wc, int Hf, int Wf, int C,
                        bd_stream_t stream);
size_t bd_fpn_deconv_wgrad_workspace_bytes(int N, int Hc, int Wc, int C);
int bd_fpn_deconv_wgrad(const void* x, const void* dy, float* dw, int accumulate, void* ws, size_t ws_bytes, int N, int Hc, int Wc,
                        int Hf, int Wf, int C, bd_stream_t stream);

int bd_relu_bf16(const void* x, void* y, int64_t n, bd_stream_t stream);
int bd_relu_bwd_bf16(const void* g, const void* mask, const void* add, void* y, int64_t n, bd_stream_t stream);
int bd_add_bf16(const void* a, const void* b, void* y, int64_t n, bd_stream_t stream);


int bd_anchors_generate(int H, int W, int stride, float offset, const float* base, int A, float* out,
                        bd_stream_t stream);
int bd_points_generate(int H, int W, int stride, float offset, int A, float* out, bd_stream_t stream);

int bd_box_pairwise(const float* b1, int m, const float* b2, int n, int mode, float* out, bd_stream_t stream);

int bd_box_encode(const float* anchors, const float* gt, int64_t n, const float* mean4_host,
                  const float* std4_host, float* out, bd_stream_t stream);
int bd_box_decode(const float* anchors, const float* deltas, int64_t n, const float* mean4_host,
                  const float* std4_host, float* out, bd_stream_t stream);

int bd_retina_assign_encode(const float* anchors, int A, const float* gt_boxes, const int32_t* num_gt, int N,
                            int Gmax, float thr_lo, float thr_hi, int allow_low_quality,
                            const float* mean4_host, const float* std4_host, int32_t* labels,
                            int32_t* match_idx, float* offsets, int32_t* num_fg, void* ws, size_t ws_bytes,
                            bd_stream_t stream);

int bd_fcos_assign(const float* points, int P, const int32_t* lvl_start_host, const float* soi_host,
                   const int32_t* strides_host, int L, float radius, const float* gt_boxes,
                   const int32_t* num_gt, int N, int Gmax, int32_t* labels, float* offsets, float* ctrness,
                   float* stats, bd_stream_t stream);

size_t bd_atss_assign_workspace_bytes(int N, int P);
int bd_atss_assign(const float* points, int P, const int32_t* lvl_start_host, const int32_t* strides_host, int L, int topk,
                   float anchor_scale, const float* gt_boxes, const int32_t* num_gt, int N, int Gmax, int32_t* labels,
                   float* offsets, float* ctrness, float* stats, void* ws, size_t ws_bytes, bd_stream_t stream);

size_t bd_ota_assign_workspace_bytes(int N, int P);
int bd_ota_assign(const float* points, int P, const int32_t* lvl_start_host, const int32_t* strides_host, int L, const void* logits,
                  int K, const void* pred_ltrb, const float* gt_boxes, const int32_t* num_gt, int N, int Gmax, float alpha,
                  float gamma, float reg_weight, float center_radius, int candidate_k, int32_t* labels, float* targets,
                  float* gt_ious, float* stats, void* ws, size_t ws_bytes, bd_stream_t stream);

size_t bd_ota_sinkhorn_workspace_bytes(int N, int P, int Gmax);
int bd_ota_assign_sinkhorn(const float* points, int P, const int32_t* lvl_start_host, const int32_t* strides_host, int L,
                           const void* logits, int K, const void* pred_ltrb, const float* gt_boxes, const int32_t* num_gt, int N,
                           int Gmax, float alpha, float gamma, float reg_weight, float center_radius, int topq, float eps, int iters,
                           int32_t* labels, float* targets, float* gt_ious, float* stats, void* ws, size_t ws_bytes,
                           bd_stream_t stream);

size_t bd_freeanchor_workspace_bytes(int N, int Gmax, int bucket, int A);
int bd_freeanchor_loss_fwd_bwd(const void* logits, const void* offsets, int box_ld, int anchors_per_pix, const float* anchors,
                               int A, int K, const float* gt_boxes, const int32_t* num_gt, int N, int Gmax, const float* mean4,
                               const float* std4, float iou_thresh, int bucket, float beta, float reg_weight, float alpha,
                               float gamma, float* loss_out, void* d_logits, void* d_offsets, void* ws, size_t ws_bytes,
                               bd_stream_t stream);

size_t bd_nms_workspace_bytes(int n);
int bd_batched_nms(const float* boxes, const float* scores, const int32_t* idxs, int n, float iou_thresh,
                   int max_output, int32_t* keep, int32_t* num_keep, void* ws, size_t ws_bytes,
                   bd_stream_t stream);


int bd_focal_loss_fwd_bwd(const void* logits, const int32_t* labels, int64_t rows, int K, float alpha,
                          float gamma, const void* norm, int norm_is_float, float grad_scale,
                          float* loss_sum, void* dlogits, bd_stream_t stream);
int bd_focal_loss_fwd_bwd_general(const void* logits, const int32_t* labels, int64_t rows, int K, float alpha,
                                  float gamma, const void* norm, int norm_is_float, float grad_scale,
                                  float* loss_sum, void* dlogits, bd_stream_t stream);
// ... 191 lines not shown
```

Before: 639.4 images/sec.

## Skip zero-gradient patches in RetinaNet box-branch 3x3 dgrad and wgrad

Adds a gradient-sparsity scan that marks spatial patches whose output gradient is all zero, compacts the live patches into a list, and runs sparse variants of the 3x3 dgrad and ring wgrad kernels that only visit live patches (and their halo neighbours). Dead dgrad outputs are zeroed explicitly unless the result accumulates in place. It is enabled by default for the box tower and bbox_pred, whose regression-loss gradients are zero away from positive anchors. The cost is extra scan and compaction launches, a single-block compaction kernel, and per-descriptor scratch buffers; the tail-split scheduling is disabled on the sparse path.

Result: faster. 679.4 images/sec (median of 6 runs) (+6.3%).

```diff
diff --git a/basedet_amd/_lib.py b/basedet_amd/_lib.py
--- a/basedet_amd/_lib.py
+++ b/basedet_amd/_lib.py
@@ -23,6 +23,7 @@
         ("in_off", C.c_int32 * BD_MAX_SEGS), ("out_off", C.c_int32 * BD_MAX_SEGS),
         ("in_pix_per_img", C.c_int32), ("out_pix_per_img", C.c_int32),
         ("route", C.c_int32 * 4), ("sr_seed", C.c_uint32),
+        ("gskip", C.c_int32), ("gskip_ws", C.c_void_p), ("gskip_ws_bytes", C.c_size_t),
     ]
 
 
@@ -42,6 +43,7 @@
     "bd_probe_kernel_clock": (_I, [C.c_char_p, _I, C.POINTER(C.c_double), C.POINTER(C.c_double)]),
     "bd_conv2d_fwd": (_I, [_D, _P, _P, _P, _P, _P, _I, _P]),
     "bd_conv2d_dgrad": (_I, [_D, _P, _P, _P, _P, _P, _I, _P]),
+    "bd_conv2d_dgrad_gskip_bytes": (_Z, [_D]),
     "bd_conv2d_fwd_bits": (_I, [_D, _P, _P, _P, _P, _P, _P, _I, _P]),
     "bd_conv2d_fwd_ex": (_I, [_D, _P, _P, _P, _P, _P, _P, _P, _F, _I, _P]),
     "bd_conv2d_dgrad_ex": (_I, [_D, _P, _P, _P, _P, _P, _P, _P, _F, _I, _P]),
diff --git a/basedet_amd/build.py b/basedet_amd/build.py
--- a/basedet_amd/build.py
+++ b/basedet_amd/build.py
@@ -16,6 +16,7 @@
     "conv_igemm.hip": [],
     "conv3x3.hip": [],
     "conv3x3_pp.hip": [],
+    "gskip.hip": [],
     "conv3x3_pp128.hip": [],
     "conv1x1.hip": [],
     "conv1x1_ring.hip": [],
diff --git a/basedet_amd/csrc/conv3x3_pp.hip b/basedet_amd/csrc/conv3x3_pp.hip
--- a/basedet_amd/csrc/conv3x3_pp.hip
+++ b/basedet_amd/csrc/conv3x3_pp.hip
@@ -37,6 +37,10 @@
     float inv_ppi;
     PSeg seg[MAX_SEG];
     float* gn_part;
+    const int* sp_live;
+    const int* sp_list;
+    const int* sp_count;
+    int sp_keep_dead;
 };
 
 typedef __attribute__((address_space(3))) void lds_void_t;
@@ -64,15 +68,15 @@
 #define PP_FENCE() __builtin_amdgcn_sched_barrier(0)
 #define PP_BARRIER() do { asm volatile("" ::: "memory"); __builtin_amdgcn_s_barrier(); asm volatile("" ::: "memory"); } while (0)
 
-template <int MODE, bool GNS = false>
+template <int MODE, bool GNS = false, bool SPARSE = false>
 __global__ __launch_bounds__(512, 1) void conv3x3_pp_kernel(const PParams p) {
     extern __shared__ __attribute__((aligned(16))) unsigned char smem[];
-    if ((int)blockIdx.x >= p.main_grid) {
+    if (!SPARSE && (int)blockIdx.x >= p.main_grid) {
         pp128::body<MODE, TAIL_CO>(p, smem, (int)blockIdx.x - p.main_grid, (int)gridDim.x - p.main_grid, p.total_patches, p.tail_end,
                                    (p.CO + TAIL_CO - 1) / TAIL_CO);
         return;
     }
-    if (blockIdx.x == 0 && threadIdx.x == 0) bd_clk_mark(g_pp_clk, false);
+    if (!SPARSE && blockIdx.x == 0 && threadIdx.x == 0) bd_clk_mark(g_pp_clk, false);
     unsigned char* wbuf = smem;
     unsigned char* xbuf = smem + W_BYTES;
     float* sbias = reinterpret_cast<float*>(smem + W_BYTES + X_BYTES);
@@ -100,6 +104,48 @@
     const int pt_step = p.main_grid / p.n_tiles;
     const int co0 = ct * TILE_CO;
 
+    auto zero_dead = [&](int z0, int zn) {
+        if (p.sp_keep_dead) return;
+        const int cpp = p.CO >> 3;
+        const int items = PH * PW * cpp;
+        for (int k0 = 0; z0 + k0 * zn < p.total_patches; k0 += 512) {
+            const int k = k0 + wave * 64 + lane;
+            const int q = z0 + k * zn;
+            const bool dead = q < p.total_patches && p.sp_live[q] == 0;
+            unsigned long long m = __ballot(dead);
+            while (m) {
+                const int l = __builtin_ctzll(m);
+                m &= m - 1;
+                const int qq = z0 + (k0 + wave * 64 + l) * zn;
+                const int n = qq / p.patches_per_img, rem = qq - n * p.patches_per_img;
+                int sgi = 0;
+#pragma unroll
+                for (int z = 1; z < MAX_SEG; ++z)
+                    if (z < p.nseg && rem >= p.seg[z].patch_start) sgi = z;
+                const int H = p.seg[sgi].H, W = p.seg[sgi].W, pwn = p.seg[sgi].pw;
+                const int local = rem - p.seg[sgi].patch_start, by = local / pwn, bx = local - by * pwn;
+                const long long img = (long long)n * p.dst_ppi + p.seg[sgi].dst_off;
+                for (int i = lane; i < items; i += 64) {
+                    const int px = i / cpp, ch = i - px * cpp;
+                    const int y = by * PH + px / PW, x = bx * PW + (px & (PW - 1));
+                    if (y < H && x < W)
+                        *reinterpret_cast<u32x4_t*>(p.dst + (img + (long long)y * W + x) * p.CO + ch * 8) = (u32x4_t){0u, 0u, 0u, 0u};
+                }
+            }
+        }
+    };
+    int n_px = p.px_tiles, n_live = p.total_patches;
+    int z_first = 0;
+    if constexpr (SPARSE) {
+        n_live = __builtin_amdgcn_readfirstlane(*p.sp_count);
+        n_px = (n_live + NPATCH - 1) / NPATCH;
+        z_first = n_px * p.n_tiles < p.main_grid ? n_px * p.n_tiles : p.main_grid;
+        if (pt >= n_px) {
+            zero_dead(bid - z_first, p.main_grid - z_first);
+            return;
+        }
+    }
+
     constexpr unsigned X_NONE = 0x80000000u;
     const int x_lds0 = (tid >> 3) * X_PITCH + xpos(tid & 7);
     unsigned x_off[XPASSES];
@@ -109,9 +155,10 @@
     auto build_table = [&](int k0) {
         const int k = k0 + (lane >> 2);
         const int ptile = pt_first + k * pt_step;
-        const int pid = ptile * NPATCH + (lane & (NPATCH - 1));
+        int pid = ptile * NPATCH + (lane & (NPATCH - 1));
+        if (SPARSE) pid = (ptile < n_px && pid < n_live) ? p.sp_list[pid] : p.total_patches;
         int vH = 0, vW = 0, vy = 0, vx = 0, vs = 0, vd = 0;
-        if (ptile < p.px_tiles && pid < p.total_patches) {
+        if (ptile < n_px && pid < p.total_patches) {
             const int n = pp_div(pid, p.patches_per_img, p.inv_ppi);
             const int rem = pid - n * p.patches_per_img;
             int g_start = p.seg[0].patch_start, g_H = p.seg[0].H, g_W = p.seg[0].W, g_pw = p.seg[0].pw;
@@ -280,7 +327,7 @@
 #endif
     for (;;) {
     const int pt_next = pt + pt_step;
-    const bool more = pt_next < p.px_tiles;
+    const bool more = pt_next < n_px;
     int n_oy0 = 0, n_px0 = 0, n_H = 0, n_W = 0, n_dst = 0;
 #pragma unroll
     for (int i = 0; i < 8; ++i)
@@ -545,7 +592,10 @@
     PP_FENCE();
     PP_STAMP();
     }
-    if (blockIdx.x == 0 && threadIdx.x == 0) bd_clk_mark(g_pp_clk, true);
+    if constexpr (SPARSE) {
+        if (z_first == p.main_grid) zero_dead(bid, p.main_grid);
+    }
+    if (!SPARSE && blockIdx.x == 0 && threadIdx.x == 0) bd_clk_mark(g_pp_clk, true);
 #ifdef BD_PP_STAMP
     if (st_on) { g_pp_stamp[63] = __builtin_amdgcn_s_memrealtime(); g_pp_stamp[61] = __builtin_amdgcn_s_memtime(); }
     if (threadIdx.x == 0 && blockIdx.x < 1024) { asm volatile("s_waitcnt vmcnt(0)" ::: "memory"); g_pp_span[2 * blockIdx.x + 1] = __builtin_amdgcn_s_memrealtime(); }
@@ -557,6 +607,15 @@
 BD_KNOB int g_pp_tail_split = 1;
 BD_KNOB int g_pp_persistent = 1;
 extern BD_KNOB int g_patch_pp;
+int bd_gskip_patches(const bd_conv_desc* d, int ph, int pw);
+void bd_gskip_scan(const bd_conv_desc* d, const void* g, int ph, int pw, int* mask, hipStream_t stream);
+void bd_gskip_compact(const bd_conv_desc* d, int ph, int pw, const int* mask, int* live, int* list, int* count, hipStream_t stream);
+
+extern "C" size_t bd_conv2d_dgrad_gskip_bytes(const bd_conv_desc* d) {
+    if (!d || d->nseg < 1 || d->nseg > BD_MAX_SEGS || !(d->R == 3 && d->S == 3 && d->stride == 1 && d->pad == 1)) return 0;
+    return ((size_t)3 * bd_gskip_patches(d, PH, PW) + 4) * sizeof(int);
+}
+
 static int pp_launch(const bd_conv_desc* d, int mode, const void* src, const void* w, const float* bias, const void* add,
                      const void* mask, void* dst, int flags, float* gn_part, hipStream_t stream) {
     PParams p{};
@@ -590,7 +649,10 @@
     int px_tiles = cdiv(p.total_patches, NPATCH);
     p.tail_end = p.total_patches;
     const int num_cus = bd_num_cus();
-    if (g_pp_tail_split && !gn_part && p.n_tiles == 1 && px_tiles > num_cus) {
+    const bool in_place = (flags & BD_EPI_ADD_BEFORE) && add && add == dst;
+    const bool sparse = mode == 1 && d->gskip && !gn_part && !(flags & BD_EPI_ADD_AFTER) &&
+                        (!((flags & BD_EPI_ADD_BEFORE) && add) || (in_place && !(flags & BD_EPI_MASK)));
+    if (g_pp_tail_split && !sparse && !gn_part && p.n_tiles == 1 && px_tiles > num_cus) {
         const int r = px_tiles % num_cus;
         if (r > 0 && r * (TILE_CO / TAIL_CO) <= num_cus) {
             px_tiles -= r;
@@ -611,9 +673,19 @@
     }
     BD_ONCE_PER_DEVICE(
         (void)hipFuncSetAttribute(reinterpret_cast<const void*>(&conv3x3_pp_kernel<0>), hipFuncAttributeMaxDynamicSharedMemorySize, LDS_BYTES);
-        (void)hipFuncSetAttribute(reinterpret_cast<const void*>(&conv3x3_pp_kernel<1>), hipFuncAttributeMaxDynamicSharedMemorySize, LDS_BYTES));
+        (void)hipFuncSetAttribute(reinterpret_cast<const void*>(&conv3x3_pp_kernel<1>), hipFuncAttributeMaxDynamicSharedMemorySize, LDS_BYTES);
+        (void)hipFuncSetAttribute(reinterpret_cast<const void*>(&conv3x3_pp_kernel<1, false, true>), hipFuncAttributeMaxDynamicSharedMemorySize,
+                                  LDS_BYTES));
     bd_note_kernel("conv3x3_pp_kernel");
-    if (gn_part) {
+    if (sparse) {
+        int* mk = (int*)d->gskip_ws;
+        const int tot = p.total_patches;
+        p.sp_live = mk + tot; p.sp_list = mk + 2 * tot; p.sp_count = mk + 3 * tot;
+        p.sp_keep_dead = in_place ? 1 : 0;
+        bd_gskip_scan(d, src, PH, PW, mk, stream);
+        bd_gskip_compact(d, PH, PW, mk, mk + tot, mk + 2 * tot, mk + 3 * tot, stream);
+        hipLaunchKernelGGL((conv3x3_pp_kernel<1, false, true>), dim3(p.main_grid), dim3(512), LDS_BYTES, stream, p);
+    } else if (gn_part) {
         BD_ONCE_PER_DEVICE((void)hipFuncSetAttribute(reinterpret_cast<const void*>(&conv3x3_pp_kernel<0, true>), hipFuncAttributeMaxDynamicSharedMemorySize, LDS_BYTES));
         hipLaunchKernelGGL((conv3x3_pp_kernel<0, true>), dim3(p.main_grid), dim3(512), LDS_BYTES, stream, p);
     } else if (mode == 0) hipLaunchKernelGGL((conv3x3_pp_kernel<0>), dim3(p.main_grid + tail_wgs), dim3(512), LDS_BYTES, stream, p);
diff --git a/basedet_amd/csrc/conv_igemm.hip b/basedet_amd/csrc/conv_igemm.hip
--- a/basedet_amd/csrc/conv_igemm.hip
+++ b/basedet_amd/csrc/conv_igemm.hip
@@ -556,6 +556,11 @@
                              const unsigned* maskbits, void* dx, void* dx8, float q_scale, int flags, bd_stream_t stream) {
     if (int e = check_desc(d)) return e;
     BD_REQUIRE(g && w_packed_t && dx, "conv2d_dgrad: null pointer");
+    if (d->gskip && is_3x3s1(d)) {
+        const size_t need = bd_conv2d_dgrad_gskip_bytes(d);
+        BD_REQUIRE(d->gskip_ws && d->gskip_ws_bytes >= need, "conv2d_dgrad: gskip scratch %zu < required %zu bytes (or NULL)",
+                   (size_t)d->gskip_ws_bytes, need);
+    }
     if (d->stride == 1) flags &= ~BD_EPI_SPARSE;
     BD_REQUIRE(d->Cout % 8 == 0, "conv2d_dgrad: Cout=%d must be a multiple of 8 (pad the gradient)", d->Cout);
     BD_REQUIRE(d->Cin % 8 == 0, "conv2d_dgrad: Cin=%d must be a multiple of 8", d->Cin);
diff --git a/basedet_amd/csrc/conv_wgrad.hip b/basedet_amd/csrc/conv_wgrad.hip
--- a/basedet_amd/csrc/conv_wgrad.hip
+++ b/basedet_amd/csrc/conv_wgrad.hip
@@ -323,7 +323,10 @@
 int bd_wgrad3x3_launch(const bd_conv_desc* d, const void* x, const void* g, float* slab, float* csum, int* splits_out, hipStream_t stream);
 bool bd_wgrad3x3r_eligible(const bd_conv_desc* d);
 size_t bd_wgrad3x3r_slab_bytes(const bd_conv_desc* d, int* splits_out);
-int bd_wgrad3x3r_launch(const bd_conv_desc* d, const void* x, const void* g, float* slab, float* csum, int* splits_out, hipStream_t stream);
+int bd_wgrad3x3r_launch(const bd_conv_desc* d, const void* x, const void* g, float* slab, float* csum, const int* gflags, int* splits_out,
+                        hipStream_t stream);
+int bd_wgrad3x3r_gskip_patches(const bd_conv_desc* d);
+void bd_gskip_scan(const bd_conv_desc* d, const void* g, int ph, int pw, int* mask, hipStream_t stream);
 void bd_wgrad3x3r_entry(const bd_conv_desc* d, BdRedEntry* e);
 bool bd_wgrad1x1r_eligible(const bd_conv_desc* d);
 size_t bd_wgrad1x1r_slab_bytes(const bd_conv_desc* d, int* splits_out);
@@ -344,10 +347,25 @@
     launch_batch(&e, 1, stream);
 }
 
+namespace {
+size_t align256(size_t v) { return (v + 255) & ~size_t(255); }
+int gskip_patches(const bd_conv_desc* d) {
+    return d->gskip && bd_wgrad3x3r_eligible(d) ? bd_wgrad3x3r_gskip_patches(d) : 0;
+}
+size_t wgrad_ws_base(const bd_conv_desc* d);
+}
+
 extern "C" size_t bd_conv2d_wgrad_workspace_bytes(const bd_conv_desc* d) {
     BdRouteScope rs__(d);
     if (rs__.rc != BD_OK) return 0;
     if (!d || d->nseg < 1 || d->nseg > BD_MAX_SEGS) return 0;
+    const size_t base = wgrad_ws_base(d);
+    const int gp = gskip_patches(d);
+    return gp > 0 ? align256(base) + (size_t)gp * sizeof(int) : base;
+}
+
+namespace {
+size_t wgrad_ws_base(const bd_conv_desc* d) {
     const Plan pl = make_plan(d);
     size_t splits = (size_t)pl.splits;
     if (is_3x3s1(d)) {
@@ -369,9 +387,6 @@
     }
     return bytes;
 }
-
-namespace {
-size_t align256(size_t v) { return (v + 255) & ~size_t(255); }
 }
 
 extern "C" size_t bd_colsum_workspace_bytes(int C);
@@ -493,7 +508,12 @@
     if (g_wgrad_use_3x3 && g_wgrad_use_ring && bd_wgrad3x3r_eligible(d)) {
         int splitsr = 1;
         bd_note_kernel("conv_wgrad3x3_ring_kernel");
-        bd_wgrad3x3r_launch(d, x, g, (float*)ws, dbias ? (float*)extra : nullptr, &splitsr, (hipStream_t)stream);
+        int* gflags = nullptr;
+        if (gskip_patches(d) > 0) {
+            gflags = (int*)((unsigned char*)ws + align256(wgrad_ws_base(d)));
+            bd_gskip_scan(d, g, 8, 8, gflags, (hipStream_t)stream);
+        }
+        bd_wgrad3x3r_launch(d, x, g, (float*)ws, dbias ? (float*)extra : nullptr, gflags, &splitsr, (hipStream_t)stream);
         BD_CHECK_LAUNCH("bd_conv2d_wgrad(3x3 ring)");
         BdRedEntry e{};
         bd_wgrad3x3r_entry(d, &e);
diff --git a/basedet_amd/csrc/conv_wgrad3x3_ring.hip b/basedet_amd/csrc/conv_wgrad3x3_ring.hip
--- a/basedet_amd/csrc/conv_wgrad3x3_ring.hip
+++ b/basedet_amd/csrc/conv_wgrad3x3_ring.hip
@@ -16,6 +16,7 @@
 constexpr int LDS_BYTES = NSTAGE * STAGE;
 constexpr int REGS = 36;
 constexpr unsigned X_NONE = 0x80000000u;
+constexpr int LIST_MAX = 3072;
 
 typedef __attribute__((address_space(3))) void lds_void_rk_t;
 
@@ -26,6 +27,7 @@
     const bf16_raw* g;
     float* slab;
     float* csum;
+    const int* gflags;
     int Cin, Cout, N, nseg;
     int in_ppi, out_ppi;
     unsigned x_bytes, g_bytes;
@@ -47,6 +49,7 @@
     asm volatile("s_mov_b32 m0, %1\n\ts_nop 0\n\tbuffer_load_dwordx4 %0, %2, %3 offen lds" : : "v"(voff), "s"(lds_addr), "s"(rsrc), "s"(soff) : "memory");
 }
 
+template <bool SPARSE>
 __global__ __launch_bounds__(512) void conv_wgrad3x3_ring_kernel(const RParams p) {
     extern __shared__ __attribute__((aligned(16))) unsigned char smem[];
     const int tid = threadIdx.x, lane = tid & 63, wave = __builtin_amdgcn_readfirstlane(tid >> 6);
@@ -67,7 +70,30 @@
     const int pbeg = split * p.patches_per_split;
     int pend = pbeg + p.patches_per_split;
     if (pend > p.total_patches) pend = p.total_patches;
-    const int nsteps = pend > pbeg ? pend - pbeg : 0;
+    int nsteps = pend > pbeg ? pend - pbeg : 0;
+    int* live_list = reinterpret_cast<int*>(smem + LDS_BYTES);
+    if constexpr (SPARSE) {
+        __shared__ int wsum[8];
+        int base = 0;
+        for (int c0 = 0; c0 < nsteps; c0 += 512) {
+            const int i = c0 + tid;
+            const bool lv = i < nsteps && p.gflags[pbeg + i] != 0;
+            const unsigned long long bal = __ballot(lv);
+            const int pre = __popcll(bal & ((1ull << lane) - 1ull));
+            if (lane == 0) wsum[wave] = __popcll(bal);
+            __syncthreads();
+            int off = base, tot = 0;
+#pragma unroll
+            for (int w = 0; w < 8; ++w) {
+                off += w < wave ? wsum[w] : 0;
+                tot += wsum[w];
+            }
+            if (lv) live_list[off + pre] = i;
+            base += tot;
+            __syncthreads();
+        }
+        nsteps = base;
+    }
 
     const bool two_x = wave + 8 < X_PIECES;
     int x_iy[2], x_ix[2], x_cb[2];
@@ -123,7 +149,12 @@
         c_rows = (sg.H + 7) >> 3;
         level_vectors();
     };
+    int c_li = 0;
     auto advance = [&]() {
+        if constexpr (SPARSE) {
+            if (++c_li < nsteps) seek(pbeg + __builtin_amdgcn_readfirstlane(live_list[c_li]));
+            return;
+        }
         if (++c_bx < sg.pw) return;
         c_bx = 0;
         if (++c_by < c_rows) return;
@@ -250,7 +281,7 @@
     if (wave >= 4) __builtin_amdgcn_s_setprio(1);
 #endif
     if (nsteps > 0) {
-        seek(pbeg);
+        seek(SPARSE ? pbeg + __builtin_amdgcn_readfirstlane(live_list[0]) : pbeg);
 #pragma unroll 1
         for (int d = 0; d < DEPTH; ++d) {
             issue_x(d, d >= nsteps);
@@ -384,9 +415,16 @@
     return (size_t)pl.splits * pl.tiles * 8 * REGS * 1024;
 }
 
-int bd_wgrad3x3r_launch(const bd_conv_desc* d, const void* x, const void* g, float* slab, float* csum, int* splits_out, hipStream_t stream) {
+int bd_wgrad3x3r_gskip_patches(const bd_conv_desc* d) {
+    const RPlan pl = ring_plan(d);
+    return pl.per <= LIST_MAX ? pl.total : 0;
+}
+
+int bd_wgrad3x3r_launch(const bd_conv_desc* d, const void* x, const void* g, float* slab, float* csum, const int* gflags, int* splits_out,
+                        hipStream_t stream) {
     RParams p{};
     const RPlan pl = ring_plan(d);
+    p.gflags = gflags;
     p.x = (const bf16_raw*)x; p.g = (const bf16_raw*)g; p.slab = slab; p.csum = csum;
     p.Cin = d->Cin; p.Cout = d->Cout; p.N = d->N; p.nseg = d->nseg;
     p.in_ppi = d->in_pix_per_img; p.out_ppi = d->out_pix_per_img;
@@ -402,8 +440,14 @@
         ps += cdiv(d->Ho[s], 8) * sg.pw;
     }
     BD_ONCE_PER_DEVICE(
-        (void)hipFuncSetAttribute(reinterpret_cast<const void*>(&conv_wgrad3x3_ring_kernel), hipFuncAttributeMaxDynamicSharedMemorySize, LDS_BYTES));
-    hipLaunchKernelGGL(conv_wgrad3x3_ring_kernel, dim3(pl.splits * pl.tiles), dim3(512), LDS_BYTES, stream, p);
+        (void)hipFuncSetAttribute(reinterpret_cast<const void*>(&conv_wgrad3x3_ring_kernel<false>), hipFuncAttributeMaxDynamicSharedMemorySize,
+                                  LDS_BYTES);
+        (void)hipFuncSetAttribute(reinterpret_cast<const void*>(&conv_wgrad3x3_ring_kernel<true>), hipFuncAttributeMaxDynamicSharedMemorySize,
+                                  LDS_BYTES + LIST_MAX * 4));
+    if (gflags && pl.per <= LIST_MAX)
+        hipLaunchKernelGGL(conv_wgrad3x3_ring_kernel<true>, dim3(pl.splits * pl.tiles), dim3(512), LDS_BYTES + LIST_MAX * 4, stream, p);
+    else
+        hipLaunchKernelGGL(conv_wgrad3x3_ring_kernel<false>, dim3(pl.splits * pl.tiles), dim3(512), LDS_BYTES, stream, p);
     *splits_out = pl.splits;
     return 0;
 }
diff --git a/basedet_amd/csrc/gskip.hip b/basedet_amd/csrc/gskip.hip
--- /dev/null
+++ b/basedet_amd/csrc/gskip.hip
@@ -0,0 +1,164 @@
+#include "common.h"
+
+namespace {
+
+enum { GS_ANY = 1, GS_TOP = 2, GS_BOT = 4, GS_LEFT = 8, GS_RIGHT = 16, GS_TL = 32, GS_TR = 64, GS_BL = 128, GS_BR = 256 };
+
+struct GsSeg { int patch_start, H, W, pw, off; };
+
+struct GsParams {
+    const bf16_raw* g;
+    int* mask;
+    int C, ppi, ph, pw_px, nseg, patches_per_img, total;
+    GsSeg seg[BD_MAX_SEGS];
+};
+
+__device__ __forceinline__ int gs_level(const GsParams& p, int rem) {
+    int s = 0;
+#pragma unroll
+    for (int k = 1; k < BD_MAX_SEGS; ++k)
+        if (k < p.nseg && rem >= p.seg[k].patch_start) s = k;
+    return s;
+}
+
+__global__ __launch_bounds__(256) void gskip_scan_kernel(const GsParams p) {
+    __shared__ int sbits;
+    const int tid = threadIdx.x;
+    const int pid = blockIdx.x;
+    const int n = pid / p.patches_per_img, rem = pid - n * p.patches_per_img;
+    const int s = gs_level(p, rem);
+    const int H = p.seg[s].H, W = p.seg[s].W, pwn = p.seg[s].pw;
+    const int local = rem - p.seg[s].patch_start, by = local / pwn, bx = local - by * pwn;
+    const int y0 = by * p.ph, x0 = bx * p.pw_px;
+    const int cpp = p.C >> 3;
+    const int items = p.ph * p.pw_px * cpp;
+    const long long img = (long long)n * p.ppi + p.seg[s].off;
+    if (tid == 0) sbits = 0;
+    __syncthreads();
+    int bits = 0;
+    constexpr int U = 8;
+    for (int b = 0; b < items; b += 256 * U) {
+        u32x4_t v[U];
+        int pix[U];
+#pragma unroll
+        for (int k = 0; k < U; ++k) {
+            const int i = b + k * 256 + tid;
+            v[k] = (u32x4_t){0u, 0u, 0u, 0u};
+            pix[k] = -1;
+            if (i < items) {
+                const int px = i / cpp, ch = i - px * cpp;
+                const int py = px / p.pw_px, pxx = px - py * p.pw_px;
+                const int y = y0 + py, x = x0 + pxx;
+                if (y < H && x < W) {
+                    v[k] = *reinterpret_cast<const u32x4_t*>(p.g + (img + (long long)y * W + x) * p.C + ch * 8);
+                    pix[k] = px;
+                }
+            }
+        }
+#pragma unroll
+        for (int k = 0; k < U; ++k) {
+            if (pix[k] >= 0 && (v[k][0] | v[k][1] | v[k][2] | v[k][3])) {
+                const int py = pix[k] / p.pw_px, pxx = pix[k] - py * p.pw_px;
+                const bool t = py == 0, bo = py == p.ph - 1, l = pxx == 0, r = pxx == p.pw_px - 1;
+                bits |= GS_ANY | (t ? GS_TOP : 0) | (bo ? GS_BOT : 0) | (l ? GS_LEFT : 0) | (r ? GS_RIGHT : 0) | (t && l ? GS_TL : 0) |
+                        (t && r ? GS_TR : 0) | (bo && l ? GS_BL : 0) | (bo && r ? GS_BR : 0);
+            }
+        }
+    }
+#pragma unroll
+    for (int m = 32; m >= 1; m >>= 1) bits |= __shfl_xor(bits, m, 64);
+    if ((tid & 63) == 0 && bits) atomicOr(&sbits, bits);
+    __syncthreads();
+    if (tid == 0) p.mask[pid] = sbits;
+}
+
+__global__ __launch_bounds__(1024) void gskip_compact_kernel(const GsParams p, int* live, int* list, int* count) {
+    constexpr int KP = 8;
+    __shared__ int wsum[16];
+    const int tid = threadIdx.x, wv = tid >> 6, ln = tid & 63;
+    int base = 0;
+    for (int c0 = 0; c0 < p.total; c0 += 1024 * KP) {
+        int lv[KP];
+#pragma unroll
+        for (int j = 0; j < KP; ++j) {
+            const int q = c0 + tid * KP + j;
+            lv[j] = 0;
+            if (q < p.total) {
+                const int n = q / p.patches_per_img, rem = q - n * p.patches_per_img;
+                const int s = gs_level(p, rem);
+                const int pwn = p.seg[s].pw, rows = (p.seg[s].H + p.ph - 1) / p.ph;
+                const int local = rem - p.seg[s].patch_start, by = local / pwn, bx = local - by * pwn;
+                const int* m = p.mask + (long long)n * p.patches_per_img + p.seg[s].patch_start;
+                const bool up = by > 0, dn = by + 1 < rows, lf = bx > 0, rt = bx + 1 < pwn;
+                int v = m[by * pwn + bx] & GS_ANY;
+                if (up) v |= m[(by - 1) * pwn + bx] & GS_BOT;
+                if (dn) v |= m[(by + 1) * pwn + bx] & GS_TOP;
+                if (lf) v |= m[by * pwn + bx - 1] & GS_RIGHT;
+                if (rt) v |= m[by * pwn + bx + 1] & GS_LEFT;
+                if (up && lf) v |= m[(by - 1) * pwn + bx - 1] & GS_BR;
+                if (up && rt) v |= m[(by - 1) * pwn + bx + 1] & GS_BL;
+                if (dn && lf) v |= m[(by + 1) * pwn + bx - 1] & GS_TR;
+                if (dn && rt) v |= m[(by + 1) * pwn + bx + 1] & GS_TL;
+                lv[j] = v != 0;
+            }
+        }
+        int cnt = 0;
+#pragma unroll
+        for (int j = 0; j < KP; ++j) cnt += lv[j];
+        int inc = cnt;
+#pragma unroll
+        for (int o = 1; o < 64; o <<= 1) {
+            const int y = __shfl_up(inc, o, 64);
+            if (ln >= o) inc += y;
+        }
+        if (ln == 63) wsum[wv] = inc;
+        __syncthreads();
+        int off = base + inc - cnt, tot = 0;
+#pragma unroll
+        for (int w = 0; w < 16; ++w) {
+            off += w < wv ? wsum[w] : 0;
+            tot += wsum[w];
+        }
+#pragma unroll
+        for (int j = 0; j < KP; ++j) {
+            const int q = c0 + tid * KP + j;
+            if (q < p.total) live[q] = lv[j];
+            if (lv[j]) list[off++] = q;
+        }
+        base += tot;
+        __syncthreads();
+    }
+    if (tid == 0) *count = base;
+}
+
+GsParams gs_params(const bd_conv_desc* d, int ph, int pw) {
+    GsParams p{};
+    p.C = d->Cout; p.ppi = d->out_pix_per_img; p.ph = ph; p.pw_px = pw; p.nseg = d->nseg;
+    int ps = 0;
+    for (int s = 0; s < d->nseg; ++s) {
+        GsSeg& sg = p.seg[s];
+        sg.patch_start = ps; sg.H = d->Ho[s]; sg.W = d->Wo[s]; sg.pw = cdiv(d->Wo[s], pw); sg.off = d->out_off[s];
+        ps += cdiv(d->Ho[s], ph) * sg.pw;
+    }
+    p.patches_per_img = ps;
+    p.total = ps * d->N;
+    return p;
+}
+
+}
+
+int bd_gskip_patches(const bd_conv_desc* d, int ph, int pw) {
+    return gs_params(d, ph, pw).total;
+}
+
+void bd_gskip_scan(const bd_conv_desc* d, const void* g, int ph, int pw, int* mask, hipStream_t stream) {
+    GsParams p = gs_params(d, ph, pw);
+    p.g = (const bf16_raw*)g; p.mask = mask;
+    if (p.total > 0) hipLaunchKernelGGL(gskip_scan_kernel, dim3(p.total), dim3(256), 0, stream, p);
+}
+
+void bd_gskip_compact(const bd_conv_desc* d, int ph, int pw, const int* mask, int* live, int* list, int* count, hipStream_t stream) {
+    GsParams p = gs_params(d, ph, pw);
+    p.mask = const_cast<int*>(mask);
+    hipLaunchKernelGGL(gskip_compact_kernel, dim3(1), dim3(1024), 0, stream, p, live, list, count);
+}
diff --git a/basedet_amd/models/engine.py b/basedet_amd/models/engine.py
--- a/basedet_amd/models/engine.py
+++ b/basedet_amd/models/engine.py
@@ -45,6 +45,8 @@
         self.w_fwd = torch.empty((self.cout, k * k, cin), dtype=torch.bfloat16, device=device)
         self.w_dgrad = torch.empty((cin, k * k, self.cout), dtype=torch.bfloat16, device=device) if trainable else None
         self._desc_cache = {}
+        self.gskip = False
+        self._gskip_cache = {}
         self.fp8 = False
         self.fp8_dgrad = False
         self.fp8_wgrad = False
@@ -149,6 +151,17 @@
             self._desc_cache[key] = d
         return d
 
+    def bwd_desc(self, gin: Geom, gout: Geom):
+        d = self.desc(gin, gout)
+        if not self.gskip:
+            return d
+        h = self._gskip_cache.get(id(d))
+        if h is None:
+            nb = ops.conv2d_dgrad_gskip_bytes(d)
+            scratch = torch.empty((max(nb, 4) + 3) // 4, dtype=torch.int32, device=self.device)
+            h = self._gskip_cache[id(d)] = (ops.gskip_desc(d, scratch), scratch)
+        return h[0]
+
     def forward(self, x, gin, gout, y, add=None, relu=False, bits=None, x8=None, y8=None, q_scale=1.0):
         flags = (ops.EPI_RELU if relu else 0) | (ops.EPI_ADD_BEFORE if add is not None else 0)
         if self.fp8_1x1 and x8 is not None and ops.conv1x1_fp8_ok(self.desc(gin, gout), 0):
@@ -185,7 +198,7 @@
             flags |= ops.EPI_MASK
         if maskbits is not None:
             mask = None
-        d = self.desc(gin, gout)
+        d = self.bwd_desc(gin, gout)
         if self.amax_slot is not None and self.probe_ctl[0] and (self.fp8_1x1_dgrad or self.fp8_dgrad):
             ops.absmax_bf16(g, self.amax_slot)
         if self.fp8_1x1_dgrad and g8 is not None and ops.conv1x1_fp8_ok(d, 1):
@@ -205,7 +218,7 @@
         return self.fp8_dgrad or ops.dense_1x1_bits_ok(self.desc(gin, gout))
 
     def wgrad(self, x, g, gin, gout, ws, colsum_ws=None, x8=None, g8=None, queue=None):
-        d = self.desc(gin, gout)
+        d = self.bwd_desc(gin, gout)
         if self.fp8_wgrad and x8 is not None and g8 is not None:
             ops.conv2d_wgrad_fp8(d, x8, g8, 1.0 / (self.act_scale * self.grad_scale), self.gw, ws, row_scale=self.row_scale)
             if self.gb is not None:
@@ -230,7 +243,7 @@
         ops.conv1x1_thin_bwd(x, g, self.w, gin.pixels, self.cin, self.cout, dx, self.gw, self.gb, self.cout_real, ws)
 
     def wgrad_ws_bytes(self, gin, gout):
-        d = self.desc(gin, gout)
+        d = self.bwd_desc(gin, gout)
         n = ops.conv2d_wgrad_bias_workspace_bytes(d) if self.gb is not None else ops.conv2d_wgrad_workspace_bytes(d)
         return max(n, ops.conv2d_wgrad_fp8_workspace_bytes(d)) if self.fp8_wgrad else n
 
diff --git a/basedet_amd/models/retinanet.py b/basedet_amd/models/retinanet.py
--- a/basedet_amd/models/retinanet.py
+++ b/basedet_amd/models/retinanet.py
@@ -34,6 +34,9 @@
         self.cls_score = add("head.cls_score", ch, A * K, 3, 1, 1, bias=True)
         self.box_ld = _round_up(A * 4, 8)
         self.bbox_pred = add("head.bbox_pred", ch, A * 4, 3, 1, 1, bias=True, cout_pad=self.box_ld)
+        if bool(m.get("SPARSE_BOX_BWD", True)) and m.get("WEIGHT_DTYPE", "bf16") == "bf16":
+            for c in self.box_tower + [self.bbox_pred]:
+                c.gskip = True
         scales = np.asarray(m.ANCHOR.SCALES, np.float32).tolist()
         ratios = np.asarray(m.ANCHOR.RATIOS, np.float32).tolist()
         if len(ratios) == 1:
diff --git a/basedet_amd/ops.py b/basedet_amd/ops.py
--- a/basedet_amd/ops.py
+++ b/basedet_amd/ops.py
@@ -109,6 +109,19 @@
         return dx
     check(L().bd_conv2d_dgrad(C.byref(_stamp(d)), ptr(g), ptr(w_packed_t), ptr(add), ptr(mask), ptr(dx), flags, stream_ptr()), "bd_conv2d_dgrad")
     return dx
+
+
+def conv2d_dgrad_gskip_bytes(d):
+    return int(L().bd_conv2d_dgrad_gskip_bytes(C.byref(d)))
+
+
+def gskip_desc(d, scratch=None):
+    h = ConvDesc.from_buffer_copy(d)
+    h.gskip = 1
+    if scratch is not None:
+        h.gskip_ws = scratch.data_ptr()
+        h.gskip_ws_bytes = scratch.numel() * scratch.element_size()
+    return h
 
 
 def quantize_fp8(x, scale, q):
diff --git a/include/basedet_hip.h b/include/basedet_hip.h
--- a/include/basedet_hip.h
+++ b/include/basedet_hip.h
@@ -35,6 +35,9 @@
     int32_t in_pix_per_img, out_pix_per_img;
     int32_t route[4];
     uint32_t sr_seed;
+    int32_t gskip;
+    void* gskip_ws;
+    size_t gskip_ws_bytes;
 } bd_conv_desc;
 
 const char* bd_last_error_string(void);
@@ -50,6 +53,7 @@
 
 int bd_conv2d_dgrad(const bd_conv_desc* d, const void* g, const void* w_packed_t, const void* add,
                     const void* mask, void* dx, int flags, bd_stream_t stream);
+size_t bd_conv2d_dgrad_gskip_bytes(const bd_conv_desc* d);
 
 int bd_conv2d_fwd_bits(const bd_conv_desc* d, const void* x, const void* w_packed, const float* bias, const void* add, void* y,
                        uint32_t* ybits, int flags, bd_stream_t stream);
```
